# adri-romsor/iterative_inference_segm

Measured on AMD Instinct MI355X. Metric: refined images/s (FCN-8 + standard DAE, 10-step iterative inference, 224x224, 11 classes), higher is better.
Workload: dtype f32; 1 GPU; BASELINE configs[1]: FCN-8 + standard DAE (f64c1p2, pool4, trackind, skip), 224x224x3, batch 64/GPU, 10 steps, step 0.1, early stop off; per batch: pred_fcn_fn, val_fn, pred_dae_fn+val_fn, refine, val_fn; global_batch=64, parallelism=dp1

## Files before the change

### include/iiseg.h

```cpp
#ifndef IISEG_H
#define IISEG_H

#include <stdint.h>

#ifdef __cplusplus
extern "C" {
#endif

typedef enum iiseg_status {
    IISEG_OK = 0,
    IISEG_ERR_NULL = -1,
    IISEG_ERR_SHAPE = -2,
    IISEG_ERR_ALIGN = -3,
    IISEG_ERR_LAUNCH = -4,
    IISEG_ERR_UNSUPPORTED = -5
} iiseg_status;

const char* iiseg_strerror(int status);
const char* iiseg_last_hip_error(void);
int iiseg_abi_version(void);
const char* iiseg_target_arch(void);

int iiseg_profile_begin(int capacity);
int iiseg_profile_count(void);
int iiseg_profile_end(float* ms, int capacity);


#define IISEG_CONV_RELU 1u
#define IISEG_CONV_UNPOOL 2u
#define IISEG_CONV_TRANSPOSED2 4u
#define IISEG_CONV_X3 8u
#define IISEG_CONV_ZINS 16u

typedef struct iiseg_conv_desc {
    int32_t B, C1, C2, H, W;
    int32_t Cout, KH, KW, pad, dil;
    int32_t oy0, ox0, OH, OW;
    int32_t AH, AW, ay0, ax0;
    uint32_t flags;
    int32_t Kpad, Mpad;
    int32_t out_ctot, out_c0;
    int32_t out_H, out_W, out_y0, out_x0;
    int32_t tile_y0, tile_x0;
} iiseg_conv_desc;

int iiseg_conv_ktab_entries(const iiseg_conv_desc* d);
int iiseg_conv_plan(iiseg_conv_desc* d);

int iiseg_conv_pack_f32(void* stream, const iiseg_conv_desc* d, const float* w,
                        int64_t stride_o, int64_t stride_c, float* wp, int32_t* ktab);

int iiseg_conv_f32(void* stream, const iiseg_conv_desc* d, const float* x1, const float* x2,
                   const float* pre, const float* pooled, const float* wp, const int32_t* ktab,
                   const float* bias, const float* add, float* out);

int iiseg_conv_small_supported(const iiseg_conv_desc* d);
int iiseg_conv_pool_supported(const iiseg_conv_desc* d);
int iiseg_conv_pool_f32(void* stream, const iiseg_conv_desc* d, const float* x1, const float* x2,
                        const float* pre, const float* pooled, const float* wp, const int32_t* ktab,
                        const float* bias, const float* add, float* out, float* pool_out);

int iiseg_conv_mask_supported(const iiseg_conv_desc* d);
int iiseg_conv_mask_f32(void* stream, const iiseg_conv_desc* d, const float* x1, const float* x2,
                        const float* pre, const float* pooled, const uint8_t* mask_in,
                        const float* wp, const int32_t* ktab, const float* bias, const float* add,
                        float* out, float* pool_out, uint8_t* mask_out);

int iiseg_conv_bnrelu_supported(const iiseg_conv_desc* d);
int iiseg_conv_bnrelu_f32(void* stream, const iiseg_conv_desc* d, const float* x, int64_t x_bstride,
                          const float* beta, const float* gamma, const float* mean,
                          const float* inv_std, const float* wp, const int32_t* ktab,
                          const float* bias, float* out);

#define IISEG_WINO_INPUT 1u
#define IISEG_WINO_GEMM 2u
#define IISEG_WINO_OUTPUT 4u
#define IISEG_WINO_ALL 7u
#define IISEG_WINO_FUSED 8u
int iiseg_conv_wino_supported(const iiseg_conv_desc* d);
int64_t iiseg_conv_wino_weight_elems(const iiseg_conv_desc* d);
int64_t iiseg_conv_wino_workspace_elems(const iiseg_conv_desc* d);
int iiseg_conv_wino_pack_f32(void* stream, const iiseg_conv_desc* d, const float* w,
                             int64_t stride_o, int64_t stride_c, float* U);
int iiseg_conv_wino_f32(void* stream, const iiseg_conv_desc* d, const float* x1, const float* x2,
                        const float* pre, const float* pooled, const float* U, const float* bias,
                        const float* add, float* workspace, float* out, uint32_t stages);

int iiseg_conv_wino_bf16_supported(const iiseg_conv_desc* d);
int64_t iiseg_conv_wino_bf16_weight_bytes(const iiseg_conv_desc* d);
int64_t iiseg_conv_wino_bf16_workspace_bytes(const iiseg_conv_desc* d);
int iiseg_conv_wino_bf16_pack(void* stream, const iiseg_conv_desc* d, const float* w,
                              int64_t stride_o, int64_t stride_c, void* U16);
int iiseg_conv_wino_bf16(void* stream, const iiseg_conv_desc* d, const float* x1, const float* x2,
                         const float* pre, const float* pooled, const void* U16, const float* bias,
                         const float* add, void* workspace, float* out, uint32_t stages);

int iiseg_conv_gemm_bf16_supported(const iiseg_conv_desc* d);
int64_t iiseg_conv_gemm_bf16_weight_bytes(const iiseg_conv_desc* d);
int64_t iiseg_conv_gemm_bf16_workspace_bytes(const iiseg_conv_desc* d);
int iiseg_conv_gemm_bf16_pack(void* stream, const iiseg_conv_desc* d, const float* w,
                              int64_t stride_o, int64_t stride_c, void* U16);
int iiseg_conv_gemm_bf16(void* stream, const iiseg_conv_desc* d, const float* x, const void* U16,
                         const float* bias, void* workspace, float* out);

int iiseg_conv_halo_bf16_supported(const iiseg_conv_desc* d);
int64_t iiseg_conv_halo_bf16_weight_bytes(const iiseg_conv_desc* d);
int iiseg_conv_halo_bf16_pack(void* stream, const iiseg_conv_desc* d, const float* w,
                              int64_t stride_o, int64_t stride_c, void* wp16);
int iiseg_conv_halo_bf16(void* stream, const iiseg_conv_desc* d, const float* x1, const float* x2,
                         const float* pre, const float* pooled, const void* wp16, const float* bias,
                         const float* add, float* out, float* pool_out, const uint8_t* mask_in,
                         uint8_t* mask_out);

int iiseg_conv_wino_f64_supported(const iiseg_conv_desc* d);
int64_t iiseg_conv_wino_f64_weight_elems(const iiseg_conv_desc* d);
int64_t iiseg_conv_wino_f64_workspace_elems(const iiseg_conv_desc* d);
int iiseg_conv_wino_pack_f64(void* stream, const iiseg_conv_desc* d, const double* w,
                             int64_t stride_o, int64_t stride_c, double* U);
int iiseg_conv_wino_f64(void* stream, const iiseg_conv_desc* d, const double* x1, const double* x2,
                        const double* pre, const double* pooled, const double* U, const double* bias,
                        const double* add, double* workspace, double* out);

int iiseg_conv_c8_supported(const iiseg_conv_desc* d);
int iiseg_conv_c8_is_flat(const iiseg_conv_desc* d);
int iiseg_conv_c8_tiling(const iiseg_conv_desc* d, int pool, int32_t* out4);
int iiseg_conv_c8_force_tiling(int kind, int th, int tw);
int iiseg_conv_c8(void* stream, const iiseg_conv_desc* d, const void* x1, const void* x2,
                  const uint8_t* mask_in, const void* wp16, const float* bias, const void* add,
                  int add_kind, void* out, int out_kind, void* pool_out, uint8_t* mask_out);
int iiseg_conv_c8_slice(void* stream, const iiseg_conv_desc* d, const void* x1, int32_t x1_ctot,
                        const void* x2, const uint8_t* mask_in, const void* wp16, const float* bias,
                        const void* add, int add_kind, void* out, int out_kind, void* pool_out,
                        uint8_t* mask_out);
int iiseg_unpool_c8(void* stream, const void* up, const uint8_t* mask, void* out, int BC8, int H, int W,
                    int y0, int x0, int wh, int ww);
int iiseg_conv_c8_m16_supported(const iiseg_conv_desc* d);
int iiseg_conv_c8_m16(void* stream, const iiseg_conv_desc* d, const void* x1, int in_ctot,
                      const uint8_t* mask_in, const float* bn_a, const float* bn_b, const void* wp16,
                      const float* bias, void* out, int out_kind);
int64_t iiseg_conv_c8_m16_workspace_bytes(const iiseg_conv_desc* d);
int iiseg_conv_c8_m16_ws(void* stream, const iiseg_conv_desc* d, const void* x1, int in_ctot,
                         const uint8_t* mask_in, const float* bn_a, const float* bn_b, const void* wp16,
                         const float* bias, void* out, int out_kind, void* workspace,
                         int64_t workspace_bytes, float* stat_mean, float* stat_inv_std, double stat_eps,
                         const float* fold_beta, const float* fold_gamma, float* fold_a, float* fold_b,
                         int fold_n);
int64_t iiseg_conv1x1_c8_weight_bytes(int Cout, int Cin);
int iiseg_conv1x1_c8_pack(void* stream, const float* w, int64_t stride_o, int64_t stride_c, int Cout,
                          int Cin_w, int Cin, void* wp);
int iiseg_conv1x1_c8(void* stream, const void* x, int B, int Cin, int in_ctot, int H, int W,
                     const float* bn_a, const float* bn_b, const void* wp, const float* bias, int Cout,
                     int pool, void* out, int out_ctot, int out_c0);
int iiseg_bn_fold_f32(void* stream, const float* beta, const float* gamma, const float* mean,
                      const float* inv_std, float* a, float* b, int n);
int64_t iiseg_bn_stats_c8_workspace_elems(int n);
int iiseg_bn_stats_c8(void* stream, const void* x, int B, int Ctot, int c0, int n, int H, int W,
                      double eps, float* mean, float* inv_std, double* workspace);
int iiseg_nchw_to_c8(void* stream, const float* x, void* out, int B, int C, int H, int W, int C8n);
int iiseg_c8_to_nchw(void* stream, const void* x, float* out, int B, int C, int H, int W, int C8n);
int iiseg_nchw_to_c8_slice(void* stream, const float* x, void* out, int B, int C, int H, int W, int C8tot,
                           int c8_0);
int iiseg_c8_slice_to_nchw(void* stream, const void* x, float* out, int B, int C, int H, int W, int C8tot,
                           int c8_0);
int iiseg_pool_mask_c8(void* stream, const void* pre, int pre_f32, void* pooled, uint8_t* mask,
                       int BC8, int PH, int PW, int py0, int px0, int H, int W, int y0, int x0, int wh,
                       int ww);
int iiseg_conv_c8_split_weights(void* stream, const float* w, int64_t stride_o, int64_t stride_c,
                                int Cout, int Cin, float* out);
int iiseg_nchw_to_c8x3(void* stream, const float* x, void* out, int B, int C, int H, int W, int C8n);
int iiseg_c8x3_to_nchw(void* stream, const void* x, float* out, int B, int C, int H, int W, int C8n);
int iiseg_pool_mask_c8x3(void* stream, const void* pre, void* pooled, uint8_t* mask, int B, int C8n,
                         int PH, int PW, int py0, int px0, int H, int W, int y0, int x0, int wh,
                         int ww);

int iiseg_conv_gemm_supported(const iiseg_conv_desc* d);
int64_t iiseg_conv_gemm_workspace_elems(const iiseg_conv_desc* d);
int iiseg_conv_gemm_f32(void* stream, const iiseg_conv_desc* d, const float* x, const float* wp,
                        const float* bias, float* workspace, float* out, uint32_t stages);

int iiseg_maxpool2x2_f32(void* stream, const float* x, float* out, int32_t BC, int32_t H,
                         int32_t W);

int iiseg_maxpool2x2_window_f32(void* stream, const float* x, float* out, int32_t BC, int32_t H,
                                int32_t W, int32_t y0, int32_t x0, int32_t wh, int32_t ww);
int iiseg_maxpool2x2_window_f64(void* stream, const double* x, double* out, int32_t BC, int32_t H,
                                int32_t W, int32_t y0, int32_t x0, int32_t wh, int32_t ww);

int iiseg_unpool_eqmask_f32(void* stream, const float* up, const float* pre,
                            const float* pooled, float* out, int32_t BC, int32_t H, int32_t W);
int iiseg_unpool_eqmask_window_f32(void* stream, const float* up, const float* pre,
                                   const float* pooled, float* out, int32_t BC, int32_t H,
                                   int32_t W, int32_t y0, int32_t x0, int32_t wh, int32_t ww);

typedef struct iiseg_deconv_desc {
    int32_t B, Cin, H, W, Cout, K, stride;
    int32_t oy0, ox0, OH, OW;
    int32_t AH, AW, ay0, ax0;
} iiseg_deconv_desc;

int iiseg_deconv_f32(void* stream, const iiseg_deconv_desc* d, const float* x, const float* w,
                     const float* bias, const float* add, float* out);

int iiseg_deconv_phase_supported(const iiseg_deconv_desc* d, int has_add, int is_f64);
int64_t iiseg_deconv_phase_weight_elems(const iiseg_deconv_desc* d);
int iiseg_deconv_phase_pack_f32(void* stream, const iiseg_deconv_desc* d, const float* w, float* wp);
int iiseg_deconv_phase_pack_f64(void* stream, const iiseg_deconv_desc* d, const double* w, double* wp);
int iiseg_deconv_phase_f32(void* stream, const iiseg_deconv_desc* d, const float* x, const float* wp,
                           const float* bias, const float* add, float* out);
int iiseg_deconv_phase_f64(void* stream, const iiseg_deconv_desc* d, const double* x, const double* wp,
                           const double* bias, const double* add, double* out);

int iiseg_crop_softmax_f32(void* stream, const float* score, const float* minuend, float* out,
                           int32_t B, int32_t C, int32_t SH, int32_t SW, int32_t sy0,
                           int32_t sx0, int32_t H, int32_t W);

int iiseg_refine_partials(int32_t H, int32_t W);
int iiseg_refine_update_f32(void* stream, const float* score, float* y, const int32_t* active,
                            double* partial, int32_t B, int32_t C, int32_t SH, int32_t SW,
                            int32_t sy0, int32_t sx0, int32_t H, int32_t W, float step);
int iiseg_refine_update_c8_f32(void* stream, const float* score, float* y, const int32_t* active,
                               double* partial, void* y8, int32_t C8n, int32_t B, int32_t C,
                               int32_t SH, int32_t SW, int32_t sy0, int32_t sx0, int32_t H, int32_t W,
                               float step);
int iiseg_refine_finalize(void* stream, const double* partial, int32_t* active, int32_t* iters,
                          double* last_norm, int32_t B, int32_t nblk, int32_t HW, double eps);

int iiseg_ctx_tail_partials(int32_t H, int32_t W);
int iiseg_ctx_tail_f32(void* stream, const float* x, const float* wp6, int32_t Mpad6, const float* b6,
                       const float* wp7, int32_t Mpad7, const float* b7, float* y, const int32_t* active,
                       double* partial, float* ycat, int32_t cat_ctot, int32_t cat_c0, int32_t cat_H,
                       int32_t cat_W, int32_t cat_y0, int32_t cat_x0, int32_t B, int32_t C, int32_t H,
                       int32_t W, float step);

int iiseg_confusion_f32(void* stream, const float* y, const float* t, int64_t* cm, double* sums,
                        int32_t B, int32_t C, int32_t HW);

int iiseg_confusion_masked_f32(void* stream, const float* y, const float* t, const int32_t* active,
                               int64_t* cm, double* sums, int32_t B, int32_t C, int32_t HW);
int iiseg_confusion_masked_f64(void* stream, const double* y, const double* t,
                               const int32_t* active, int64_t* cm, double* sums, int32_t B,
                               int32_t C, int32_t HW);

int iiseg_count_nonfinite_f32(void* stream, const float* x, int64_t n, int32_t* counter);
int iiseg_count_nonfinite_f64(void* stream, const double* x, int64_t n, int32_t* counter);

int iiseg_sqerr_softmax_bwd_f32(void* stream, const float* score, const float* y, float* gscore,
                                int32_t B, int32_t C, int32_t SH, int32_t SW, int32_t sy0,
                                int32_t sx0, int32_t H, int32_t W);
int iiseg_sqerr_softmax_bwd_f64(void* stream, const double* score, const double* y, double* gscore,
                                int32_t B, int32_t C, int32_t SH, int32_t SW, int32_t sy0,
                                int32_t sx0, int32_t H, int32_t W);
int iiseg_depool_bwd_f32(void* stream, const float* gout, const float* pre, const float* pooled,
                         float* gup, int32_t BC, int32_t H, int32_t W);
int iiseg_depool_bwd_f64(void* stream, const double* gout, const double* pre, const double* pooled,
                         double* gup, int32_t BC, int32_t H, int32_t W);
int iiseg_pool_relu_bwd_f32(void* stream, const float* gpool, const float* pre, const float* pooled,
                            float* gz, int32_t BC, int32_t H, int32_t W);
int iiseg_pool_relu_bwd_f64(void* stream, const double* gpool, const double* pre,
                            const double* pooled, double* gz, int32_t BC, int32_t H, int32_t W);
int iiseg_grad_update_f32(void* stream, const float* score, const float* gthrough, float* y,
                          const int32_t* active, double* partial, int32_t B, int32_t C, int32_t SH,
                          int32_t SW, int32_t sy0, int32_t sx0, int32_t H, int32_t W, float step);
int iiseg_grad_update_f64(void* stream, const double* score, const double* gthrough, double* y,
                          const int32_t* active, double* partial, int32_t B, int32_t C, int32_t SH,
                          int32_t SW, int32_t sy0, int32_t sx0, int32_t H, int32_t W, double step);

int iiseg_add_noise_f32(void* stream, const float* x, const float* eps, float sigma, float* out,
                        int64_t n);
int iiseg_add_noise_f64(void* stream, const double* x, const double* eps, double sigma, double* out,
// ... 86 lines not shown
```

### iterative_inference_segm_amd/_lib.py

```python
import ctypes as C
import os

HERE = os.path.dirname(os.path.abspath(__file__))
LIB_PATH = os.path.join(HERE, 'libiiseg_hip.so')

ABI_VERSION = 32

CONV_RELU = 1
CONV_UNPOOL = 2
CONV_X3 = 8
CONV_TRANSPOSED2 = 4
CONV_ZINS = 16


class ConvDesc(C.Structure):
    _fields_ = [(n, C.c_int32) for n in
                ('B', 'C1', 'C2', 'H', 'W', 'Cout', 'KH', 'KW', 'pad', 'dil',
                 'oy0', 'ox0', 'OH', 'OW', 'AH', 'AW', 'ay0', 'ax0')] + \
               [('flags', C.c_uint32), ('Kpad', C.c_int32), ('Mpad', C.c_int32),
                ('out_ctot', C.c_int32), ('out_c0', C.c_int32),
                ('out_H', C.c_int32), ('out_W', C.c_int32), ('out_y0', C.c_int32),
                ('out_x0', C.c_int32), ('tile_y0', C.c_int32), ('tile_x0', C.c_int32)]


class DeconvDesc(C.Structure):
    _fields_ = [(n, C.c_int32) for n in
                ('B', 'Cin', 'H', 'W', 'Cout', 'K', 'stride', 'oy0', 'ox0', 'OH', 'OW',
                 'AH', 'AW', 'ay0', 'ax0')]


CRF_BILATERAL = 1
CRF_INPUT_0_255 = 2


class CrfDesc(C.Structure):
    _fields_ = [(n, C.c_int32) for n in ('B', 'C', 'H', 'W', 'R')] + [('flags', C.c_uint32)] + \
               [(n, C.c_double) for n in ('sxy_g', 'w_g', 'sxy_b', 'srgb', 'w_b', 'clip')]


_vp, _i32, _i64, _f32, _f64 = C.c_void_p, C.c_int32, C.c_int64, C.c_float, C.c_double

SIGNATURES = {
    'iiseg_strerror': (C.c_char_p, [C.c_int]),
    'iiseg_last_hip_error': (C.c_char_p, []),
    'iiseg_abi_version': (C.c_int, []),
    'iiseg_profile_begin': (C.c_int, [C.c_int]),
    'iiseg_profile_count': (C.c_int, []),
    'iiseg_profile_end': (C.c_int, [C.POINTER(C.c_float), C.c_int]),
    'iiseg_target_arch': (C.c_char_p, []),
    'iiseg_conv_ktab_entries': (C.c_int, [C.POINTER(ConvDesc)]),
    'iiseg_conv_plan': (C.c_int, [C.POINTER(ConvDesc)]),
    'iiseg_conv_pack_f32': (C.c_int, [_vp, C.POINTER(ConvDesc), _vp, _i64, _i64, _vp, _vp]),
    'iiseg_conv_f32': (C.c_int, [_vp, C.POINTER(ConvDesc)] + [_vp] * 9),
    'iiseg_conv_small_supported': (C.c_int, [C.POINTER(ConvDesc)]),
    'iiseg_conv_pool_supported': (C.c_int, [C.POINTER(ConvDesc)]),
    'iiseg_conv_pool_f32': (C.c_int, [_vp, C.POINTER(ConvDesc)] + [_vp] * 10),
    'iiseg_conv_mask_supported': (C.c_int, [C.POINTER(ConvDesc)]),
    'iiseg_conv_mask_f32': (C.c_int, [_vp, C.POINTER(ConvDesc)] + [_vp] * 12),
    'iiseg_conv_bnrelu_supported': (C.c_int, [C.POINTER(ConvDesc)]),
    'iiseg_conv_bnrelu_f32': (C.c_int, [_vp, C.POINTER(ConvDesc), _vp, _i64] + [_vp] * 8),
    'iiseg_conv_wino_supported': (C.c_int, [C.POINTER(ConvDesc)]),
    'iiseg_conv_wino_weight_elems': (_i64, [C.POINTER(ConvDesc)]),
    'iiseg_conv_wino_workspace_elems': (_i64, [C.POINTER(ConvDesc)]),
    'iiseg_conv_wino_pack_f32': (C.c_int, [_vp, C.POINTER(ConvDesc), _vp, _i64, _i64, _vp]),
    'iiseg_conv_wino_f32': (C.c_int, [_vp, C.POINTER(ConvDesc)] + [_vp] * 9 + [C.c_uint32]),
    'iiseg_conv_wino_bf16_supported': (C.c_int, [C.POINTER(ConvDesc)]),
    'iiseg_conv_wino_bf16_weight_bytes': (_i64, [C.POINTER(ConvDesc)]),
    'iiseg_conv_wino_bf16_workspace_bytes': (_i64, [C.POINTER(ConvDesc)]),
    'iiseg_conv_wino_bf16_pack': (C.c_int, [_vp, C.POINTER(ConvDesc), _vp, _i64, _i64, _vp]),
    'iiseg_conv_wino_bf16': (C.c_int, [_vp, C.POINTER(ConvDesc)] + [_vp] * 9 + [C.c_uint32]),
    'iiseg_conv_gemm_bf16_supported': (C.c_int, [C.POINTER(ConvDesc)]),
    'iiseg_conv_gemm_bf16_weight_bytes': (_i64, [C.POINTER(ConvDesc)]),
    'iiseg_conv_gemm_bf16_workspace_bytes': (_i64, [C.POINTER(ConvDesc)]),
    'iiseg_conv_gemm_bf16_pack': (C.c_int, [_vp, C.POINTER(ConvDesc), _vp, _i64, _i64, _vp]),
    'iiseg_conv_gemm_bf16': (C.c_int, [_vp, C.POINTER(ConvDesc)] + [_vp] * 5),
    'iiseg_conv_halo_bf16_supported': (C.c_int, [C.POINTER(ConvDesc)]),
    'iiseg_conv_halo_bf16_weight_bytes': (_i64, [C.POINTER(ConvDesc)]),
    'iiseg_conv_halo_bf16_pack': (C.c_int, [_vp, C.POINTER(ConvDesc), _vp, _i64, _i64, _vp]),
    'iiseg_conv_halo_bf16': (C.c_int, [_vp, C.POINTER(ConvDesc)] + [_vp] * 11),
    'iiseg_conv_wino_f64_supported': (C.c_int, [C.POINTER(ConvDesc)]),
    'iiseg_conv_wino_f64_weight_elems': (_i64, [C.POINTER(ConvDesc)]),
    'iiseg_conv_wino_f64_workspace_elems': (_i64, [C.POINTER(ConvDesc)]),
    'iiseg_conv_wino_pack_f64': (C.c_int, [_vp, C.POINTER(ConvDesc), _vp, _i64, _i64, _vp]),
    'iiseg_conv_wino_f64': (C.c_int, [_vp, C.POINTER(ConvDesc)] + [_vp] * 9),
    'iiseg_conv_c8_supported': (C.c_int, [C.POINTER(ConvDesc)]),
    'iiseg_conv_c8_is_flat': (C.c_int, [C.POINTER(ConvDesc)]),
    'iiseg_conv_c8_force_tiling': (C.c_int, [C.c_int, C.c_int, C.c_int]),
    'iiseg_conv_c8_tiling': (C.c_int, [C.POINTER(ConvDesc), C.c_int, C.POINTER(C.c_int32)]),
    'iiseg_conv_c8': (C.c_int, [_vp, C.POINTER(ConvDesc)] + [_vp] * 6 + [_i32, _vp, _i32, _vp, _vp]),
    'iiseg_conv_c8_slice': (C.c_int, [_vp, C.POINTER(ConvDesc), _vp, _i32] + [_vp] * 5 + [_i32, _vp, _i32, _vp, _vp]),
    'iiseg_unpool_c8': (C.c_int, [_vp] * 4 + [C.c_int] * 7),
    'iiseg_conv_c8_m16_supported': (C.c_int, [C.POINTER(ConvDesc)]),
    'iiseg_conv_c8_m16': (C.c_int, [_vp, C.POINTER(ConvDesc), _vp, _i32] + [_vp] * 6 + [_i32]),
    'iiseg_conv_c8_m16_workspace_bytes': (_i64, [C.POINTER(ConvDesc)]),
    'iiseg_conv_c8_m16_ws': (C.c_int, [_vp, C.POINTER(ConvDesc), _vp, _i32] + [_vp] * 6 + [_i32, _vp, _i64, _vp, _vp, _f64] + [_vp] * 4 + [_i32]),
    'iiseg_conv1x1_c8_weight_bytes': (_i64, [C.c_int, C.c_int]),
    'iiseg_conv1x1_c8_pack': (C.c_int, [_vp, _vp, _i64, _i64, C.c_int, C.c_int, C.c_int, _vp]),
    'iiseg_conv1x1_c8': (C.c_int, [_vp, _vp] + [C.c_int] * 5 + [_vp] * 4 + [C.c_int, C.c_int, _vp, C.c_int, C.c_int]),
    'iiseg_bn_fold_f32': (C.c_int, [_vp] * 7 + [_i32]),
    'iiseg_bn_stats_c8_workspace_elems': (C.c_int64, [_i32]),
    'iiseg_bn_stats_c8': (C.c_int, [_vp, _vp] + [_i32] * 6 + [C.c_double, _vp, _vp, _vp]),
    'iiseg_nchw_to_c8_slice': (C.c_int, [_vp, _vp, _vp] + [_i32] * 6),
    'iiseg_c8_slice_to_nchw': (C.c_int, [_vp, _vp, _vp] + [_i32] * 6),
    'iiseg_nchw_to_c8': (C.c_int, [_vp, _vp, _vp] + [_i32] * 5),
    'iiseg_c8_to_nchw': (C.c_int, [_vp, _vp, _vp] + [_i32] * 5),
    'iiseg_pool_mask_c8': (C.c_int, [_vp, _vp, _i32, _vp, _vp] + [_i32] * 11),
    'iiseg_conv_c8_split_weights': (C.c_int, [_vp, _vp, _i64, _i64, _i32, _i32, _vp]),
    'iiseg_nchw_to_c8x3': (C.c_int, [_vp, _vp, _vp] + [_i32] * 5),
    'iiseg_c8x3_to_nchw': (C.c_int, [_vp, _vp, _vp] + [_i32] * 5),
    'iiseg_pool_mask_c8x3': (C.c_int, [_vp, _vp, _vp, _vp] + [_i32] * 12),
    'iiseg_conv_gemm_supported': (C.c_int, [C.POINTER(ConvDesc)]),
    'iiseg_conv_gemm_workspace_elems': (_i64, [C.POINTER(ConvDesc)]),
    'iiseg_conv_gemm_f32': (C.c_int, [_vp, C.POINTER(ConvDesc)] + [_vp] * 5 + [C.c_uint32]),
    'iiseg_maxpool2x2_f32': (C.c_int, [_vp, _vp, _vp, _i32, _i32, _i32]),
    'iiseg_unpool_eqmask_f32': (C.c_int, [_vp, _vp, _vp, _vp, _vp, _i32, _i32, _i32]),
    'iiseg_maxpool2x2_window_f32': (C.c_int, [_vp] * 3 + [_i32] * 7),
    'iiseg_maxpool2x2_window_f64': (C.c_int, [_vp] * 3 + [_i32] * 7),
    'iiseg_unpool_eqmask_window_f32': (C.c_int, [_vp] * 5 + [_i32] * 7),
    'iiseg_unpool_eqmask_window_f64': (C.c_int, [_vp] * 5 + [_i32] * 7),
    'iiseg_deconv_f32': (C.c_int, [_vp, C.POINTER(DeconvDesc)] + [_vp] * 5),
    'iiseg_deconv_phase_supported': (C.c_int, [C.POINTER(DeconvDesc), C.c_int, C.c_int]),
    'iiseg_deconv_phase_weight_elems': (C.c_int64, [C.POINTER(DeconvDesc)]),
    'iiseg_deconv_phase_pack_f32': (C.c_int, [_vp, C.POINTER(DeconvDesc), _vp, _vp]),
    'iiseg_deconv_phase_pack_f64': (C.c_int, [_vp, C.POINTER(DeconvDesc), _vp, _vp]),
    'iiseg_deconv_phase_f32': (C.c_int, [_vp, C.POINTER(DeconvDesc)] + [_vp] * 5),
    'iiseg_deconv_phase_f64': (C.c_int, [_vp, C.POINTER(DeconvDesc)] + [_vp] * 5),
    'iiseg_crop_softmax_f32': (C.c_int, [_vp, _vp, _vp, _vp] + [_i32] * 8),
    'iiseg_refine_partials': (C.c_int, [_i32, _i32]),
    'iiseg_refine_update_f32': (C.c_int, [_vp] * 5 + [_i32] * 8 + [_f32]),
    'iiseg_refine_update_c8_f32': (C.c_int, [_vp] * 6 + [_i32] * 9 + [_f32]),
    'iiseg_refine_finalize': (C.c_int, [_vp] * 5 + [_i32] * 3 + [_f64]),
    'iiseg_ctx_tail_partials': (C.c_int, [_i32, _i32]),
    'iiseg_ctx_tail_f32': (C.c_int, [_vp] * 3 + [_i32] + [_vp] * 2 + [_i32] + [_vp] * 5 + [_i32] * 10 + [_f32]),
    'iiseg_confusion_f32': (C.c_int, [_vp] * 5 + [_i32] * 3),
    'iiseg_confusion_masked_f32': (C.c_int, [_vp] * 6 + [_i32] * 3),
    'iiseg_confusion_masked_f64': (C.c_int, [_vp] * 6 + [_i32] * 3),
    'iiseg_bn_stats_workspace_elems': (_i64, [_i32]),
    'iiseg_bn_stats_f32': (C.c_int, [_vp, _vp, _i64, _i32, _i32, _i32, _f32, _vp, _vp, _vp]),
    'iiseg_bn_relu_f32': (C.c_int, [_vp, _vp, _i64, _i32, _i32, _i32] + [_vp] * 5),
    'iiseg_bn_stats_f64': (C.c_int, [_vp, _vp, _i64, _i32, _i32, _i32, _f64, _vp, _vp, _vp]),
    'iiseg_bn_relu_f64': (C.c_int, [_vp, _vp, _i64, _i32, _i32, _i32] + [_vp] * 5),
    'iiseg_sqerr_softmax_bwd_f32': (C.c_int, [_vp] * 4 + [_i32] * 8),
    'iiseg_sqerr_softmax_bwd_f64': (C.c_int, [_vp] * 4 + [_i32] * 8),
    'iiseg_depool_bwd_f32': (C.c_int, [_vp] * 5 + [_i32] * 3),
    'iiseg_depool_bwd_f64': (C.c_int, [_vp] * 5 + [_i32] * 3),
    'iiseg_pool_relu_bwd_f32': (C.c_int, [_vp] * 5 + [_i32] * 3),
    'iiseg_pool_relu_bwd_f64': (C.c_int, [_vp] * 5 + [_i32] * 3),
    'iiseg_grad_update_f32': (C.c_int, [_vp] * 6 + [_i32] * 8 + [C.c_float]),
    'iiseg_grad_update_f64': (C.c_int, [_vp] * 6 + [_i32] * 8 + [C.c_double]),
    'iiseg_add_noise_f32': (C.c_int, [_vp, _vp, _vp, C.c_float, _vp, _i64]),
    'iiseg_add_noise_f64': (C.c_int, [_vp, _vp, _vp, C.c_double, _vp, _i64]),
    'iiseg_dropout_apply_f32': (C.c_int, [_vp, _vp, _vp, C.c_float, _i64]),
    'iiseg_dropout_apply_f64': (C.c_int, [_vp, _vp, _vp, C.c_double, _i64]),
    'iiseg_bn_affine_window_f32': (C.c_int, [_vp, _vp] + [_i32] * 8 + [_vp] * 4),
    'iiseg_bn_affine_window_f64': (C.c_int, [_vp, _vp] + [_i32] * 8 + [_vp] * 4),
    'iiseg_conv_plan_f64': (C.c_int, [C.POINTER(ConvDesc)]),
    'iiseg_conv_pack_f64': (C.c_int, [_vp, C.POINTER(ConvDesc), _vp, _i64, _i64, _vp]),
    'iiseg_conv_f64': (C.c_int, [_vp, C.POINTER(ConvDesc)] + [_vp] * 8),
    'iiseg_conv_halo_f64_supported': (C.c_int, [C.POINTER(ConvDesc)]),
    'iiseg_conv_pool_f64_supported': (C.c_int, [C.POINTER(ConvDesc)]),
    'iiseg_conv_pool_f64': (C.c_int, [_vp, C.POINTER(ConvDesc)] + [_vp] * 9),
    'iiseg_conv_mask_f64_supported': (C.c_int, [C.POINTER(ConvDesc)]),
    'iiseg_conv_mask_f64': (C.c_int, [_vp, C.POINTER(ConvDesc)] + [_vp] * 11),
    'iiseg_conv_gemm_f64_supported': (C.c_int, [C.POINTER(ConvDesc)]),
    'iiseg_conv_gemm_f64_workspace_elems': (_i64, [C.POINTER(ConvDesc)]),
    'iiseg_conv_gemm_f64': (C.c_int, [_vp, C.POINTER(ConvDesc)] + [_vp] * 5),
    'iiseg_im2col_f64': (C.c_int, [_vp, _vp, _vp] + [_i32] * 6),
    'iiseg_maxpool2x2_f64': (C.c_int, [_vp, _vp, _vp, _i32, _i32, _i32]),
    'iiseg_unpool_eqmask_f64': (C.c_int, [_vp, _vp, _vp, _vp, _vp, _i32, _i32, _i32]),
    'iiseg_deconv_f64': (C.c_int, [_vp, C.POINTER(DeconvDesc)] + [_vp] * 5),
    'iiseg_crop_softmax_f64': (C.c_int, [_vp, _vp, _vp, _vp] + [_i32] * 8),
    'iiseg_refine_update_f64': (C.c_int, [_vp] * 5 + [_i32] * 8 + [_f64]),
    'iiseg_confusion_f64': (C.c_int, [_vp] * 5 + [_i32] * 3),
    'iiseg_count_nonfinite_f32': (C.c_int, [_vp, _vp, _i64, _vp]),
    'iiseg_count_nonfinite_f64': (C.c_int, [_vp, _vp, _i64, _vp]),
    'iiseg_crf_supported': (C.c_int, [C.POINTER(CrfDesc)]),
    'iiseg_crf_prepare_f32': (C.c_int, [_vp, C.POINTER(CrfDesc)] + [_vp] * 7),
    'iiseg_crf_prepare_f64': (C.c_int, [_vp, C.POINTER(CrfDesc)] + [_vp] * 7),
    'iiseg_crf_step_f32': (C.c_int, [_vp, C.POINTER(CrfDesc)] + [_vp] * 6),
    'iiseg_crf_step_f64': (C.c_int, [_vp, C.POINTER(CrfDesc)] + [_vp] * 6),
}

_lib = None


def load():
    global _lib
    if _lib is not None:
        return _lib
    if not os.path.exists(LIB_PATH):
        raise RuntimeError(
            'libiiseg_hip.so is missing (%s). Build it with '
            '`python -m iterative_inference_segm_amd.build`; there is no CPU fallback.' % LIB_PATH)
    import torch
    lib = C.CDLL(LIB_PATH)
    for name, (res, args) in SIGNATURES.items():
        fn = getattr(lib, name)
        fn.restype = res
        fn.argtypes = args
    if lib.iiseg_abi_version() != ABI_VERSION:
# ... 13 lines not shown
```

### iterative_inference_segm_amd/csrc/abi.hip

```cpp
#include <mutex>
#include <vector>
#include "common.h"

namespace {
std::mutex g_prof_mu;
std::vector<hipEvent_t> g_prof_ev;
int g_prof_on = 0, g_prof_n = 0, g_prof_cap = 0;
}

extern "C" int iiseg_prof_next(hipEvent_t* start, hipEvent_t* stop) {
    if (!g_prof_on) return 0;
    std::lock_guard<std::mutex> g(g_prof_mu);
    if (!g_prof_on || g_prof_n >= g_prof_cap) return 0;
    *start = g_prof_ev[2 * g_prof_n];
    *stop = g_prof_ev[2 * g_prof_n + 1];
    ++g_prof_n;
    return 1;
}

extern "C" int iiseg_profile_begin(int capacity) {
    if (capacity <= 0) return IISEG_ERR_SHAPE;
    std::lock_guard<std::mutex> g(g_prof_mu);
    while ((int)g_prof_ev.size() < 2 * capacity) {
        hipEvent_t e;
        if (hipEventCreate(&e) != hipSuccess) return IISEG_ERR_LAUNCH;
        g_prof_ev.push_back(e);
    }
    g_prof_cap = capacity;
    g_prof_n = 0;
    g_prof_on = 1;
    return IISEG_OK;
}

extern "C" int iiseg_profile_count(void) { return g_prof_on ? g_prof_n : -1; }

extern "C" int iiseg_profile_end(float* ms, int capacity) {
    std::lock_guard<std::mutex> g(g_prof_mu);
    if (!g_prof_on) return -1;
    g_prof_on = 0;
    const int n = g_prof_n < capacity ? g_prof_n : capacity;
    for (int i = 0; i < n; ++i) {
        if (hipEventSynchronize(g_prof_ev[2 * i + 1]) != hipSuccess ||
            hipEventElapsedTime(&ms[i], g_prof_ev[2 * i], g_prof_ev[2 * i + 1]) != hipSuccess)
            return IISEG_ERR_LAUNCH;
    }
    return n;
}

extern "C" const char* iiseg_strerror(int status) {
    switch (status) {
        case IISEG_OK: return "ok";
        case IISEG_ERR_NULL: return "required pointer is NULL";
        case IISEG_ERR_SHAPE: return "inconsistent or unsupported shape";
        case IISEG_ERR_ALIGN: return "pointer is not 16-byte aligned";
        case IISEG_ERR_LAUNCH: return "kernel launch failed";
        case IISEG_ERR_UNSUPPORTED: return "no kernel variant implements this request";
        default: return "unknown iiseg status";
    }
}

extern "C" const char* iiseg_last_hip_error(void) {
    return hipGetErrorString((hipError_t)iiseg_hip_error_slot());
}

extern "C" int iiseg_abi_version(void) { return 32; }
extern "C" const char* iiseg_target_arch(void) { return "gfx950"; }
```

### iterative_inference_segm_amd/csrc/conv_wino.hip

```cpp
#include <hip/hip_runtime.h>
#include <stdint.h>
#include <stdlib.h>
#include "iiseg.h"
#include "common.h"
#include "conv_common.h"

using namespace iiseg;

namespace {

struct WinoParams {
    const float* x1;
    const float* x2;
    const float* pre;
    const float* pooled;
    int h2, w2;
    const float* U;
    const float* bias;
    const float* add;
    float* V;
    float* M;
    float* out;
    int B, C1, C2, H, W;
    int Cout, pad;
    int oy0, ox0, OH, OW;
    int ty0, tx0, nty, ntx;
    int T, Tpad;
    int Kc, Mpad;
    int AH, AW, ay0, ax0;
    int relu;
    int out_ctot, out_c0, out_H, out_W, out_y0, out_x0;
    int n_ttiles, n_mtiles;
};

constexpr int RSRC_W3 = 0x00027000;

__device__ __forceinline__ __amdgpu_buffer_rsrc_t mk_rsrc(const float* base, int bytes) {
    return __builtin_amdgcn_make_buffer_rsrc((void*)base, 0, bytes, RSRC_W3);
}

__global__ void wino_weight_kernel(const float* __restrict__ w, int64_t so, int64_t sc,
                                   float* __restrict__ U, int Cin, int Cout, int Kc, int Mpad) {
    const int64_t n = (int64_t)Kc * Mpad;
    for (int64_t i = blockIdx.x * (int64_t)blockDim.x + threadIdx.x; i < n;
         i += (int64_t)gridDim.x * blockDim.x) {
        const int c = (int)(i / Mpad), co = (int)(i % Mpad);
        double g[3][3], t[4][3];
        const bool real = c < Cin && co < Cout;
#pragma unroll
        for (int a = 0; a < 3; ++a)
#pragma unroll
            for (int b = 0; b < 3; ++b) g[a][b] = real ? (double)w[co * so + c * sc + a * 3 + b] : 0.0;
#pragma unroll
        for (int b = 0; b < 3; ++b) {
            t[0][b] = g[0][b];
            t[1][b] = 0.5 * (g[0][b] + g[1][b] + g[2][b]);
            t[2][b] = 0.5 * (g[0][b] - g[1][b] + g[2][b]);
            t[3][b] = g[2][b];
        }
#pragma unroll
        for (int a = 0; a < 4; ++a) {
            const double u0 = t[a][0], u1 = 0.5 * (t[a][0] + t[a][1] + t[a][2]),
                         u2 = 0.5 * (t[a][0] - t[a][1] + t[a][2]), u3 = t[a][2];
            U[(int64_t)(a * 4 + 0) * n + i] = (float)u0;
            U[(int64_t)(a * 4 + 1) * n + i] = (float)u1;
            U[(int64_t)(a * 4 + 2) * n + i] = (float)u2;
            U[(int64_t)(a * 4 + 3) * n + i] = (float)u3;
        }
    }
}

constexpr int ICH = 4;
template <bool UNPOOL, int PY, int PX>
__global__ __launch_bounds__(256) void wino_input_kernel(const WinoParams p) {
    const int t = blockIdx.x * 256 + threadIdx.x;
    if (t >= p.T) return;
    const int ntt = p.nty * p.ntx;
    const int b = t / ntt;
    const int r = t - b * ntt;
    const int tyl = r / p.ntx, txl = r - tyl * p.ntx;
    const int iy0 = p.ty0 + 2 * tyl - p.pad, ix0 = p.tx0 + 2 * txl - p.pad;
    int rowoff[4];
    bool rok[4], cok[4];
#pragma unroll
    for (int i = 0; i < 4; ++i) {
        rok[i] = (unsigned)(iy0 + i) < (unsigned)p.H;
        cok[i] = (unsigned)(ix0 + i) < (unsigned)p.W;
        rowoff[i] = (iy0 + i) * p.W + ix0;
    }
    constexpr int NQY = UNPOOL ? (PY ? 3 : 2) : 1, NQX = UNPOOL ? (PX ? 3 : 2) : 1;
    const int qy0 = (iy0 - PY) >> 1, qx0 = (ix0 - PX) >> 1;
    bool qrok[NQY], qcok[NQX];
    int qoff[NQY];
    if constexpr (UNPOOL) {
#pragma unroll
        for (int i = 0; i < NQY; ++i) {
            qrok[i] = (unsigned)(qy0 + i) < (unsigned)p.h2;
            qoff[i] = (qy0 + i) * p.w2 + qx0;
        }
#pragma unroll
        for (int j = 0; j < NQX; ++j) qcok[j] = (unsigned)(qx0 + j) < (unsigned)p.w2;
    }
    const size_t HW = (size_t)p.H * p.W, hw2 = (size_t)p.h2 * p.w2;
    const size_t xis = (size_t)p.Kc * p.Tpad;
    constexpr int NC_ = UNPOOL ? ICH / 2 : ICH;
    const int c0 = blockIdx.y * NC_;
    float pv[NC_][4][4];
    float pq[UNPOOL ? NC_ : 1][NQY][NQX], uq[UNPOOL ? NC_ : 1][NQY][NQX];
#pragma unroll
    for (int cc = 0; cc < NC_; ++cc) {
        const int c = min(c0 + cc, p.Kc - 1);
        if constexpr (UNPOOL) {
            const float* prep = p.pre + ((size_t)b * p.C1 + c) * HW;
            const float* poolp = p.pooled + ((size_t)b * p.C1 + c) * hw2;
            const float* upp = p.x1 + ((size_t)b * p.C1 + c) * hw2;
#pragma unroll
            for (int i = 0; i < NQY; ++i)
#pragma unroll
                for (int j = 0; j < NQX; ++j) {
                    const int o = (qrok[i] && qcok[j]) ? qoff[i] + j : 0;
                    pq[cc][i][j] = poolp[o];
                    uq[cc][i][j] = upp[o];
                }
#pragma unroll
            for (int i = 0; i < 4; ++i)
#pragma unroll
                for (int j = 0; j < 4; ++j) pv[cc][i][j] = prep[(rok[i] && cok[j]) ? rowoff[i] + j : 0];
        } else {
            const float* src = c < p.C1 ? p.x1 + ((size_t)b * p.C1 + c) * HW
                                        : p.x2 + ((size_t)b * p.C2 + (c - p.C1)) * HW;
#pragma unroll
            for (int i = 0; i < 4; ++i)
#pragma unroll
                for (int j = 0; j < 4; ++j) pv[cc][i][j] = src[(rok[i] && cok[j]) ? rowoff[i] + j : 0];
        }
    }
#pragma unroll
    for (int cc = 0; cc < NC_; ++cc) {
        const int c = c0 + cc;
        if (c >= p.Kc) break;
        float d[4][4];
#pragma unroll
        for (int i = 0; i < 4; ++i)
#pragma unroll
            for (int j = 0; j < 4; ++j) {
                if constexpr (UNPOOL) {
                    const int qi = (PY + i) >> 1, qj = (PX + j) >> 1;
                    const bool ok = rok[i] && cok[j] && qrok[qi] && qcok[qj];
                    d[i][j] = (ok && pv[cc][i][j] == pq[cc][qi][qj]) ? uq[cc][qi][qj] : 0.f;
                } else {
                    d[i][j] = (rok[i] && cok[j]) ? pv[cc][i][j] : 0.f;
                }
            }
        float e[4][4];
#pragma unroll
        for (int j = 0; j < 4; ++j) {
            e[0][j] = d[0][j] - d[2][j];
            e[1][j] = d[1][j] + d[2][j];
            e[2][j] = d[2][j] - d[1][j];
            e[3][j] = d[1][j] - d[3][j];
        }
        float* v = p.V + (size_t)c * p.Tpad + t;
#pragma unroll
        for (int i = 0; i < 4; ++i) {
            v[(size_t)(i * 4 + 0) * xis] = e[i][0] - e[i][2];
            v[(size_t)(i * 4 + 1) * xis] = e[i][1] + e[i][2];
            v[(size_t)(i * 4 + 2) * xis] = e[i][2] - e[i][1];
            v[(size_t)(i * 4 + 3) * xis] = e[i][1] - e[i][3];
        }
    }
}


constexpr int ILDS_E = 12, ILDS_CH = 8;
template <bool UNPOOL, int NT>
__global__ __launch_bounds__(NT) void wino_input_lds_kernel(const WinoParams p, const int chunks) {
    constexpr int ILDS_CAP = ILDS_E * NT;
    __shared__ __attribute__((aligned(16))) float Ls[2][ILDS_CAP];
    const int tid = threadIdx.x;
    const int b = blockIdx.x / chunks, chunk = blockIdx.x - b * chunks;
    const int ntt = p.nty * p.ntx;
    const int tl0 = chunk * NT, tl = tl0 + tid;
    const bool tvalid = tl < ntt;
    const int row_first = tl0 / p.ntx;
    const int row_last = min(ntt - 1, tl0 + NT - 1) / p.ntx;
    const int NR = 2 * (row_last - row_first + 1) + 2, NC = 2 * p.ntx + 2, NE = NR * NC;
    const int iyb = p.ty0 + 2 * row_first - p.pad, ixb = p.tx0 - p.pad;
    int goff[ILDS_E], qoff[UNPOOL ? ILDS_E : 1];
#pragma unroll
    for (int i = 0; i < ILDS_E; ++i) {
        const int e = i * NT + tid;
        const int r = e / NC, c = e - r * NC;
        const int iy = iyb + r, ix = ixb + c;
        bool ok = e < NE && (unsigned)iy < (unsigned)p.H && (unsigned)ix < (unsigned)p.W;
        goff[i] = ok ? iy * p.W + ix : -1;
        if constexpr (UNPOOL) {
            ok = ok && iy < 2 * p.h2 && ix < 2 * p.w2;
            qoff[i] = ok ? (iy >> 1) * p.w2 + (ix >> 1) : -1;
        }
    }
    const int tyl = tl / p.ntx, txl = tl - tyl * p.ntx;
    const int lbase = 2 * (tyl - row_first) * NC + 2 * txl;
    const size_t HW = (size_t)p.H * p.W, hw2 = (size_t)p.h2 * p.w2;
    const size_t xis = (size_t)p.Kc * p.Tpad;
    const int t = b * ntt + tl;
    const int c0 = blockIdx.y * ILDS_CH;
    float v[ILDS_E];

    auto fetch = [&](int c) __attribute__((always_inline)) {
        if constexpr (UNPOOL) {
            const float* prep = p.pre + ((size_t)b * p.C1 + c) * HW;
            const float* poolp = p.pooled + ((size_t)b * p.C1 + c) * hw2;
            const float* upp = p.x1 + ((size_t)b * p.C1 + c) * hw2;
            float pv[ILDS_E], pq[ILDS_E], uq[ILDS_E];
#pragma unroll
            for (int i = 0; i < ILDS_E; ++i) {
                const int go = qoff[i] >= 0 ? goff[i] : 0, qo = qoff[i] >= 0 ? qoff[i] : 0;
                pv[i] = prep[go];
                pq[i] = poolp[qo];
                uq[i] = upp[qo];
            }
#pragma unroll
            for (int i = 0; i < ILDS_E; ++i) v[i] = (qoff[i] >= 0 && pv[i] == pq[i]) ? uq[i] : 0.f;
        } else {
            const float* src = c < p.C1 ? p.x1 + ((size_t)b * p.C1 + c) * HW
                                        : p.x2 + ((size_t)b * p.C2 + (c - p.C1)) * HW;
            float pv[ILDS_E];
#pragma unroll
            for (int i = 0; i < ILDS_E; ++i) pv[i] = src[goff[i] >= 0 ? goff[i] : 0];
#pragma unroll
            for (int i = 0; i < ILDS_E; ++i) v[i] = goff[i] >= 0 ? pv[i] : 0.f;
        }
    };

    fetch(c0);
    for (int cc = 0; cc < ILDS_CH; ++cc) {
        const int c = c0 + cc;
        float* L = Ls[cc & 1];
#pragma unroll
        for (int i = 0; i < ILDS_E; ++i)
            if (i * NT + tid < NE) L[i * NT + tid] = v[i];
        if (cc + 1 < ILDS_CH) fetch(c + 1);
        __syncthreads();
        if (tvalid) {
            float d[4][4];
#pragma unroll
            for (int i = 0; i < 4; ++i) {
                const float2 lo = *reinterpret_cast<const float2*>(L + lbase + i * NC);
                const float2 hi = *reinterpret_cast<const float2*>(L + lbase + i * NC + 2);
                d[i][0] = lo.x; d[i][1] = lo.y; d[i][2] = hi.x; d[i][3] = hi.y;
            }
            float e[4][4];
#pragma unroll
            for (int j = 0; j < 4; ++j) {
                e[0][j] = d[0][j] - d[2][j];
                e[1][j] = d[1][j] + d[2][j];
                e[2][j] = d[2][j] - d[1][j];
                e[3][j] = d[1][j] - d[3][j];
            }
            float* vo = p.V + (size_t)c * p.Tpad + t;
#pragma unroll
            for (int i = 0; i < 4; ++i) {
                vo[(size_t)(i * 4 + 0) * xis] = e[i][0] - e[i][2];
                vo[(size_t)(i * 4 + 1) * xis] = e[i][1] + e[i][2];
                vo[(size_t)(i * 4 + 2) * xis] = e[i][2] - e[i][1];
                vo[(size_t)(i * 4 + 3) * xis] = e[i][1] - e[i][3];
            }
        }
    }
}

template <int BM, int BN, int WM, int WN, int NBUF, int BK = 16>
__global__ __launch_bounds__(WM * WN * 64, 2) void wino_gemm_kernel(const WinoParams p) {
    constexpr int NCH = BK / 2;
    constexpr int WTM = BM / WM, WTN = BN / WN;
    constexpr int TM = WTM / 32, TN = WTN / 32;
    constexpr int NW = WM * WN, NT = NW * 64;
    constexpr int AV = BK * BM / 4, BV = BK * BN / 4;
    constexpr int NA = NW == 8 ? 256 : NT;
    constexpr int APT = AV / NA, BPT = BV / 256;
    static_assert((NW == 4 || NW == 8) && AV % NA == 0 && BV % 256 == 0, "tile config");

    __shared__ __attribute__((aligned(16))) float As[NBUF][BK][BM];
    __shared__ __attribute__((aligned(16))) float Bs[NBUF][BK][BN];

    const int per_xi = p.n_ttiles * p.n_mtiles;
    int xi, tt, mt;
    {
        const int nb = gridDim.x, bid = blockIdx.x;
        const int q = nb / 8, r = nb % 8, xcd = bid % 8, l = bid / 8;
        const int v = (xcd < r ? xcd * (q + 1) : r * (q + 1) + (xcd - r) * q) + l;
        xi = v / per_xi;
        const int w = v - xi * per_xi;
// ... 192 lines not shown
    for (int s = 0; s < total; ++s) {
        const int buf = s & 1;
        int nxi = xi, nkt1 = kt + 1;
        if (nkt1 == nkt) { nkt1 = 0; ++nxi; }
        const bool more = s + 1 < total;
        float a[2][TM], b[2][TN];
#pragma unroll
        for (int i = 0; i < TM; ++i) a[0][i] = As[buf][lh][wm * WTM + i * 32 + l31];
#pragma unroll
        for (int j = 0; j < TN; ++j) b[0][j] = Bs[buf][lh][wn * WTN + j * 32 + l31];
        static_for<0, NCH>([&](auto CH) __attribute__((always_inline)) {
            constexpr int ch = decltype(CH)::value;
            if constexpr (ch + 1 < NCH) {
                const int kk = (ch + 1) * 2 + lh;
#pragma unroll
                for (int i = 0; i < TM; ++i) a[(ch + 1) & 1][i] = As[buf][kk][wm * WTM + i * 32 + l31];
#pragma unroll
                for (int j = 0; j < TN; ++j) b[(ch + 1) & 1][j] = Bs[buf][kk][wn * WTN + j * 32 + l31];
            }
#pragma unroll
            for (int i = 0; i < TM; ++i)
#pragma unroll
                for (int j = 0; j < TN; ++j)
                    acc[i][j] = __builtin_amdgcn_mfma_f32_32x32x2f32(a[ch & 1][i], b[ch & 1][j],
                                                                     acc[i][j], 0, 0, 0);
            if constexpr (ch == 0) {
                if (more) WINO_STAGE(nxi, nkt1, buf ^ 1)
            }
            __builtin_amdgcn_sched_barrier(0);
        });
        if (nkt1 == 0) {
            const int wi = xi >> 2, wj = xi & 3;
            const float r0 = wi < 3 ? 1.f : 0.f, r1 = wi == 0 ? 0.f : (wi == 1 ? 1.f : -1.f);
            const float c0 = wj < 3 ? 1.f : 0.f, c1 = wj == 0 ? 0.f : (wj == 1 ? 1.f : -1.f);
            const float k00 = r0 * c0, k01 = r0 * c1, k10 = r1 * c0, k11 = r1 * c1;
#define WINO_FOLD(Q, KQ)                                                                            \
            if ((KQ) != 0.f) {                                                                      \
                _Pragma("unroll") for (int i = 0; i < TM; ++i)                                      \
                _Pragma("unroll") for (int j = 0; j < TN; ++j)                                      \
                _Pragma("unroll") for (int r = 0; r < 16; ++r)                                      \
                    Y[Q][i][j][r] = fmaf((KQ), acc[i][j][r], Y[Q][i][j][r]);                        \
            }
            WINO_FOLD(0, k00)
            WINO_FOLD(1, k01)
            WINO_FOLD(2, k10)
            WINO_FOLD(3, k11)
#undef WINO_FOLD
#pragma unroll
            for (int i = 0; i < TM; ++i)
#pragma unroll
                for (int j = 0; j < TN; ++j)
#pragma unroll
                    for (int r = 0; r < 16; ++r) acc[i][j][r] = 0.f;
        }
        xi = nxi;
        kt = nkt1;
        asm volatile("s_waitcnt vmcnt(0)" ::: "memory");
        __syncthreads();
    }
#undef WINO_STAGE

    typedef float f32x2u __attribute__((ext_vector_type(2), aligned(4)));
    const int ntt = p.nty * p.ntx;
    const size_t OPL = (size_t)p.out_H * p.out_W, APL = (size_t)p.AH * p.AW;
    float* Lbias = &As[0][0][0];
    for (int f = tid; f < BM; f += NT) Lbias[f] = (p.bias && m0 + f < p.Cout) ? p.bias[m0 + f] : 0.f;
    __syncthreads();
    float bias_r[TM][16];
#pragma unroll
    for (int i = 0; i < TM; ++i)
#pragma unroll
        for (int r = 0; r < 16; ++r) bias_r[i][r] = Lbias[wm * WTM + i * 32 + (r & 3) + 8 * (r >> 2) + 4 * lh];
#pragma unroll
    for (int j = 0; j < TN; ++j) {
        const int t = t0 + wn * WTN + j * 32 + l31;
        if (t >= p.T) continue;
        const int b = t / ntt;
        const int rr = t - b * ntt;
        const int tyl = rr / p.ntx, txl = rr - tyl * p.ntx;
        const int wy = p.ty0 + 2 * tyl - p.oy0, wx = p.tx0 + 2 * txl - p.ox0;
        const bool rok[2] = {(unsigned)wy < (unsigned)p.OH, (unsigned)(wy + 1) < (unsigned)p.OH};
        const bool cok[2] = {(unsigned)wx < (unsigned)p.OW, (unsigned)(wx + 1) < (unsigned)p.OW};
        const bool pair = cok[0] && cok[1];
        float* ob = p.out + ((size_t)b * p.out_ctot + p.out_c0) * OPL +
                    (ptrdiff_t)(p.out_y0 + wy) * p.out_W + p.out_x0 + wx;
        const float* ab = p.add ? p.add + (size_t)b * p.Cout * APL +
                                      (ptrdiff_t)(p.ay0 + wy) * p.AW + p.ax0 + wx
                                : nullptr;
#pragma unroll
        for (int i = 0; i < TM; ++i)
#pragma unroll
            for (int r = 0; r < 16; ++r) {
                const int co = m0 + wm * WTM + i * 32 + (r & 3) + 8 * (r >> 2) + 4 * lh;
                if (co >= p.Cout) continue;
                const float bias = bias_r[i][r];
                float* oc = ob + (size_t)co * OPL;
                const float* ac = ab ? ab + (size_t)co * APL : nullptr;
#pragma unroll
                for (int a = 0; a < 2; ++a) {
                    if (!rok[a]) continue;
                    float v0 = Y[2 * a][i][j][r] + bias, v1 = Y[2 * a + 1][i][j][r] + bias;
                    if (pair) {
                        if (ac) {
                            const f32x2u a2 = *reinterpret_cast<const f32x2u*>(ac + a * p.AW);
                            v0 += a2[0];
                            v1 += a2[1];
                        }
                        if (p.relu) {
                            v0 = fmaxf(v0, 0.f);
                            v1 = fmaxf(v1, 0.f);
                        }
                        *reinterpret_cast<f32x2u*>(oc + (size_t)a * p.out_W) = f32x2u{v0, v1};
                    } else {
                        if (cok[0]) {
                            if (ac) v0 += ac[a * p.AW];
                            if (p.relu) v0 = fmaxf(v0, 0.f);
                            oc[(size_t)a * p.out_W] = v0;
                        }
                        if (cok[1]) {
                            if (ac) v1 += ac[a * p.AW + 1];
                            if (p.relu) v1 = fmaxf(v1, 0.f);
                            oc[(size_t)a * p.out_W + 1] = v1;
                        }
                    }
                }
            }
    }
}

constexpr int OCH = 4;
__global__ __launch_bounds__(256) void wino_output_kernel(const WinoParams p) {
    const int t = blockIdx.x * 256 + threadIdx.x;
    if (t >= p.T) return;
    const int ntt = p.nty * p.ntx;
    const int b = t / ntt;
    const int r = t - b * ntt;
    const int tyl = r / p.ntx, txl = r - tyl * p.ntx;
    const int wy = p.ty0 + 2 * tyl - p.oy0, wx = p.tx0 + 2 * txl - p.ox0;
    const bool okr[2] = {(unsigned)wy < (unsigned)p.OH, (unsigned)(wy + 1) < (unsigned)p.OH};
    const bool okc[2] = {(unsigned)wx < (unsigned)p.OW, (unsigned)(wx + 1) < (unsigned)p.OW};
    const size_t xis = (size_t)p.Mpad * p.Tpad;
    const size_t OPL = (size_t)p.out_H * p.out_W, APL = (size_t)p.AH * p.AW;
    const int co0 = blockIdx.y * OCH;
    float mv[OCH][16], av[OCH][4];
#pragma unroll
    for (int cc = 0; cc < OCH; ++cc) {
        const int co = min(co0 + cc, p.Cout - 1);
        const float* m = p.M + (size_t)co * p.Tpad + t;
#pragma unroll
        for (int x = 0; x < 16; ++x) mv[cc][x] = m[(size_t)x * xis];
        if (p.add) {
            const float* ad = p.add + ((size_t)b * p.Cout + co) * APL;
#pragma unroll
            for (int i = 0; i < 2; ++i)
#pragma unroll
                for (int j = 0; j < 2; ++j) {
                    const bool ok = okr[i] && okc[j];
                    const ptrdiff_t idx = (ptrdiff_t)(p.ay0 + wy + i) * p.AW + p.ax0 + wx + j;
                    const float a = ad[ok ? idx : 0];
                    av[cc][i * 2 + j] = ok ? a : 0.f;
                }
        }
    }
#pragma unroll
    for (int cc = 0; cc < OCH; ++cc) {
        const int co = co0 + cc;
        if (co >= p.Cout) break;
        float s2[2][4];
#pragma unroll
        for (int j = 0; j < 4; ++j) {
            const float m0 = mv[cc][j], m1 = mv[cc][4 + j], m2 = mv[cc][8 + j], m3 = mv[cc][12 + j];
            s2[0][j] = m0 + m1 + m2;
            s2[1][j] = m1 - m2 - m3;
        }
        const float bias = p.bias ? p.bias[co] : 0.f;
        float* o = p.out + ((size_t)b * p.out_ctot + p.out_c0 + co) * OPL +
                   (ptrdiff_t)(p.out_y0 + wy) * p.out_W + p.out_x0 + wx;
#pragma unroll
        for (int i = 0; i < 2; ++i) {
            float y[2] = {s2[i][0] + s2[i][1] + s2[i][2], s2[i][1] - s2[i][2] - s2[i][3]};
#pragma unroll
            for (int j = 0; j < 2; ++j) {
                if (okr[i] && okc[j]) {
                    float v = y[j] + bias;
                    if (p.add) v += av[cc][i * 2 + j];
                    if (p.relu) v = fmaxf(v, 0.f);
                    o[(ptrdiff_t)i * p.out_W + j] = v;
                }
            }
        }
    }
}

inline int round_up(int v, int m) { return (v + m - 1) / m * m; }

struct WinoGeom {
    int Kc, Mpad, bm, ty0, tx0, nty, ntx, T, Tpad;
};

int wino_geom(const iiseg_conv_desc* d, WinoGeom& g) {
    if (!d) return IISEG_ERR_NULL;
    if (d->KH != 3 || d->KW != 3 || d->dil != 1 || (d->flags & IISEG_CONV_TRANSPOSED2))
        return IISEG_ERR_UNSUPPORTED;
    if ((d->flags & IISEG_CONV_UNPOOL) && d->C2 != 0) return IISEG_ERR_UNSUPPORTED;
    if (d->B <= 0 || d->C1 <= 0 || d->C2 < 0 || d->H <= 0 || d->W <= 0 || d->Cout <= 0 ||
        d->pad < 0 || d->OH <= 0 || d->OW <= 0 || d->oy0 < 0 || d->ox0 < 0)
        return IISEG_ERR_SHAPE;
    const int fullH = d->H + 2 * d->pad - 2, fullW = d->W + 2 * d->pad - 2;
    if (d->oy0 + d->OH > fullH || d->ox0 + d->OW > fullW) return IISEG_ERR_SHAPE;
    if ((d->C1 + d->C2) % 16) return IISEG_ERR_UNSUPPORTED;
    g.Kc = d->C1 + d->C2;
    g.bm = d->Cout > 128 ? 256 : (d->Cout > 64 ? 128 : 64);
    g.Mpad = round_up(d->Cout, g.bm);
    if ((d->tile_y0 | d->tile_x0) & ~1) return IISEG_ERR_SHAPE;
    g.ty0 = d->oy0 - ((d->oy0 - d->tile_y0) & 1);
    g.tx0 = d->ox0 - ((d->ox0 - d->tile_x0) & 1);
    g.nty = (d->oy0 + d->OH - g.ty0 + 1) >> 1;
    g.ntx = (d->ox0 + d->OW - g.tx0 + 1) >> 1;
    const int64_t T = (int64_t)d->B * g.nty * g.ntx;
    const int64_t Tpad = (T + 127) / 128 * 128;
    if (Tpad * g.Kc * 4 >= (int64_t)1 << 31 || (int64_t)g.Kc * g.Mpad * 4 >= (int64_t)1 << 31)
        return IISEG_ERR_UNSUPPORTED;
    g.T = (int)T;
    g.Tpad = (int)Tpad;
    return IISEG_OK;
}

void launch_wino_input(hipStream_t s, const WinoParams& p, bool unpool) {
    static const int lds = getenv("IISEG_WINO_INPUT_LDS") ? atoi(getenv("IISEG_WINO_INPUT_LDS")) : 1;
    const int ntt = p.nty * p.ntx;
    int nt = 0;
    double best = 0.0;
    for (int cand = 256; cand >= 128; cand >>= 1) {
        const int span = (cand - 1 + p.ntx - 1) / p.ntx + 1;
        const int rows = span < p.nty ? span : p.nty;
        if ((2 * rows + 2) * (2 * p.ntx + 2) > ILDS_E * cand) continue;
        const double util = (double)ntt / (((ntt + cand - 1) / cand) * cand);
        if (util > best + 0.02) { best = util; nt = cand; }
    }
    if (lds && nt && best >= 0.8 && p.Kc % ILDS_CH == 0) {
        const int chunks = (ntt + nt - 1) / nt;
        const dim3 g2(p.B * chunks, p.Kc / ILDS_CH);
#define WINO_ILDS(U, N) IISEG_LAUNCH((wino_input_lds_kernel<U, N>), g2, dim3(N), 0, s, p, chunks)
        if (unpool) { if (nt == 256) WINO_ILDS(true, 256); else if (nt == 128) WINO_ILDS(true, 128); else WINO_ILDS(true, 64); }
        else { if (nt == 256) WINO_ILDS(false, 256); else if (nt == 128) WINO_ILDS(false, 128); else WINO_ILDS(false, 64); }
#undef WINO_ILDS
        return;
    }
    const int nc = unpool ? ICH / 2 : ICH;
    const dim3 grid((p.T + 255) / 256, (p.Kc + nc - 1) / nc), block(256);
    if (!unpool) {
        IISEG_LAUNCH((wino_input_kernel<false, 0, 0>), grid, block, 0, s, p);
        return;
    }
    const int py = (p.ty0 - p.pad) & 1, px = (p.tx0 - p.pad) & 1;
    if (py && px) IISEG_LAUNCH((wino_input_kernel<true, 1, 1>), grid, block, 0, s, p);
    else if (py) IISEG_LAUNCH((wino_input_kernel<true, 1, 0>), grid, block, 0, s, p);
    else if (px) IISEG_LAUNCH((wino_input_kernel<true, 0, 1>), grid, block, 0, s, p);
    else IISEG_LAUNCH((wino_input_kernel<true, 0, 0>), grid, block, 0, s, p);
}

}

int iiseg_wino_output_launch(hipStream_t s, const iiseg_conv_desc* d, const float* M, int Mpad,
                             int Tpad, const float* bias, const float* add, float* out) {
    WinoParams p = {};
    p.M = const_cast<float*>(M);
    p.bias = bias; p.add = add; p.out = out;
    p.B = d->B; p.Cout = d->Cout; p.pad = d->pad;
    p.oy0 = d->oy0; p.ox0 = d->ox0; p.OH = d->OH; p.OW = d->OW;
    p.ty0 = d->oy0 - ((d->oy0 - d->tile_y0) & 1);
    p.tx0 = d->ox0 - ((d->ox0 - d->tile_x0) & 1);
    p.nty = (d->oy0 + d->OH - p.ty0 + 1) >> 1;
    p.ntx = (d->ox0 + d->OW - p.tx0 + 1) >> 1;
    p.T = d->B * p.nty * p.ntx;
    p.Tpad = Tpad; p.Mpad = Mpad;
    p.AH = d->AH; p.AW = d->AW; p.ay0 = d->ay0; p.ax0 = d->ax0;
    p.relu = (d->flags & IISEG_CONV_RELU) ? 1 : 0;
    p.out_ctot = d->out_ctot > 0 ? d->out_ctot : d->Cout;
    p.out_c0 = d->out_ctot > 0 ? d->out_c0 : 0;
    p.out_H = d->out_H > 0 ? d->out_H : d->OH;
    p.out_W = d->out_H > 0 ? d->out_W : d->OW;
    p.out_y0 = d->out_H > 0 ? d->out_y0 : 0;
    p.out_x0 = d->out_H > 0 ? d->out_x0 : 0;
    IISEG_LAUNCH(wino_output_kernel, dim3((p.T + 255) / 256, (d->Cout + OCH - 1) / OCH),
                       dim3(256), 0, s, p);
    return iiseg_check_launch();
}

extern "C" int iiseg_conv_wino_supported(const iiseg_conv_desc* d) {
    WinoGeom g;
    return wino_geom(d, g) == IISEG_OK ? 1 : 0;
}

extern "C" int64_t iiseg_conv_wino_weight_elems(const iiseg_conv_desc* d) {
    WinoGeom g;
    if (wino_geom(d, g) != IISEG_OK) return 0;
    return (int64_t)16 * g.Kc * g.Mpad;
}

extern "C" int64_t iiseg_conv_wino_workspace_elems(const iiseg_conv_desc* d) {
    WinoGeom g;
    if (wino_geom(d, g) != IISEG_OK) return 0;
    return (int64_t)16 * g.Tpad * ((int64_t)g.Kc + g.Mpad);
}

extern "C" int iiseg_conv_wino_pack_f32(void* stream, const iiseg_conv_desc* d, const float* w,
                                        int64_t stride_o, int64_t stride_c, float* U) {
    WinoGeom g;
    const int st = wino_geom(d, g);
    if (st) return st;
    if (!w || !U) return IISEG_ERR_NULL;
    const int64_t n = (int64_t)g.Kc * g.Mpad;
    const int grid = (int)((n + 255) / 256 < 4096 ? (n + 255) / 256 : 4096);
    IISEG_LAUNCH(wino_weight_kernel, dim3(grid), dim3(256), 0, (hipStream_t)stream, w,
                       stride_o, stride_c, U, d->C1 + d->C2, d->Cout, g.Kc, g.Mpad);
    return iiseg_check_launch();
}

extern "C" int iiseg_conv_wino_f32(void* stream, const iiseg_conv_desc* d, const float* x1,
                                   const float* x2, const float* pre, const float* pooled,
                                   const float* U, const float* bias,
                                   const float* add, float* workspace, float* out,
                                   uint32_t stages) {
    WinoGeom g;
    const int st = wino_geom(d, g);
    if (st) return st;
    if (!x1 || !U || !workspace || !out) return IISEG_ERR_NULL;
    if (d->C2 > 0 && !x2) return IISEG_ERR_NULL;
    const bool unpool = (d->flags & IISEG_CONV_UNPOOL) != 0;
    if (unpool && (!pre || !pooled)) return IISEG_ERR_NULL;
    if (((uintptr_t)U & 15) || ((uintptr_t)workspace & 15)) return IISEG_ERR_ALIGN;
    WinoParams p;
    p.x1 = x1;
    p.x2 = x2;
    p.pre = pre;
    p.pooled = pooled;
    p.h2 = d->H / 2;
    p.w2 = d->W / 2;
    p.U = U;
    p.bias = bias;
    p.add = add;
    p.V = workspace;
    p.M = workspace + (size_t)16 * g.Kc * g.Tpad;
    p.out = out;
    p.B = d->B; p.C1 = d->C1; p.C2 = d->C2; p.H = d->H; p.W = d->W;
    p.Cout = d->Cout; p.pad = d->pad;
    p.oy0 = d->oy0; p.ox0 = d->ox0; p.OH = d->OH; p.OW = d->OW;
    p.ty0 = g.ty0; p.tx0 = g.tx0; p.nty = g.nty; p.ntx = g.ntx;
    p.T = g.T; p.Tpad = g.Tpad; p.Kc = g.Kc; p.Mpad = g.Mpad;
    p.AH = d->AH; p.AW = d->AW; p.ay0 = d->ay0; p.ax0 = d->ax0;
    if (add && (d->ay0 < 0 || d->ax0 < 0 || d->ay0 + d->OH > d->AH || d->ax0 + d->OW > d->AW))
        return IISEG_ERR_SHAPE;
    p.relu = (d->flags & IISEG_CONV_RELU) ? 1 : 0;
    p.out_ctot = d->out_ctot > 0 ? d->out_ctot : d->Cout;
    p.out_c0 = d->out_ctot > 0 ? d->out_c0 : 0;
    if (p.out_c0 < 0 || p.out_c0 + d->Cout > p.out_ctot) return IISEG_ERR_SHAPE;
    p.out_H = d->out_H > 0 ? d->out_H : d->OH;
    p.out_W = d->out_H > 0 ? d->out_W : d->OW;
    p.out_y0 = d->out_H > 0 ? d->out_y0 : 0;
    p.out_x0 = d->out_H > 0 ? d->out_x0 : 0;
    if (p.out_y0 < 0 || p.out_x0 < 0 || p.out_y0 + d->OH > p.out_H || p.out_x0 + d->OW > p.out_W)
        return IISEG_ERR_SHAPE;
    p.n_ttiles = g.Tpad / 128;
    p.n_mtiles = g.Mpad / g.bm;
    hipStream_t s = (hipStream_t)stream;
    const int tb = (g.T + 255) / 256;
    if (stages & IISEG_WINO_FUSED) {
        if (g.Kc % 32) return IISEG_ERR_UNSUPPORTED;
        if (stages & IISEG_WINO_INPUT)
            launch_wino_input(s, p, unpool);
        if (stages & IISEG_WINO_GEMM) {
            if (g.bm == 64) {
                p.n_mtiles = g.Mpad / 64;
                IISEG_LAUNCH((wino_fused_kernel<64, 128, 1, 4, 32, 2>),
                                   dim3(p.n_ttiles * p.n_mtiles), dim3(256), 0, s, p);
                return iiseg_check_launch();
            }
            p.n_mtiles = g.Mpad / 128;
            const int w0 = p.n_ttiles * p.n_mtiles, w2 = (g.Tpad / 64) * p.n_mtiles;
            const double cost0 = (w0 + 255) / 256, cost2 = 0.5 * 1.03 * ((w2 + 255) / 256);
            static const int bk64 = getenv("IISEG_WINO_FUSED_BK") ? atoi(getenv("IISEG_WINO_FUSED_BK")) == 64 : 0;
            const bool big = bk64 && g.Kc % 64 == 0;
            if (g.Kc <= 128 || cost2 < cost0) {
                p.n_ttiles = g.Tpad / 64;
                if (big)
                    IISEG_LAUNCH((wino_fused_kernel<128, 64, 2, 2, 64, 2>),
                                       dim3(p.n_ttiles * p.n_mtiles), dim3(256), 0, s, p);
                else
                IISEG_LAUNCH((wino_fused_kernel<128, 64, 2, 2, 32, 2>),
                                   dim3(p.n_ttiles * p.n_mtiles), dim3(256), 0, s, p);
            } else if (big)
                IISEG_LAUNCH((wino_fused_kernel<128, 128, 2, 4, 64, 2>),
                                   dim3(p.n_ttiles * p.n_mtiles), dim3(512), 0, s, p);
            else
            IISEG_LAUNCH((wino_fused_kernel<128, 128, 2, 4, 32, 2>),
                               dim3(p.n_ttiles * p.n_mtiles), dim3(512), 0, s, p);
        }
        return iiseg_check_launch();
    }
    if (stages & IISEG_WINO_INPUT)
        launch_wino_input(s, p, unpool);
    const int grid = 16 * p.n_ttiles * p.n_mtiles;
    if (stages & IISEG_WINO_GEMM) {
        static const int nbuf = getenv("IISEG_WINO_NBUF") ? atoi(getenv("IISEG_WINO_NBUF")) : 2;
        int bm = g.bm;
        if (bm == 64) {
            IISEG_LAUNCH((wino_gemm_kernel<64, 128, 1, 4, 2>), dim3(grid), dim3(256), 0, s, p);
            bm = 0;
        }
        if (bm == 256) {
            const int w256 = grid, w128 = 2 * grid;
            if (0.5 * 1.06 * ((w128 + 255) / 256) < (double)((w256 + 255) / 256)) bm = 128;
        }
        const int grid2 = bm ? 16 * p.n_ttiles * (g.Mpad / bm) : 0;
        if (bm) p.n_mtiles = g.Mpad / bm;
        static const int bk32 = getenv("IISEG_WINO_GEMM_BK") ? atoi(getenv("IISEG_WINO_GEMM_BK")) == 32 : 0;
        if (bm && bk32 && g.Kc % 32 == 0 && nbuf != 3) {
            if (bm == 256)
                IISEG_LAUNCH((wino_gemm_kernel<256, 128, 4, 2, 2, 32>), dim3(grid), dim3(512), 0, s, p);
            else
                IISEG_LAUNCH((wino_gemm_kernel<128, 128, 2, 2, 2, 32>), dim3(grid2), dim3(256), 0, s, p);
        } else
        if (bm == 0) {
        } else if (bm == 256 && nbuf == 3)
            IISEG_LAUNCH((wino_gemm_kernel<256, 128, 4, 2, 3>), dim3(grid), dim3(512), 0, s, p);
        else if (bm == 256)
            IISEG_LAUNCH((wino_gemm_kernel<256, 128, 4, 2, 2>), dim3(grid), dim3(512), 0, s, p);
        else if (nbuf == 3)
            IISEG_LAUNCH((wino_gemm_kernel<128, 128, 2, 2, 3>), dim3(grid2), dim3(256), 0, s, p);
        else
            IISEG_LAUNCH((wino_gemm_kernel<128, 128, 2, 2, 2>), dim3(grid2), dim3(256), 0, s, p);
    }
    if (stages & IISEG_WINO_OUTPUT)
        IISEG_LAUNCH(wino_output_kernel, dim3(tb, (d->Cout + OCH - 1) / OCH), dim3(256), 0, s,
                           p);
    return iiseg_check_launch();
}

namespace {

struct GemmConvGeom {
    int K, Kpad, Mpad, bm, T, Tpad, S, Kc;
};

__global__ __launch_bounds__(256) void gemm_im2col_kernel(const float* __restrict__ x,
                                                          float* __restrict__ V, int B, int C, int H,
                                                          int W, int KH, int KW, int OH, int OW, int K,
                                                          int Kpad, int T, int Tpad) {
    const int t = blockIdx.x * 256 + threadIdx.x;
    if (t >= T) return;
    const int OHW = OH * OW;
    const int b = t / OHW, r = t - b * OHW;
    const int oy = r / OW, ox = r - oy * OW;
    const int KK = KH * KW;
    const float* xb = x + (size_t)b * C * H * W + (size_t)oy * W + ox;
    for (int k = blockIdx.y; k < Kpad; k += gridDim.y) {
        float v = 0.f;
        if (k < K) {
            const int c = k / KK, tap = k - c * KK;
            const int ky = tap / KW, kx = tap - ky * KW;
            v = xb[(size_t)c * H * W + ky * W + kx];
        }
        V[(size_t)k * Tpad + t] = v;
    }
}

__global__ __launch_bounds__(256) void gemm_output_kernel(const float* __restrict__ M,
                                                          const float* __restrict__ bias,
                                                          float* __restrict__ out, int Cout, int OHW,
                                                          int T, int Tpad, int Mpad, int S, int relu) {
    const int t = blockIdx.x * 256 + threadIdx.x;
    if (t >= T) return;
    const int b = t / OHW, px = t - b * OHW;
    const size_t ss = (size_t)Mpad * Tpad;
    for (int co = blockIdx.y; co < Cout; co += gridDim.y) {
        const float* m = M + (size_t)co * Tpad + t;
        float v = m[0];
        for (int s = 1; s < S; ++s) v += m[(size_t)s * ss];
        if (bias) v += bias[co];
        if (relu) v = fmaxf(v, 0.f);
        out[((size_t)b * Cout + co) * OHW + px] = v;
    }
}

int gemm_conv_geom(const iiseg_conv_desc* d, GemmConvGeom& g) {
    if (!d) return IISEG_ERR_NULL;
    if (d->pad != 0 || d->dil != 1 || d->C2 != 0 ||
        (d->flags & (IISEG_CONV_UNPOOL | IISEG_CONV_TRANSPOSED2)))
        return IISEG_ERR_UNSUPPORTED;
    const int fullH = d->H - d->KH + 1, fullW = d->W - d->KW + 1;
    if (fullH <= 0 || fullW <= 0) return IISEG_ERR_SHAPE;
    if (d->oy0 != 0 || d->ox0 != 0 || d->OH != fullH || d->OW != fullW || d->out_ctot != 0 ||
        d->out_H != 0)
        return IISEG_ERR_UNSUPPORTED;
    g.K = d->C1 * d->KH * d->KW;
    g.Kpad = d->Kpad;
    g.Mpad = d->Mpad;
    if (g.Kpad < g.K || g.Kpad % 16 || g.Mpad % 128 || g.Mpad < d->Cout) return IISEG_ERR_UNSUPPORTED;
    g.bm = g.Mpad % 256 == 0 ? 256 : 128;
    const int64_t T = (int64_t)d->B * fullH * fullW;
    const int64_t Tpad = (T + 127) / 128 * 128;
    if (Tpad * g.Kpad * 4 >= (int64_t)1 << 31 || (int64_t)g.Kpad * g.Mpad * 4 >= (int64_t)1 << 31)
        return IISEG_ERR_UNSUPPORTED;
    g.T = (int)T;
    g.Tpad = (int)Tpad;
    const int tiles = 25 * (g.Mpad / g.bm), units = g.Kpad / 16;
    const double tile_s = 2.0 * g.Kpad * g.bm * 128 / (131e12 / 256);
    const double red_s = 8.0 * g.Mpad * 3200 / 5e12;
    double best = 1e30;
    g.S = 1;
    for (int S = 1; S <= 16; ++S) {
        if (units % S || units / S < 8) continue;
        const double cost = (double)((S * tiles + 255) / 256) / S * tile_s + S * red_s;
        if (cost < best) { best = cost; g.S = S; }
    }
    g.Kc = g.Kpad / g.S;
    return IISEG_OK;
}

}

// ... 59 lines not shown
```

### iterative_inference_segm_amd/csrc/pool_unpool.hip

```cpp
#include "common.h"

namespace {

template <typename T>
__global__ __launch_bounds__(256) void maxpool2x2_kernel(const T* __restrict__ x,
                                                         T* __restrict__ out, int BC, int H,
                                                         int W, int h, int w) {
    const size_t n = (size_t)BC * h * w;
    for (size_t i = blockIdx.x * (size_t)blockDim.x + threadIdx.x; i < n;
         i += (size_t)gridDim.x * blockDim.x) {
        const int ox = (int)(i % w);
        const size_t t = i / w;
        const int oy = (int)(t % h);
        const size_t bc = t / h;
        const T* r0 = x + (bc * H + 2 * oy) * (size_t)W + 2 * ox;
        const T* r1 = r0 + W;
        const T a = r0[0] > r0[1] ? r0[0] : r0[1];
        const T b = r1[0] > r1[1] ? r1[0] : r1[1];
        out[i] = a > b ? a : b;
    }
}

template <typename T>
__global__ __launch_bounds__(256) void unpool_eqmask_kernel(const T* __restrict__ up,
                                                            const T* __restrict__ pre,
                                                            const T* __restrict__ pooled,
                                                            T* __restrict__ out, int BC, int H,
                                                            int W, int h, int w) {
    const size_t n = (size_t)BC * H * W;
    for (size_t i = blockIdx.x * (size_t)blockDim.x + threadIdx.x; i < n;
         i += (size_t)gridDim.x * blockDim.x) {
        const int x = (int)(i % W);
        const size_t t = i / W;
        const int y = (int)(t % H);
        const size_t bc = t / H;
        T v = 0;
        if (y < 2 * h && x < 2 * w) {
            const size_t j = (bc * h + (y >> 1)) * (size_t)w + (x >> 1);
            v = (pre[i] == pooled[j]) ? up[j] : (T)0;
        }
        out[i] = v;
    }
}

template <typename T>
__global__ __launch_bounds__(256) void maxpool2x2_window_kernel(const T* __restrict__ x,
                                                                T* __restrict__ out, int BC, int H,
                                                                int W, int h, int w, int y0, int x0,
                                                                int wh, int ww) {
    const size_t n = (size_t)BC * wh * ww;
    if (n < ((size_t)1 << 31)) {
        const unsigned n32 = (unsigned)n, uww = (unsigned)ww, uwh = (unsigned)wh;
        for (unsigned i = blockIdx.x * blockDim.x + threadIdx.x; i < n32; i += gridDim.x * blockDim.x) {
            const unsigned t = i / uww;
            const int ox = x0 + (int)(i - t * uww);
            const unsigned bc = t / uwh;
            const int oy = y0 + (int)(t - bc * uwh);
            const T* r0 = x + ((size_t)bc * H + 2 * oy) * (size_t)W + 2 * ox;
            const T* r1 = r0 + W;
            const T a = r0[0] > r0[1] ? r0[0] : r0[1];
            const T b = r1[0] > r1[1] ? r1[0] : r1[1];
            out[((size_t)bc * h + oy) * (size_t)w + ox] = a > b ? a : b;
        }
        return;
    }
    for (size_t i = blockIdx.x * (size_t)blockDim.x + threadIdx.x; i < n;
         i += (size_t)gridDim.x * blockDim.x) {
        const int ox = x0 + (int)(i % ww);
        const size_t t = i / ww;
        const int oy = y0 + (int)(t % wh);
        const size_t bc = t / wh;
        const T* r0 = x + (bc * H + 2 * oy) * (size_t)W + 2 * ox;
        const T* r1 = r0 + W;
        const T a = r0[0] > r0[1] ? r0[0] : r0[1];
        const T b = r1[0] > r1[1] ? r1[0] : r1[1];
        out[(bc * h + oy) * (size_t)w + ox] = a > b ? a : b;
    }
}

template <typename T>
__global__ __launch_bounds__(256) void unpool_eqmask_window_kernel(
    const T* __restrict__ up, const T* __restrict__ pre, const T* __restrict__ pooled,
    T* __restrict__ out, int BC, int H, int W, int h, int w, int y0, int x0, int wh, int ww) {
    const size_t n = (size_t)BC * wh * ww;
    for (size_t i = blockIdx.x * (size_t)blockDim.x + threadIdx.x; i < n;
         i += (size_t)gridDim.x * blockDim.x) {
        const int x = x0 + (int)(i % ww);
        const size_t t = i / ww;
        const int y = y0 + (int)(t % wh);
        const size_t bc = t / wh;
        const size_t o = (bc * H + y) * (size_t)W + x;
        T v = 0;
        if (y < 2 * h && x < 2 * w) {
            const size_t j = (bc * h + (y >> 1)) * (size_t)w + (x >> 1);
            v = (pre[o] == pooled[j]) ? up[j] : (T)0;
        }
        out[o] = v;
    }
}

template <typename T>
__global__ __launch_bounds__(256) void depool_bwd_kernel(const T* __restrict__ gout,
                                                         const T* __restrict__ pre,
                                                         const T* __restrict__ pooled,
                                                         T* __restrict__ gup, int BC, int H, int W,
                                                         int h, int w) {
    const size_t n = (size_t)BC * h * w;
    for (size_t i = blockIdx.x * (size_t)blockDim.x + threadIdx.x; i < n;
         i += (size_t)gridDim.x * blockDim.x) {
        const int ox = (int)(i % w);
        const size_t t = i / w;
        const int oy = (int)(t % h);
        const size_t bc = t / h;
        const size_t o = (bc * H + 2 * oy) * (size_t)W + 2 * ox;
        const T m = pooled[i];
        T s = 0;
        s += pre[o] == m ? gout[o] : (T)0;
        s += pre[o + 1] == m ? gout[o + 1] : (T)0;
        s += pre[o + W] == m ? gout[o + W] : (T)0;
        s += pre[o + W + 1] == m ? gout[o + W + 1] : (T)0;
        gup[i] = s;
    }
}

template <typename T>
__global__ __launch_bounds__(256) void pool_relu_bwd_kernel(const T* __restrict__ gpool,
                                                            const T* __restrict__ pre,
                                                            const T* __restrict__ pooled,
                                                            T* __restrict__ gz, int BC, int H, int W,
                                                            int h, int w) {
    const size_t n = (size_t)BC * H * W;
    for (size_t i = blockIdx.x * (size_t)blockDim.x + threadIdx.x; i < n;
         i += (size_t)gridDim.x * blockDim.x) {
        const int x = (int)(i % W);
        const size_t t = i / W;
        const int y = (int)(t % H);
        const size_t bc = t / H;
        T v = 0;
        if (y < 2 * h && x < 2 * w) {
            const size_t j = (bc * h + (y >> 1)) * (size_t)w + (x >> 1);
            const T pv = pre[i];
            v = (pv == pooled[j] && pv > (T)0) ? gpool[j] : (T)0;
        }
        gz[i] = v;
    }
}

inline int grid_for(size_t n) {
    size_t g = (n + 255) / 256;
    return (int)(g < 1 ? 1 : (g > 8192 ? 8192 : g));
}

template <typename T>
int maxpool(void* stream, const T* x, T* out, int32_t BC, int32_t H, int32_t W) {
    if (!x || !out) return IISEG_ERR_NULL;
    if (BC <= 0 || H < 2 || W < 2) return IISEG_ERR_SHAPE;
    const int h = H / 2, w = W / 2;
    IISEG_LAUNCH(maxpool2x2_kernel<T>, dim3(grid_for((size_t)BC * h * w)), dim3(256), 0,
                       (hipStream_t)stream, x, out, BC, H, W, h, w);
    return iiseg_check_launch();
}

template <typename T>
int unpool(void* stream, const T* up, const T* pre, const T* pooled, T* out, int32_t BC, int32_t H,
           int32_t W) {
    if (!up || !pre || !pooled || !out) return IISEG_ERR_NULL;
    if (BC <= 0 || H < 2 || W < 2) return IISEG_ERR_SHAPE;
    IISEG_LAUNCH(unpool_eqmask_kernel<T>, dim3(grid_for((size_t)BC * H * W)), dim3(256), 0,
                       (hipStream_t)stream, up, pre, pooled, out, BC, H, W, H / 2, W / 2);
    return iiseg_check_launch();
}

template <typename T>
int maxpool_window(void* stream, const T* x, T* out, int32_t BC, int32_t H, int32_t W, int32_t y0,
                   int32_t x0, int32_t wh, int32_t ww) {
    if (!x || !out) return IISEG_ERR_NULL;
    if (BC <= 0 || H < 2 || W < 2 || y0 < 0 || x0 < 0 || wh <= 0 || ww <= 0 || y0 + wh > H / 2 ||
        x0 + ww > W / 2)
        return IISEG_ERR_SHAPE;
    IISEG_LAUNCH(maxpool2x2_window_kernel<T>, dim3(grid_for((size_t)BC * wh * ww)), dim3(256),
                       0, (hipStream_t)stream, x, out, BC, H, W, H / 2, W / 2, y0, x0, wh, ww);
    return iiseg_check_launch();
}

template <typename T>
int unpool_window(void* stream, const T* up, const T* pre, const T* pooled, T* out, int32_t BC,
                  int32_t H, int32_t W, int32_t y0, int32_t x0, int32_t wh, int32_t ww) {
    if (!up || !pre || !pooled || !out) return IISEG_ERR_NULL;
    if (BC <= 0 || H < 2 || W < 2 || y0 < 0 || x0 < 0 || wh <= 0 || ww <= 0 || y0 + wh > H ||
        x0 + ww > W)
        return IISEG_ERR_SHAPE;
    IISEG_LAUNCH(unpool_eqmask_window_kernel<T>, dim3(grid_for((size_t)BC * wh * ww)),
                       dim3(256), 0, (hipStream_t)stream, up, pre, pooled, out, BC, H, W, H / 2,
                       W / 2, y0, x0, wh, ww);
    return iiseg_check_launch();
}

template <typename T>
int depool_bwd(void* stream, const T* gout, const T* pre, const T* pooled, T* gup, int32_t BC,
               int32_t H, int32_t W) {
    if (!gout || !pre || !pooled || !gup) return IISEG_ERR_NULL;
    if (BC <= 0 || H < 2 || W < 2) return IISEG_ERR_SHAPE;
    IISEG_LAUNCH(depool_bwd_kernel<T>, dim3(grid_for((size_t)BC * (H / 2) * (W / 2))), dim3(256),
                       0, (hipStream_t)stream, gout, pre, pooled, gup, BC, H, W, H / 2, W / 2);
    return iiseg_check_launch();
}

template <typename T>
int pool_relu_bwd(void* stream, const T* gpool, const T* pre, const T* pooled, T* gz, int32_t BC,
                  int32_t H, int32_t W) {
    if (!gpool || !pre || !pooled || !gz) return IISEG_ERR_NULL;
    if (BC <= 0 || H < 2 || W < 2) return IISEG_ERR_SHAPE;
    IISEG_LAUNCH(pool_relu_bwd_kernel<T>, dim3(grid_for((size_t)BC * H * W)), dim3(256), 0,
                       (hipStream_t)stream, gpool, pre, pooled, gz, BC, H, W, H / 2, W / 2);
    return iiseg_check_launch();
}

}

extern "C" int iiseg_depool_bwd_f32(void* stream, const float* gout, const float* pre,
                                    const float* pooled, float* gup, int32_t BC, int32_t H, int32_t W) {
    return depool_bwd<float>(stream, gout, pre, pooled, gup, BC, H, W);
}
extern "C" int iiseg_depool_bwd_f64(void* stream, const double* gout, const double* pre,
                                    const double* pooled, double* gup, int32_t BC, int32_t H,
                                    int32_t W) {
    return depool_bwd<double>(stream, gout, pre, pooled, gup, BC, H, W);
}
extern "C" int iiseg_pool_relu_bwd_f32(void* stream, const float* gpool, const float* pre,
                                       const float* pooled, float* gz, int32_t BC, int32_t H,
                                       int32_t W) {
    return pool_relu_bwd<float>(stream, gpool, pre, pooled, gz, BC, H, W);
}
extern "C" int iiseg_pool_relu_bwd_f64(void* stream, const double* gpool, const double* pre,
                                       const double* pooled, double* gz, int32_t BC, int32_t H,
                                       int32_t W) {
    return pool_relu_bwd<double>(stream, gpool, pre, pooled, gz, BC, H, W);
}

extern "C" int iiseg_maxpool2x2_window_f32(void* stream, const float* x, float* out, int32_t BC,
                                           int32_t H, int32_t W, int32_t y0, int32_t x0,
                                           int32_t wh, int32_t ww) {
    return maxpool_window<float>(stream, x, out, BC, H, W, y0, x0, wh, ww);
}
extern "C" int iiseg_maxpool2x2_window_f64(void* stream, const double* x, double* out, int32_t BC,
                                           int32_t H, int32_t W, int32_t y0, int32_t x0,
                                           int32_t wh, int32_t ww) {
    return maxpool_window<double>(stream, x, out, BC, H, W, y0, x0, wh, ww);
}
extern "C" int iiseg_unpool_eqmask_window_f32(void* stream, const float* up, const float* pre,
                                              const float* pooled, float* out, int32_t BC,
                                              int32_t H, int32_t W, int32_t y0, int32_t x0,
                                              int32_t wh, int32_t ww) {
    return unpool_window<float>(stream, up, pre, pooled, out, BC, H, W, y0, x0, wh, ww);
}
extern "C" int iiseg_unpool_eqmask_window_f64(void* stream, const double* up, const double* pre,
                                              const double* pooled, double* out, int32_t BC,
                                              int32_t H, int32_t W, int32_t y0, int32_t x0,
                                              int32_t wh, int32_t ww) {
    return unpool_window<double>(stream, up, pre, pooled, out, BC, H, W, y0, x0, wh, ww);
}

extern "C" int iiseg_maxpool2x2_f32(void* stream, const float* x, float* out, int32_t BC,
                                    int32_t H, int32_t W) {
    return maxpool<float>(stream, x, out, BC, H, W);
}
extern "C" int iiseg_maxpool2x2_f64(void* stream, const double* x, double* out, int32_t BC,
                                    int32_t H, int32_t W) {
    return maxpool<double>(stream, x, out, BC, H, W);
}
extern "C" int iiseg_unpool_eqmask_f32(void* stream, const float* up, const float* pre,
                                       const float* pooled, float* out, int32_t BC, int32_t H,
                                       int32_t W) {
    return unpool<float>(stream, up, pre, pooled, out, BC, H, W);
}
extern "C" int iiseg_unpool_eqmask_f64(void* stream, const double* up, const double* pre,
                                       const double* pooled, double* out, int32_t BC, int32_t H,
                                       int32_t W) {
    return unpool<double>(stream, up, pre, pooled, out, BC, H, W);
}
```

### iterative_inference_segm_amd/dae.py

```python
import os

import numpy as np

import torch

from . import ops
from .weights import load_param_list

F64_FUSE_UNPOOL = os.environ.get('IISEG_F64_FUSE_UNPOOL', '1') != '0'


def _n_pool(concat_h, additional_pool):
    n = int(concat_h[-1][-1]) if 'pool' in concat_h[-1] else 0
    return n, n + additional_pool


def param_order(concat_h=('pool4',), conv_before_pool=1, additional_pool=2,
                unpool_type='trackind', bn=0):
    _, total = _n_pool(list(concat_h), additional_pool)
    names = []
    for p in range(total):
        for i in range(1, conv_before_pool + 1):
            names.append('conv%d_%d' % (p + 1, i))
            if bn:
# ... 30 lines not shown
        if unpool_type not in ('standard', 'trackind', 'inverse'):
            raise ValueError('Unkown unpool type')
        if unpool_type == 'standard' and dtype != torch.float32:
            raise NotImplementedError("unpool_type='standard' (4x4/2 transposed conv) is float32 "
                                      "only")
        self.bn = bool(bn)
        self.enc_bn = {}
        self.noise, self.dropout = float(noise), float(dropout)
        self.emulate_noise = bool(emulate_noise)
        self.random_source = None
        self._seed, self._gen = int(seed), None
        self.dtype = dtype
        self._bwd, self._saved = None, None
        self.unpool_type = unpool_type
        self.concat_h, self.padding, self.skip = concat_h, padding, skip
        self.conv_before_pool = conv_before_pool
        self.n_classes = n_classes
        self.n_pool, self.total = _n_pool(concat_h, additional_pool)
        self.device = device
        self.enc, self.dec = {}, {}
        for p in range(self.total):
            for i in range(1, conv_before_pool + 1):
                first_pad = (p == 0 and i == 1 and (len(concat_h) == 1 or pad_multi_concat)
                             and concat_h[-1] != 'input' and padding > 0)
                name = 'conv%d_%d' % (p + 1, i)
                self.enc[name] = ops.Conv(params[name][0], params[name][1],
                                          pad=padding if first_pad else 1, relu=True,
                                          device=device, dtype=dtype, mma=mma)
                if bn:
                    self.enc_bn[name] = tuple(
                        torch.as_tensor(np.asarray(a)).to(dtype).contiguous().to(device)
                        for a in params[name + '_bn'])
        self.hsplit = {}
        if dtype == torch.float32 and os.environ.get('IISEG_H_SPLIT', '1') != '0':
            prev = n_classes
            for p in range(self.total):
                name = 'conv%d_1' % (p + 1)
                W, b = params[name]
                ch = W.shape[1] - prev
                at = 'input' if p == 0 else 'pool%d' % p
                if ch > 0 and at in concat_h:
                    Wt = torch.as_tensor(W)
                    conv_h = ops.Conv(Wt[:, :ch].contiguous(), b, pad=self.enc[name].pad,
                                      relu=False, device=device, dtype=dtype, mma=mma)
                    conv_y = ops.Conv(Wt[:, ch:].contiguous(), None, pad=self.enc[name].pad,
                                      relu=True, device=device, dtype=dtype, mma=mma)
                    self.hsplit[name] = (conv_h, conv_y)
                prev = params['conv%d_%d' % (p + 1, conv_before_pool)][0].shape[0]
        for p in range(self.total, 0, -1):
            if unpool_type == 'standard':
                name = 'up%d' % p
                self.dec[name] = ops.Conv(params[name][0], params[name][1], pad=0, relu=False,
                                          layout='iohw', transposed=True, device=device,
                                          dtype=dtype, mma=mma)
                continue
            name = 'up_conv%d' % p
            W, b = params[name]
            if bn:
                beta, gamma, mean, inv_std = (np.asarray(a, np.float64) for a in params[name + '_bn'])
                sc = gamma * inv_std
                W = np.asarray(W, np.float64) * sc[:, None, None, None]
                b = (np.asarray(b, np.float64) - mean) * sc + beta
            self.dec[name] = ops.Conv(W, b, pad=1, relu=False, device=device,
                                      dtype=dtype, mma=mma)
        self.conv_log = None
        env = os.environ.get('IISEG_FUSE_UNPOOL', 'auto')
        self.fuse_unpool = None if env == 'auto' else env != '0'
        self.dce = os.environ.get('IISEG_DECODER_DCE', '1') != '0'
        self.licm = os.environ.get('IISEG_ENCODER_LICM', '1') != '0'
        self.fold_border = os.environ.get('IISEG_DAE_BORDER_FOLD', '1') != '0'
        self._store = None
        self._scratch_sessions = {}
        self.trace = None
        self.use_masks = os.environ.get('IISEG_DEPOOL_MASKS', '1') != '0'
        self.keep_pre = False

    def _mask_levels(self, overridden):
        if not self.use_masks or overridden or self.keep_pre or self.bn or self.trace is not None or \
                self.unpool_type == 'standard' or self.dtype not in (torch.float32, torch.float64) or \
                self.fuse_unpool is False:
            return frozenset()
        levels = set()
        for L in range(1, self.total + 1):
            enc = self.enc['conv%d_%d' % (L, self.conv_before_pool)]
            fed_by_h = self.conv_before_pool == 1 and \
                ('input' if L == 1 else 'pool%d' % (L - 1)) in self.concat_h
            if not fed_by_h and enc.pool_fusable(False) and enc.mask_ok(False) and \
                    self.dec['up_conv%d' % L].mask_ok(False):
                levels.add(L)
        return frozenset(levels)

    def new_session(self, h_list=None, y=None, tags=None):
        tags = list(tags) if tags is not None else [None] * len(h_list or [])
        if self.licm and self.fold_border and y is not None and tags and \
                all(t is not None for t in tags):
            key = (tuple(t[0] for t in tags), tuple(y.shape), y.dtype)
            st = self._store
            if st is not None and st.get('key') == key and st.get('primed'):
                st['y8_fresh'] = False
                st['h_fresh'] = True
                st['h_dep'] = [t[1] for t in tags]
                return st
            self._store = {'primed': False, 'key': key}
            return self._store
        if self.c8 and y is not None and h_list is not None and \
                all(isinstance(h, torch.Tensor) for h in h_list):
            key = (tuple(tuple(h.shape) for h in h_list), tuple(y.shape), y.dtype)
            st = self._scratch_sessions.get(key)
            if st is None:
                while len(self._scratch_sessions) >= 2:
                    self._scratch_sessions.pop(next(iter(self._scratch_sessions)))
                st = self._scratch_sessions[key] = {'stable': True}
            else:
                self._scratch_sessions[key] = self._scratch_sessions.pop(key)
            st.update(primed=False, h_stale=True, y8_fresh=False, h_fresh=False)
            return st
        return {'primed': False}

    @property
    def stable_sessions(self):
        return bool(self.c8)

    def conv_layers(self):
        d = dict(self.enc)
        d.update(self.dec)
        return d

    def scores(self, h_list, y, mask_override=None, session=None):
        h_list = list(h_list)
        if len(h_list) != len(self.concat_h):
            raise ValueError('expected %d h tensors, got %d' % (len(self.concat_h), len(h_list)))
        if self.c8:
            if mask_override is not None:
                raise NotImplementedError("mask injection needs fp32 activations (mma='bf16' / 'f32')")
            return self._scores_c8(h_list, y, session)
        pos = 0
        pending_h = None
        h_fresh = session is not None and session.get('h_fresh', False)
        if self.concat_h[pos] == 'input':
            pending_h, pos = h_list[pos], pos + 1
        t = y
        pre, pool = {}, {0: y}
        primed = session is not None and session.get('primed', False) and self.licm
        will_override = mask_override is not None or (
            self.emulate_noise and (self.noise > 0 or self.dropout > 0) and
            self.unpool_type == 'trackind')
        masked = self._mask_levels(will_override)
        if session is not None:
            if primed and session.get('masked', frozenset()) != masked:
                primed = False
            session['masked'] = masked
            if not primed:
                session['gen'] = session.get('gen', 0) + 1
        masks = {}
        dep = (0, 0, y.shape[2], y.shape[3])
        ydep = dep

        def clip(lo, hi, size):
            lo, hi = max(lo, 0), min(hi, size)
            return lo, max(hi - lo, 0)

        for p in range(self.total):
            fused_pool = None
            for i in range(1, self.conv_before_pool + 1):
                name = 'conv%d_%d' % (p + 1, i)
                conv = self.enc[name]
                fh, fw = conv.out_hw(t.shape[2], t.shape[3])
                ydep = (clip(ydep[0] + conv.pad - (conv.KH - 1), ydep[0] + ydep[2] + conv.pad, fh) +
                        clip(ydep[1] + conv.pad - (conv.KW - 1), ydep[1] + ydep[3] + conv.pad, fw))
                ydep = (ydep[0], ydep[2], ydep[1], ydep[3])
                kw = dict(anchor=(ydep[0], ydep[1]))
                if primed and pending_h is not None and h_fresh:
                    hd = session['h_dep'][pos - 1]
                    y1 = max(dep[0] + dep[2], hd[0] + hd[2])
                    x1 = max(dep[1] + dep[3], hd[1] + hd[3])
                    dep = (min(dep[0], hd[0]), min(dep[1], hd[1]), 0, 0)
                    dep = (dep[0], dep[1], y1 - dep[0], x1 - dep[1])
                if primed:
                    buf = session[name]
                    fh, fw = buf.shape[2], buf.shape[3]
                    wy0, wh = clip(dep[0] + conv.pad - (conv.KH - 1), dep[0] + dep[2] + conv.pad, fh)
                    wx0, ww = clip(dep[1] + conv.pad - (conv.KW - 1), dep[1] + dep[3] + conv.pad, fw)
                    dep = (wy0, wx0, wh, ww)
                    kw.update(window=dep, out=buf, place=(wy0, wx0))
                if pending_h is not None and name in self.hsplit:
                    conv_h, conv_y = self.hsplit[name]
                    keep = session is not None and self.licm
                    hb = session.get('hb_' + name) if keep else None
                    if hb is None:
                        hb = conv_h(pending_h)
                        if keep:
                            session['hb_' + name] = hb
                    elif h_fresh:
                        hd = session['h_dep'][pos - 1]
                        hy0, hh = clip(hd[0] + conv_h.pad - (conv_h.KH - 1), hd[0] + hd[2] + conv_h.pad,
                                       hb.shape[2])
                        hx0, hw = clip(hd[1] + conv_h.pad - (conv_h.KW - 1), hd[1] + hd[3] + conv_h.pad,
                                       hb.shape[3])
                        conv_h(pending_h, window=(hy0, hx0, hh, hw), out=hb, place=(hy0, hx0))
                    off = kw['place'] if 'place' in kw else (0, 0)
                    t = conv_y(t, add=hb, add_off=off, **kw)
                    pending_h = None
                elif pending_h is not None:
                    t = conv(pending_h, x2=t, **kw)
                    pending_h = None
                else:
                    pw_ = None
                    if i == self.conv_before_pool and not self.bn:
                        pw_ = conv.pool_window(t.shape[2], t.shape[3], dep if primed else None, c8=False)
                    if pw_ is not None:
                        fh, fw = conv.out_hw(t.shape[2], t.shape[3])
                        if primed:
                            pooled_t = session['pool%d' % (p + 1)]
                            kw.update(window=pw_, place=(pw_[0], pw_[1]))
                        else:
                            pooled_t = torch.empty((t.shape[0], conv.Cout, fh // 2, fw // 2),
                                                   dtype=t.dtype, device=t.device)
                        fused_pool = pooled_t
                        kw['pool_out'] = pooled_t
                    if (p + 1) in masked:
                        if pw_ is None:
                            raise RuntimeError('internal: level %d was planned for byte masks but '
                                               'its pool is not fused' % (p + 1))
                        m = session['mask%d' % (p + 1)] if primed else \
                            torch.empty(pooled_t.shape, dtype=torch.uint8, device=t.device)
                        masks[p + 1] = m
                        kw.update(mask_out=m, store_out=False)
                        conv(t, **kw)
                        t = torch.empty((t.shape[0], conv.Cout, fh, fw), dtype=t.dtype, device='meta')
                    else:
                        t = conv(t, **kw)
                if self.bn:
                    ops.bn_affine(t, self.enc_bn[name], window=dep if primed else None)
                if session is not None and not primed:
                    session[name] = t
                    if (p + 1) in masks and i == self.conv_before_pool:
                        session['mask%d' % (p + 1)] = masks[p + 1]
                self._count(name, conv, t, computed=(dep[2], dep[3]) if primed else None)
            pre[p + 1] = t
            ydep = (ydep[0] // 2, ydep[1] // 2,
                    min((ydep[0] + ydep[2] + 1) // 2, t.shape[2] // 2) - ydep[0] // 2,
                    min((ydep[1] + ydep[3] + 1) // 2, t.shape[3] // 2) - ydep[1] // 2)
            if primed:
                buf = session['pool%d' % (p + 1)]
                qy0, qh = clip(dep[0] // 2, (dep[0] + dep[2] + 1) // 2, buf.shape[2])
                qx0, qw = clip(dep[1] // 2, (dep[1] + dep[3] + 1) // 2, buf.shape[3])
                dep = (qy0, qx0, qh, qw)
                t = buf if fused_pool is not None else ops.maxpool2x2(t, out=buf, window=dep)
            else:
                t = fused_pool if fused_pool is not None else ops.maxpool2x2(t)
                if session is not None:
                    session['pool%d' % (p + 1)] = t
            pool[p + 1] = t
            if p < self.n_pool and pos < len(self.concat_h) and \
                    self.concat_h[pos] == 'pool%d' % (p + 1):
                pending_h, pos = h_list[pos], pos + 1
        if session is not None:
            session['primed'] = True
            session['h_fresh'] = False
        if pending_h is not None:
            raise NotImplementedError('h concatenated at the last pool feeds DePool2D directly '
                                      '(additional_pool=0); not shape-consistent in the reference')
        if self.emulate_noise and (self.noise > 0 or self.dropout > 0) and \
                self.unpool_type == 'trackind' and mask_override is None:
            mask_override = self.hidden_masks(h_list, y)
        if self.unpool_type == 'standard':
            for p in range(self.total, 0, -1):
                name = 'up%d' % p
                conv = self.dec[name]
                other = pool[p - 1]
                uh, uw = conv.out_hw(t.shape[2], t.shape[3])
                oh, ow = min(uh, other.shape[2]), min(uw, other.shape[3])
                kw = dict(window=(_center(uh, oh), _center(uw, ow), oh, ow))
                if self.skip and p > 1:
                    kw.update(add=other, add_off=(_center(other.shape[2], oh),
                                                  _center(other.shape[3], ow)))
                t = conv(t, **kw)
                self._count(name, conv, t, full=(uh, uw))
            return t
        geom = {}
        for p in range(self.total, 0, -1):
            ph, pw = pre[p].shape[2], pre[p].shape[3]
            other = pool[p - 1]
            oh, ow = min(ph, other.shape[2]), min(pw, other.shape[3])
            geom[p] = (ph, pw, oh, ow, _center(ph, oh), _center(pw, ow))
        win = {1: (0, 0, geom[1][2], geom[1][3])}
        for p in range(1, self.total):
            ph, pw, oh, ow, cy, cx = geom[p]
            y0, x0, nh, nw = win[p]
            uy0, ux0 = max(cy + y0 - 1, 0), max(cx + x0 - 1, 0)
            uy1, ux1 = min(cy + y0 + nh + 1, ph), min(cx + x0 + nw + 1, pw)
            qh, qw = geom[p + 1][2], geom[p + 1][3]
            ny0, nx0 = uy0 // 2, ux0 // 2
            ny1, nx1 = min((uy1 + 1) // 2, qh), min((ux1 + 1) // 2, qw)
            win[p + 1] = (ny0, nx0, ny1 - ny0, nx1 - nx0)
        need = win if self.dce else {p: (0, 0, geom[p][2], geom[p][3]) for p in geom}
        for p in range(self.total, 0, -1):
            name = 'up_conv%d' % p
            conv = self.dec[name]
            ph, pw, oh, ow, cy, cx = geom[p]
            other = pool[p - 1]
            y0, x0, nh, nw = need[p]
            window = (cy + y0, cx + x0, nh, nw)
            mpre, mpool = pre[p], pool[p]
            if mask_override and p in mask_override:
                mpre, mpool = mask_override[p]
            fuse = self.fuse_unpool
            if fuse is None:
                fuse = conv.dtype == torch.float32 or getattr(conv, 'wino_f64', False) or \
                    (F64_FUSE_UNPOOL and (conv.KH, conv.KW, conv.dil) == (3, 3, 1) and not conv.transposed)
            if not fuse:
                uy0, ux0 = max(cy + y0 - 1, 0), max(cx + x0 - 1, 0)
                uy1, ux1 = min(cy + y0 + nh + 1, ph), min(cx + x0 + nw + 1, pw)
                u = torch.empty_like(mpre)
                t = ops.unpool_eqmask(t, mpre, mpool, out=u, window=(uy0, ux0, uy1 - uy0, ux1 - ux0))
                mpre = mpool = None
            full = (nh, nw) == (oh, ow)
            out = None if full else torch.empty((y.shape[0], conv.Cout, oh, ow), dtype=y.dtype,
                                                device=y.device)
            kw = dict(pre=mpre, pooled=mpool, window=window, out=out,
                      place=None if full else (y0, x0),
                      anchor=(cy + win[p][0], cx + win[p][1]))
            if p in masks:
                kw.update(pre=None, pooled=None, mask_in=masks[p], unpool_hw=(ph, pw))
            if self.skip and p > 1:
                kw.update(add=other, add_off=(_center(other.shape[2], oh) + y0,
                                              _center(other.shape[3], ow) + x0))
            t = conv(t, **kw)
            self._count(name, conv, t, full=(ph, pw), computed=(nh, nw))
            if self.trace is not None:
                self.trace['fused_up%d' % p] = t
                self.trace['need%d' % p] = need[p]
        if self.trace is not None:
# ... 336 lines not shown
```

### iterative_inference_segm_amd/fcn8.py

```python
import itertools
import os

import numpy as np
import torch

from . import ops
from .weights import load_param_list

PARAM_ORDER = ['conv1_1', 'conv1_2', 'conv2_1', 'conv2_2', 'conv3_1', 'conv3_2', 'conv3_3',
               'conv4_1', 'conv4_2', 'conv4_3', 'conv5_1', 'conv5_2', 'conv5_3',
               'fc6', 'fc7', 'score_fr', 'score2', 'score_pool4', 'score4', 'score_pool3',
               'upsample']

_BLOCKS = [('conv1_1', 'conv1_2'), ('conv2_1', 'conv2_2'), ('conv3_1', 'conv3_2', 'conv3_3'),
           ('conv4_1', 'conv4_2', 'conv4_3'), ('conv5_1', 'conv5_2', 'conv5_3')]


_UID = itertools.count(1)


def _center(big, small):
    return (big - small) // 2


# ... 3 lines not shown


def _conv_region(dep, conv, fh, fw):
    ey, ex = conv.dil * (conv.KH - 1), conv.dil * (conv.KW - 1)
    y0, h = _clip(dep[0] + conv.pad - ey, dep[0] + dep[2] + conv.pad, fh)
    x0, w = _clip(dep[1] + conv.pad - ex, dep[1] + dep[3] + conv.pad, fw)
    return (y0, x0, h, w)


def _pool_region(dep, ph, pw):
    y0, h = _clip(dep[0] // 2, (dep[0] + dep[2] + 1) // 2, ph)
    x0, w = _clip(dep[1] // 2, (dep[1] + dep[3] + 1) // 2, pw)
    return (y0, x0, h, w)


class FCN8:
    def __init__(self, params, n_classes, layer=('probs_dimshuffle',), pad=100, temperature=1.0,
                 device='cuda', dtype=torch.float32, mma=None):
        if mma is None:
            mma = 'f32' if ops.DEFAULT_MMA == 'bf16x3' else ops.DEFAULT_MMA
        self.c8 = mma in ('bf16c8', 'bf16x3') and dtype == torch.float32
        self.x3 = self.c8 and mma == 'bf16x3'
        self.layer = list(layer)
        self.n_classes = n_classes
        self.pad = pad
        self.device = device
        self.dtype = dtype
        p = params
        c = lambda name, pad_, relu=True: ops.Conv(p[name][0], p[name][1], pad=pad_, relu=relu,
                                                   device=device, dtype=dtype, mma=mma)
        self.convs = {}
        for bi, names in enumerate(_BLOCKS):
            for ni, name in enumerate(names):
                self.convs[name] = c(name, pad if (bi == 0 and ni == 0) else 1)
        self.convs['fc6'] = c('fc6', 0)
        self.convs['fc7'] = c('fc7', 0)
        self.convs['score_fr'] = c('score_fr', 0)
        self.convs['score_pool4'] = c('score_pool4', 0)
        self.convs['score_pool3'] = c('score_pool3', 0)
        self.score2 = ops.Deconv(p['score2'][0], p['score2'][1], 2, device=device, dtype=dtype)
        self.score4 = ops.Deconv(p['score4'][0], p['score4'][1], 2, device=device, dtype=dtype)
        Wu, bu = p['upsample']
        self.upsample = ops.Deconv(np.asarray(Wu) / temperature, np.asarray(bu) / temperature, 8,
                                   device=device, dtype=dtype)
        self.conv_log = None
        self.fold_border = os.environ.get('IISEG_FCN_BORDER_FOLD', '1') != '0'
        self._border = {}
        self._uid = next(_UID)
        self.last_provenance = None

    def conv_layers(self):
        return self.convs

    def __call__(self, x):
        return self.forward(x)

    def forward(self, x, hs=None, session=None):
        hs = hs or {}
        own = False
        if session is None and self.fold_border and not hs:
            key = (tuple(x.shape), x.dtype)
            if self._border.get('key') != key:
                self._border = {'key': key, 'primed': False}
            session, own = self._border, True
        primed = session is not None and session.get('primed', False)
        net = {'input': x}
        t = x
        c8 = self.c8 and not hs
        if c8:
            t = ops.nchw_to_c8(x, x3=self.x3)
        dep = (0, 0, x.shape[2], x.shape[3])
        deps = {}
        pending = hs.get('input')
        for bi, names in enumerate(_BLOCKS):
            fused_pool = None
            for name in names:
                conv = self.convs[name]
                fh, fw = conv.out_hw(t.shape[2], t.shape[3])
                dep = _conv_region(dep, conv, fh, fw)
                kw = dict(anchor=(dep[0], dep[1]))
                if primed:
                    kw.update(window=dep, out=session[name], place=(dep[0], dep[1]))
                if name == names[-1] and pending is None:
                    pw_ = conv.pool_window(t.shape[2], t.shape[3], dep if primed else None, c8=c8)
                    if pw_ is not None:
                        if primed:
                            fused_pool = session['pool%d' % (bi + 1)]
                            kw.update(window=pw_, place=(pw_[0], pw_[1]))
                        elif c8:
                            fused_pool = ops.empty_c8(t.shape[0], conv.Cout, fh // 2, fw // 2, t.device,
                                                      x3=self.x3)
                        else:
                            fused_pool = torch.empty((t.shape[0], conv.Cout, fh // 2, fw // 2),
                                                     dtype=t.dtype, device=t.device)
                        kw['pool_out'] = fused_pool
                        if c8:
                            kw = dict(pool_out=fused_pool, store_out=False)
                            if primed:
                                kw['window'] = pw_
                if pending is not None:
                    t = self._conv(name, pending, x2=t, **kw)
                    pending = None
                else:
                    t = self._conv(name, t, **kw)
                if session is not None and not primed:
                    session[name] = t
            pname = 'pool%d' % (bi + 1)
            dep = _pool_region(dep, fh // 2, fw // 2)
            if fused_pool is not None:
                t = fused_pool
                if session is not None and not primed:
                    session[pname] = t
            elif primed:
                t = ops.maxpool2x2(t, out=session[pname], window=dep)
            else:
                t = ops.maxpool2x2(t)
                if session is not None:
                    session[pname] = t
            net[pname] = t
            deps[pname] = dep
            pending = hs.get(pname)
        if session is not None:
            session['primed'] = True
        if c8:
            f32 = {k: ops.c8_to_nchw(v, self.convs[_BLOCKS[int(k[-1]) - 1][-1]].Cout, x3=self.x3)
                   for k, v in net.items() if k.startswith('pool') and
                   (k in self.layer or k in ('pool3', 'pool4'))}
            net.update(f32)
            t = ops.c8_to_nchw(t, self.convs['conv5_3'].Cout, x3=self.x3)
        if pending is not None:
            t = self._conv('fc6', pending, x2=t)
        else:
            t = self._conv('fc6', t)
        t = self._conv('fc7', t)
        t = self._conv('score_fr', t)
        t = self._deconv_sum(self.score2, t, 'score_pool4', net['pool4'])
        t = self._deconv_sum(self.score4, t, 'score_pool3', net['pool3'])
        H, W = x.shape[2], x.shape[3]
        uh, uw = self.upsample.out_hw(t.shape[2], t.shape[3])
        oh, ow = min(uh, H), min(uw, W)
        score = self.upsample(t, window=(_center(uh, oh), _center(uw, ow), oh, ow))
        net['score'] = score
        net['probs_dimshuffle'] = ops.crop_softmax(score, oh, ow, off=(0, 0))
        res, prov = [], []
        for el in self.layer:
            t = net[el]
            tag = None
            if own and el.startswith('pool'):
                if not c8:
                    t = t.clone()
                tag = ((self._uid, session['key']), deps[el])
            res.append(t)
            prov.append(tag)
        self.last_provenance = prov
        return res

    def new_session(self):
        return {'primed': False}

    def _conv(self, name, t, **kw):
        conv = self.convs[name]
        out = conv(t, **kw)
        if self.conv_log is not None:
            fh, fw = conv.out_hw(t.shape[2], t.shape[3])
            if kw.get('window') is not None:
                ch, cw = kw['window'][2], kw['window'][3]
            elif out is not None:
# ... 78 lines not shown
```

### iterative_inference_segm_amd/ops.py

```python
import ctypes as C
import os

import torch

from . import _lib
from ._lib import ConvDesc, DeconvDesc, CONV_RELU, CONV_UNPOOL, CONV_TRANSPOSED2, CONV_X3, CONV_ZINS, check

CONV_PROFILE = None
CONV_PROFILE_INFO = None
KERNEL_BYTES = {}

_SUFFIX = {torch.float32: 'f32', torch.float64: 'f64'}

WINO_MIN_CIN = int(os.environ.get('IISEG_WINO_MIN_CIN', '128'))
WINO_F64 = os.environ.get('IISEG_WINO_F64', '1') != '0'
WINO_F64_MIN_CIN = int(os.environ.get('IISEG_WINO_F64_MIN_CIN', '128'))
WINO_F64_MIN_COUT = int(os.environ.get('IISEG_WINO_F64_MIN_COUT', '128'))
WINO_MIN_COUT = int(os.environ.get('IISEG_WINO_MIN_COUT', '128'))
WINO_FUSED_MAX_CIN = int(os.environ.get('IISEG_WINO_FUSED_MAX_CIN', '256'))
POOL_FUSE = os.environ.get('IISEG_POOL_FUSE', '1') != '0'
F64_POOL_FUSE = os.environ.get('IISEG_F64_POOL_FUSE', '1') != '0'
F64_MASKS = os.environ.get('IISEG_F64_MASKS', '1') != '0'
BNRELU_FUSE = os.environ.get('IISEG_BNRELU_FUSE', '0') != '0'
CONV_GEMM = os.environ.get('IISEG_CONV_GEMM', '1') != '0'
DEFAULT_MMA = os.environ.get('IISEG_MMA', 'f32')
BF16_WINO_MIN_CIN = int(os.environ.get('IISEG_BF16_WINO_MIN_CIN', '256'))
BF16_TUNE = os.environ.get('IISEG_BF16_TUNE', '0') == '1'
BF16_FORCE = os.environ.get('IISEG_BF16_FORM', '')
BF16_PICKS_FILE = os.path.join(os.path.dirname(os.path.abspath(__file__)), 'bf16_picks.json')


def _bf16_key(Cin, Cout, C1, C2, unpool, OH, OW):
    return '%d,%d,%d,%d,%d,%d,%d' % (Cin, Cout, C1, C2, 1 if unpool else 0, OH, OW)


def _load_bf16_picks():
    import json
    try:
        with open(BF16_PICKS_FILE) as f:
            return {k: v for k, v in json.load(f).get('picks', {}).items() if v in ('wino', 'halo')}
    except OSError:
        return {}


BF16_PICKS = _load_bf16_picks()
BF16_TIMES = {}


def _bf16_static_pick(Cin, OW):
    fill = OW / (32.0 * ((OW + 31) // 32))
    return 'wino' if (Cin >= 1024 or fill < 0.7) else 'halo'


C8_M16 = os.environ.get('IISEG_C8_M16', '1') != '0'
BF16_UPCONV1 = os.environ.get('IISEG_BF16_UPCONV1', '0') != '0'
BF16_WINO_MIN_COUT = int(os.environ.get('IISEG_BF16_WINO_MIN_COUT', '256'))
_wino_ws = {}
_wino_ws64 = {}
_bn_ws = {}


_WS_TAG = [0]


class workspace_tag:

    def __init__(self, tag):
        self.tag, self.prev = tag, None

    def __enter__(self):
        self.prev, _WS_TAG[0] = _WS_TAG[0], self.tag
        return self

    def __exit__(self, *exc):
        _WS_TAG[0] = self.prev
        return False


def _ws_key(device):
    return (device, _WS_TAG[0])


def _wino_workspace(n, device):
    key = _ws_key(device)
    ws = _wino_ws.get(key)
    if ws is None or ws.numel() < n:
        _wino_ws[key] = None
        ws = _wino_ws[key] = torch.empty(int(n), dtype=torch.float32, device=device)
    return ws


def _wino_workspace64(n, device):
    key = _ws_key(device)
    ws = _wino_ws64.get(key)
    if ws is None or ws.numel() < n:
        _wino_ws64[key] = None
        ws = _wino_ws64[key] = torch.empty(int(n), dtype=torch.float64, device=device)
    return ws


_m16_ws = {}


# ... 146 lines not shown
        self._W16 = None
        self._W16c8 = None
        self._form_cache = {}
        self._plans = {}
        self._packs = {}

    def out_hw(self, H, W):
        if self.transposed:
            return (H - 1) * 2 + self.KH, (W - 1) * 2 + self.KW
        return (H + 2 * self.pad - self.dil * (self.KH - 1),
                W + 2 * self.pad - self.dil * (self.KW - 1))

    def flops(self, B, OH, OW):
        return 2.0 * self.Cin * self.Cout * self.KH * self.KW * OH * OW * B

    def _plan(self, B, C1, C2, H, W, window, add_geom, unpool, out_slice=None, place=None,
              anchor=(0, 0)):
        key = (B, C1, C2, H, W, window, add_geom, unpool, out_slice, place, anchor)
        plan = self._plans.get(key)
        if plan is not None:
            return plan
        if C1 + C2 != self.Cin:
            raise RuntimeError('conv expects %d input channels, got %d+%d' % (self.Cin, C1, C2))
        fullH, fullW = self.out_hw(H, W)
        oy0, ox0, OH, OW = window if window is not None else (0, 0, fullH, fullW)
        d = ConvDesc()
        d.B, d.C1, d.C2, d.H, d.W = B, C1, C2, H, W
        d.Cout, d.KH, d.KW, d.pad, d.dil = self.Cout, self.KH, self.KW, self.pad, self.dil
        d.oy0, d.ox0, d.OH, d.OW = oy0, ox0, OH, OW
        if add_geom is not None:
            d.AH, d.AW, d.ay0, d.ax0 = add_geom
        d.flags = (CONV_RELU if self.relu else 0) | (CONV_UNPOOL if unpool else 0) | \
            (CONV_TRANSPOSED2 if self.transposed else 0)
        if out_slice is not None:
            d.out_ctot, d.out_c0 = out_slice
        if place is not None:
            d.out_H, d.out_W, d.out_y0, d.out_x0 = place
        d.tile_y0, d.tile_x0 = int(anchor[0]) & 1, int(anchor[1]) & 1
        so, sc = self.so, self.sc
        if self.via_im2col:
            d.C1, d.C2, d.H, d.W = C1 * self.KH * self.KW, 0, fullH, fullW
            d.KH = d.KW = 1
            so, sc = self.Cin * self.KH * self.KW, 1
        pkey = (d.C1, d.C2, d.H, d.W)
        packed = self._packs.get(pkey)
        if self.dtype == torch.float64:
            check(self.lib.iiseg_conv_plan_f64(C.byref(d)), 'iiseg_conv_plan_f64')
            if packed is None:
                wp = torch.empty(d.Kpad * d.Mpad, dtype=self.dtype, device=self.W.device)
                check(self.lib.iiseg_conv_pack_f64(_stream(), C.byref(d), _ptr(self.W, self.dtype),
                                                   so, sc, _ptr(wp, self.dtype)),
                      'iiseg_conv_pack_f64')
                packed = self._packs[pkey] = (wp, None)
        else:
            check(self.lib.iiseg_conv_plan(C.byref(d)), 'iiseg_conv_plan')
            if packed is None:
                wp = torch.empty(d.Kpad * d.Mpad, dtype=self.dtype, device=self.W.device)
                ktab = torch.empty(d.Kpad * 4, dtype=torch.int32, device=self.W.device)
                check(self.lib.iiseg_conv_pack_f32(_stream(), C.byref(d), _ptr(self.W), so, sc,
                                                   _ptr(wp), _ptr(ktab, torch.int32)),
                      'iiseg_conv_pack_f32')
                packed = self._packs[pkey] = (wp, ktab)
        wp, ktab = packed
        plan = (d, wp, ktab)
        self._plans[key] = plan
        return plan

    def __call__(self, x1, x2=None, pre=None, pooled=None, add=None, add_off=(0, 0),
                 window=None, out=None, out_c0=None, place=None, anchor=(0, 0), pool_out=None,
                 mask_in=None, unpool_hw=None, mask_out=None, store_out=True, out_format=None,
                 in_c=None, bn=None, stats=None, fold=None, zins=False):
        if is_c8(x1):
            return self._call_c8(x1, x2, add, add_off, window, out, place, pool_out, mask_in,
                                 unpool_hw, mask_out, store_out, out_format, out_c0, in_c, bn, stats, fold,
                                 zins)
        if zins or in_c is not None or bn is not None or stats is not None or fold is not None:
            raise RuntimeError('in_c / bn / stats: C8 input only (layers with at most 16 output channels)')
        dt = self.dtype
        unpool = pre is not None or mask_in is not None
        masked = mask_in is not None or mask_out is not None
        B, C1 = x1.shape[0], x1.shape[1]
        if masked:
            if not self.mask_ok(False):
                raise RuntimeError('DePool2D byte masks need a halo-kernel layer (Conv.mask_ok)')
            if mask_in is not None and (pre is not None or mask_in.dtype != torch.uint8 or
                                        mask_in.shape != x1.shape or unpool_hw is None or
                                        (unpool_hw[0] // 2, unpool_hw[1] // 2) != tuple(x1.shape[2:])):
                raise RuntimeError('mask_in: uint8 of x1\'s shape %s with unpool_hw, without pre'
                                   % (tuple(x1.shape),))
            if mask_out is not None and (pool_out is None or mask_out.dtype != torch.uint8 or
                                         mask_out.shape != pool_out.shape):
                raise RuntimeError('mask_out: uint8 of pool_out\'s shape')
        if not store_out and (mask_out is None or out_c0 is not None):
            raise RuntimeError('store_out=False needs pool_out and mask_out')
        if mask_in is not None:
            H, W = int(unpool_hw[0]), int(unpool_hw[1])
        elif unpool:
            H, W = pre.shape[2], pre.shape[3]
            if pooled.shape != x1.shape or pre.shape[:2] != x1.shape[:2] or \
                    (H // 2, W // 2) != tuple(x1.shape[2:]):
                raise RuntimeError('unpool shapes: up %s pre %s pooled %s'
                                   % (tuple(x1.shape), tuple(pre.shape), tuple(pooled.shape)))
        else:
            H, W = x1.shape[2], x1.shape[3]
        C2 = 0
        if x2 is not None:
            if x2.shape[0] != B or tuple(x2.shape[2:]) != (H, W):
                raise RuntimeError('concat shapes %s vs %s' % (tuple(x1.shape), tuple(x2.shape)))
            C2 = x2.shape[1]
        add_geom = None
        if add is not None:
            add_geom = (add.shape[2], add.shape[3], add_off[0], add_off[1])
            if add.shape[0] != B or add.shape[1] != self.Cout:
                raise RuntimeError('add tensor shape %s' % (tuple(add.shape),))
        if self.via_im2col:
            if x2 is not None or unpool or window is not None:
                raise NotImplementedError('float64 im2col path: plain single-source conv only')
            fullH, fullW = self.out_hw(H, W)
            cols = torch.empty((B, C1 * self.KH * self.KW, fullH, fullW), dtype=dt, device=x1.device)
            check(self.lib.iiseg_im2col_f64(_stream(), _ptr(x1, dt), _ptr(cols, dt), B, C1, H, W,
                                            self.KH, self.KW), 'iiseg_im2col_f64')
            d, wp, ktab = self._plan(B, C1, 0, H, W, None, add_geom, False)
            x1 = cols
        else:
            out_slice = None if out_c0 is None else (out.shape[1], int(out_c0))
            pl = None if place is None else (out.shape[2], out.shape[3], int(place[0]), int(place[1]))
            d, wp, ktab = self._plan(B, C1, C2, H, W, window, add_geom, unpool, out_slice, pl,
                                     (int(anchor[0]) & 1, int(anchor[1]) & 1))
        if not store_out:
            out = None
        elif place is not None:
            if self.via_im2col or out is None or out.shape[0] != B or out.dtype != dt or \
                    (out_c0 is None and out.shape[1] != self.Cout):
                raise RuntimeError('bad placement target %s' % (None if out is None else tuple(out.shape),))
        elif out_c0 is not None:
            if self.via_im2col or tuple(out.shape[2:]) != (d.OH, d.OW) or out.shape[0] != B or \
                    out.dtype != dt or out_c0 + self.Cout > out.shape[1]:
                raise RuntimeError('bad output slice %s @%d' % (tuple(out.shape), out_c0))
        elif out is None:
            out = torch.empty((B, self.Cout, d.OH, d.OW), dtype=dt, device=x1.device)
        elif tuple(out.shape) != (B, self.Cout, d.OH, d.OW) or out.dtype != dt:
            raise RuntimeError('out shape %s != %s' % (tuple(out.shape), (B, self.Cout, d.OH, d.OW)))
        prof = CONV_PROFILE
        wino16 = not masked and pool_out is None and self.wino_bf16 and \
            bool(self.lib.iiseg_conv_wino_bf16_supported(C.byref(d)))
        if wino16 and self.lib.iiseg_conv_halo_bf16_supported(C.byref(d)):
            key = _bf16_key(self.Cin, self.Cout, C1, C2, unpool, d.OH, d.OW)
            pick = BF16_FORCE or BF16_PICKS.get(key)
            if not pick and BF16_TUNE and not torch.cuda.is_current_stream_capturing():
                forms = (lambda: self._call_wino_bf16(d, x1, x2, pre, pooled, add, out, None),
                         lambda: self._call_halo_bf16(d, x1, x2, pre, pooled, add, out, None, None,
                                                      None, None, B, H, W))
                ms = []
                for f in forms:
                    f()
                    e0 = _ev(); f(); f(); f(); e1 = _ev()
                    e1.synchronize()
                    ms.append(e0.elapsed_time(e1))
                pick = BF16_PICKS[key] = 'wino' if ms[0] <= ms[1] else 'halo'
                BF16_TIMES[key] = ms
            if not pick:
                pick = _bf16_static_pick(self.Cin, d.OW)
            if pick == 'halo':
                return self._call_halo_bf16(d, x1, x2, pre, pooled, add, out, None, None, None, prof,
                                            B, H, W)
        if wino16:
            return self._call_wino_bf16(d, x1, x2, pre, pooled, add, out, prof)
        if self.halo_bf16 and \
                not (unpool and self.Cout <= 16 and mask_in is None and not BF16_UPCONV1) and \
                self.lib.iiseg_conv_halo_bf16_supported(C.byref(d)):
            return self._call_halo_bf16(d, x1, x2, pre, pooled, add, out, pool_out, mask_in,
                                        mask_out, prof, B, H, W)
        if not masked and pool_out is None and self.wino and \
                self.lib.iiseg_conv_wino_supported(C.byref(d)) and \
                self._form_by_full_map(self.lib.iiseg_conv_wino_supported, d):
            return self._call_wino(d, x1, x2, pre, pooled, add, out, prof)
        if masked and dt == torch.float64:
            if pool_out is not None:
                fh, fw = self.out_hw(H, W)
                if tuple(pool_out.shape) != (B, self.Cout, fh // 2, fw // 2) or pool_out.dtype != dt:
                    raise RuntimeError('pool_out shape %s' % (tuple(pool_out.shape),))
            ev0 = _ev() if prof is not None else None
            check(self.lib.iiseg_conv_mask_f64(_stream(), C.byref(d), _ptr(x1, dt), _ptr(x2, dt), _ptr(pre, dt),
                                               _ptr(pooled, dt), _ptr(mask_in, torch.uint8), _ptr(wp, dt),
                                               _ptr(self.b, dt), _ptr(add, dt), _ptr(out, dt), _ptr(pool_out, dt),
                                               _ptr(mask_out, torch.uint8)), 'iiseg_conv_mask_f64')
            if prof is not None:
                prof.append(('conv_halo_f64_kernel', self.flops(B, d.OH, d.OW), ev0, _ev()))
            return out
        if masked:
            if pool_out is not None:
                fh, fw = self.out_hw(H, W)
                if tuple(pool_out.shape) != (B, self.Cout, fh // 2, fw // 2):
                    raise RuntimeError('pool_out shape %s' % (tuple(pool_out.shape),))
            ev0 = _ev() if prof is not None else None
            check(self.lib.iiseg_conv_mask_f32(_stream(), C.byref(d), _ptr(x1), _ptr(x2), _ptr(pre),
                                               _ptr(pooled), _ptr(mask_in, torch.uint8), _ptr(wp),
                                               _ptr(ktab, torch.int32), _ptr(self.b), _ptr(add),
                                               _ptr(out), _ptr(pool_out),
                                               _ptr(mask_out, torch.uint8)), 'iiseg_conv_mask_f32')
            if prof is not None:
                prof.append((self.kernel, self.flops(B, d.OH, d.OW), ev0, _ev()))
            return out
        if pool_out is not None and dt == torch.float64:
            fh, fw = self.out_hw(H, W)
            if tuple(pool_out.shape) != (B, self.Cout, fh // 2, fw // 2) or pool_out.dtype != dt or \
                    not self.lib.iiseg_conv_pool_f64_supported(C.byref(d)) or add is not None:
                raise RuntimeError('conv + pool fusion is not available for this launch')
            ev0 = _ev() if prof is not None else None
            check(self.lib.iiseg_conv_pool_f64(_stream(), C.byref(d), _ptr(x1, dt), _ptr(x2, dt), _ptr(pre, dt),
                                               _ptr(pooled, dt), _ptr(wp, dt), _ptr(self.b, dt), None,
                                               _ptr(out, dt), _ptr(pool_out, dt)), 'iiseg_conv_pool_f64')
            if prof is not None:
                prof.append(('conv_halo_f64_kernel', self.flops(B, d.OH, d.OW), ev0, _ev()))
            return out
        if pool_out is not None:
            fh, fw = self.out_hw(H, W)
            if dt != torch.float32 or tuple(pool_out.shape) != (B, self.Cout, fh // 2, fw // 2) or \
                    not self.lib.iiseg_conv_pool_supported(C.byref(d)):
                raise RuntimeError('conv + pool fusion is not available for this launch')
            ev0 = _ev() if prof is not None else None
            check(self.lib.iiseg_conv_pool_f32(_stream(), C.byref(d), _ptr(x1), _ptr(x2), _ptr(pre),
                                               _ptr(pooled), _ptr(wp), _ptr(ktab, torch.int32),
                                               _ptr(self.b), _ptr(add), _ptr(out), _ptr(pool_out)),
                  'iiseg_conv_pool_f32')
            if prof is not None:
                prof.append((self.kernel, self.flops(B, d.OH, d.OW), ev0, _ev()))
            return out
        gemm_shape = self.kernel == 'conv_igemm_f32_kernel' or (
            dt == torch.float32 and (self.KH, self.KW) == (1, 1) and self.Cin >= 1024)
        if gemm_shape and CONV_GEMM and self.mma == 'bf16' and x2 is None and not unpool and \
                add is None and self.lib.iiseg_conv_gemm_bf16_supported(C.byref(d)):
            lib = self.lib
            if self._W16 is None:
                self._W16 = torch.empty(lib.iiseg_conv_gemm_bf16_weight_bytes(C.byref(d)) // 2,
                                        dtype=torch.bfloat16, device=self.W.device)
                check(lib.iiseg_conv_gemm_bf16_pack(_stream(), C.byref(d), _ptr(self.W), self.so,
                                                    self.sc, _ptr(self._W16, torch.bfloat16)),
                      'iiseg_conv_gemm_bf16_pack')
            ws = _wino_workspace((lib.iiseg_conv_gemm_bf16_workspace_bytes(C.byref(d)) + 3) // 4,
                                 x1.device)
            ev0 = _ev() if prof is not None else None
            check(lib.iiseg_conv_gemm_bf16(_stream(), C.byref(d), _ptr(x1),
                                           _ptr(self._W16, torch.bfloat16), _ptr(self.b), _ptr(ws),
                                           _ptr(out)), 'iiseg_conv_gemm_bf16')
            if prof is not None:
                prof.append(('wino_gemm_bf16_kernel', self.flops(B, d.OH, d.OW), ev0, _ev()))
            return out
        if gemm_shape and CONV_GEMM and x2 is None and not unpool and \
                add is None and self.lib.iiseg_conv_gemm_supported(C.byref(d)):
            ws = _wino_workspace(self.lib.iiseg_conv_gemm_workspace_elems(C.byref(d)), x1.device)
            args = (C.byref(d), _ptr(x1), _ptr(wp), _ptr(self.b), _ptr(ws), _ptr(out))
            if prof is None:
                check(self.lib.iiseg_conv_gemm_f32(_stream(), *args, 7), 'iiseg_conv_gemm_f32')
                return out
            names = ('gemm_im2col_kernel', 'wino_gemm_kernel', 'gemm_output_kernel')
            ev0 = _ev()
            for i, stage in enumerate((1, 2, 4)):
                check(self.lib.iiseg_conv_gemm_f32(_stream(), *args, stage), 'iiseg_conv_gemm_f32')
# ... 10 lines not shown
                  'iiseg_conv_gemm_f64')
            if prof is not None:
                prof.append(('wino64_gemm_kernel', self.flops(B, d.OH, d.OW), ev0, _ev()))
            return out
        if dt == torch.float64 and self.wino_f64 and not self.via_im2col and \
                self.lib.iiseg_conv_wino_f64_supported(C.byref(d)) and \
                self._form_by_full_map(self.lib.iiseg_conv_wino_f64_supported, d):
            return self._call_wino_f64(d, x1, x2, pre, pooled, add, out, prof, B)
        ev0 = _ev() if prof is not None else None
        if dt == torch.float64:
            check(self.lib.iiseg_conv_f64(_stream(), C.byref(d), _ptr(x1, dt), _ptr(x2, dt),
                                          _ptr(pre, dt), _ptr(pooled, dt), _ptr(wp, dt),
                                          _ptr(self.b, dt), _ptr(add, dt), _ptr(out, dt)),
                  'iiseg_conv_f64')
        else:
            check(self.lib.iiseg_conv_f32(_stream(), C.byref(d), _ptr(x1), _ptr(x2), _ptr(pre),
                                          _ptr(pooled), _ptr(wp), _ptr(ktab, torch.int32),
                                          _ptr(self.b), _ptr(add), _ptr(out)), 'iiseg_conv_f32')
        if prof is not None:
            ev1 = _ev()
            kern = self.kernel
            if dt == torch.float64 and self.lib.iiseg_conv_halo_f64_supported(C.byref(d)):
                kern = 'conv_halo_f64_kernel'
            if dt == torch.float32 and (add is None or self.b is None) and \
                    self.lib.iiseg_conv_small_supported(C.byref(d)):
                kern = 'conv_small_f32_kernel'
                KERNEL_BYTES[kern] = KERNEL_BYTES.get(kern, 0.0) + \
                    4.0 * B * (self.Cin * d.H * d.W + (2 if add is not None else 1) * self.Cout * d.OH * d.OW)
            if kern == 'conv_halo_f32_kernel' and C2 > 0 and C1 % 4:
                kern = 'conv_taps_f32_kernel'
            prof.append((kern, self.flops(B, d.OH, d.OW), ev0, ev1))
        return out


    def bnrelu_conv(self, stack, n, bn, out, out_c0):
        if self.dtype != torch.float32 or not BNRELU_FUSE or (self.KH, self.KW) != (3, 3) or \
                self.Cout > 16 or self.dil != 1 or self.transposed:
            return None
        B, cap, H, W = stack.shape
        pl = None
        out_slice = (out.shape[1], int(out_c0))
        d, wp, ktab = self._plan(B, n, 0, H, W, None, None, False, out_slice, pl)
        if not self.lib.iiseg_conv_bnrelu_supported(C.byref(d)) or \
                tuple(out.shape[2:]) != (d.OH, d.OW) or out_c0 + self.Cout > out.shape[1]:
            return None
        prof = CONV_PROFILE
        beta, gamma, mean, inv_std = bn
        ev0 = _ev() if prof is not None else None
        check(self.lib.iiseg_conv_bnrelu_f32(_stream(), C.byref(d), _ptr(stack), cap * H * W,
                                             _ptr(beta), _ptr(gamma), _ptr(mean), _ptr(inv_std),
                                             _ptr(wp), _ptr(ktab, torch.int32), _ptr(self.b),
                                             _ptr(out)), 'iiseg_conv_bnrelu_f32')
        if prof is not None:
            prof.append((self.kernel, self.flops(B, d.OH, d.OW), ev0, _ev()))
        return out

    def _form_by_full_map(self, supported, d):
        key = (id(supported), d.B, d.C1, d.C2, d.H, d.W, d.flags)
        ok = self._form_cache.get(key)
        if ok is None:
            full = ConvDesc()
            C.memmove(C.byref(full), C.byref(d), C.sizeof(ConvDesc))
            fh, fw = self.out_hw(d.H, d.W)
            full.oy0, full.ox0, full.OH, full.OW = 0, 0, fh, fw
            full.out_H = full.out_W = full.out_y0 = full.out_x0 = 0
            if full.AH:
                full.AH, full.AW, full.ay0, full.ax0 = max(full.AH, fh), max(full.AW, fw), 0, 0
            ok = self._form_cache[key] = bool(supported(C.byref(full)))
        return ok

    def _f64_halo_runs(self):
        ok = self._form_cache.get('f64_halo')
        if ok is None:
            d = ConvDesc()
            d.B, d.C1, d.C2, d.H, d.W = 1, self.Cin, 0, 16, 16
            d.Cout, d.KH, d.KW, d.pad, d.dil = self.Cout, self.KH, self.KW, self.pad, self.dil
            d.OH, d.OW = self.out_hw(16, 16)
            d.flags = CONV_RELU if self.relu else 0
            ok = self.lib.iiseg_conv_plan_f64(C.byref(d)) == 0 and \
                bool(self.lib.iiseg_conv_halo_f64_supported(C.byref(d)))
            self._form_cache['f64_halo'] = ok
        return ok

    def pool_fusable(self, c8=None):
        if not POOL_FUSE:
            return False
        if self.dtype == torch.float64:
            return F64_POOL_FUSE and (self.KH, self.KW) == (3, 3) and self.dil == 1 and not self.transposed and \
                not self.wino_f64 and self.Cout > 16 and self._f64_halo_runs()
        if self.dtype != torch.float32:
            return False
        if self.c8 and c8 is not False:
            return True
        if self.mma == 'bf16':
            return self.halo_bf16
        return not (self.wino or self.kernel != 'conv_halo_f32_kernel' or not 16 < self.Cout < 256)

    def mask_ok(self, c8=None):
        if self.c8 and c8 is not False:
            return True
        if self.dtype == torch.float64:
            return F64_MASKS and (self.KH, self.KW) == (3, 3) and self.dil == 1 and not self.transposed and \
                not self.wino_f64 and self._f64_halo_runs()
        if self.dtype != torch.float32 or (self.KH, self.KW) != (3, 3) or self.dil != 1 or \
                self.transposed or self.kernel != 'conv_halo_f32_kernel' or self.wino_bf16:
            return False
        return self.halo_bf16 if self.mma == 'bf16' else not self.wino

    def pool_window(self, H, W, region=None, c8=None):
        if not self.pool_fusable(c8):
            return None
        fh, fw = self.out_hw(H, W)
        if region is None:
            return (0, 0, fh, fw)
        y0, x0 = region[0] & ~1, region[1] & ~1
        y1, x1 = min((region[0] + region[2] + 1) & ~1, fh), min((region[1] + region[3] + 1) & ~1, fw)
        if region[0] + region[2] == fh:
            y1 = fh
        if region[1] + region[3] == fw:
            x1 = fw
        return (y0, x0, y1 - y0, x1 - x0)

    def c8_tiling(self, d, pool):
        t = (C.c_int32 * 4)()
        check(self.lib.iiseg_conv_c8_tiling(C.byref(d), 1 if pool else 0, t), 'iiseg_conv_c8_tiling')
        return tuple(t)

    def _call_c8_m16(self, x1, window, out, place, mask_in, unpool_hw, out_format, out_c0, in_c, bn,
                     stats=None, fold=None):
        lib = self.lib
        unpool = mask_in is not None
        B = x1.shape[0]
        in_ctot = c8_ctot(x1)
        C1 = x1.shape[1] * 8 if in_c is None else int(in_c)
        if C1 % 16 or C1 > x1.shape[1] * 8 or C1 < self.Cin or C1 - self.Cin >= 16:
            raise RuntimeError('conv of %d input channels on the first %d of %d C8 channels'
                               % (self.Cin, C1, in_ctot))
        if unpool:
            if unpool_hw is None or not is_c8_mask(mask_in) or tuple(mask_in.shape) != tuple(x1.shape) or \
                    (unpool_hw[0] // 2, unpool_hw[1] // 2) != tuple(x1.shape[2:4]) or C1 != in_ctot or \
                    not x1.is_contiguous():
                raise RuntimeError('C8 DePool2D input: up %s, mask %s, unpool_hw %s'
                                   % (tuple(x1.shape), tuple(mask_in.shape), unpool_hw))
            H, W = int(unpool_hw[0]), int(unpool_hw[1])
        else:
            H, W = x1.shape[2], x1.shape[3]
        fullH, fullW = self.out_hw(H, W)
        oy0, ox0, OH, OW = window if window is not None else (0, 0, fullH, fullW)
        fmt = out_format or ('c8' if self.Cout % 8 == 0 else 'nchw')
        if fmt not in ('c8', 'nchw'):
            raise RuntimeError('16-channel C8 layer: bf16 C8 or fp32 NCHW output')
        d = ConvDesc()
        d.B, d.C1, d.C2, d.H, d.W = B, C1, 0, H, W
        d.Cout, d.KH, d.KW, d.pad, d.dil = self.Cout, 3, 3, self.pad, 1
        d.oy0, d.ox0, d.OH, d.OW = oy0, ox0, OH, OW
        d.flags = (CONV_RELU if self.relu else 0) | (CONV_UNPOOL if unpool else 0)
        if place is not None:
            if out is None:
                raise RuntimeError('placement needs a target')
            d.out_H, d.out_W, d.out_y0, d.out_x0 = out.shape[2], out.shape[3], int(place[0]), int(place[1])
        if out is None:
            if out_c0 is not None:
                raise RuntimeError('out_c0 needs a target')
            out = torch.empty((B, self.Cout, OH, OW), dtype=torch.float32, device=x1.device) if fmt == 'nchw' \
                else torch.empty((B, 2, OH, OW, 8), dtype=torch.bfloat16, device=x1.device)
        if fmt == 'nchw':
            ok = out.dim() == 4 and out.dtype == torch.float32 and out.shape[1] == self.Cout and out_c0 is None
        else:
            ok = out.dim() == 5 and out.dtype == torch.bfloat16 and out.shape[1] % 2 == 0
            if ok and (out_c0 is not None or out.shape[1] != 2 or not out.is_contiguous()):
                c0 = int(out_c0 or 0)
                ok = c0 % 16 == 0 and c0 + 16 <= out.shape[1] * 8
                d.out_ctot, d.out_c0 = c8_ctot(out), c0
        if not ok or out.shape[0] != B or (place is None and tuple(out.shape[2:4]) != (OH, OW)):
            raise RuntimeError('bad output target %s for a 16-channel C8 layer' % (tuple(out.shape),))
        if bn is not None:
            if len(bn) != 2 or any(t.dtype != torch.float32 or t.numel() < C1 for t in bn):
                raise RuntimeError('bn = (a, b): float32, at least %d entries' % C1)
        if self._W16c8 is None:
            dp = ConvDesc()
            dp.B, dp.C1, dp.C2, dp.H, dp.W = 1, self.Cin, 0, 8, 8
            dp.Cout, dp.KH, dp.KW, dp.pad, dp.dil = self.Cout, 3, 3, 1, 1
            dp.OH, dp.OW = 8, 8
            self._W16c8 = torch.empty(lib.iiseg_conv_halo_bf16_weight_bytes(C.byref(dp)) // 2,
                                      dtype=torch.bfloat16, device=self.W.device)
            check(lib.iiseg_conv_halo_bf16_pack(_stream(), C.byref(dp), _ptr(self.W), self.so, self.sc,
                                                _ptr(self._W16c8, torch.bfloat16)),
                  'iiseg_conv_halo_bf16_pack')
        dtp = lambda t: None if t is None else (_c8ptr(t) if is_c8(t) else _ptr(t, t.dtype))
        prof = CONV_PROFILE
        ev0 = _ev() if prof is not None else None
        nws = lib.iiseg_conv_c8_m16_workspace_bytes(C.byref(d))
        ws = _m16_workspace(nws, x1.device) if nws else None
# ... 153 lines not shown
        ev0 = _ev() if prof is not None else None
        check(lib.iiseg_conv_c8_slice(_stream(), C.byref(d), dtp(x1), int(x1_ctot), dtp(x2), dtp(mask_in),
                                      dtp(self._W16c8), _ptr(self.b), dtp(add), add_kind, dtp(conv_out),
                                      conv_kind, dtp(conv_pool), dtp(conv_mask)), 'iiseg_conv_c8_slice')
        if prof is not None:
            prof.append(('conv_c8_kernel<x3>' if x3 else 'conv_c8_kernel', self.flops(B, OH, OW), ev0,
                         _ev()))
            if CONV_PROFILE_INFO is not None:
                CONV_PROFILE_INFO.append(dict(
                    Cin=self.Cin, Cout=self.Cout, C1=d.C1, C2=d.C2, H=H, W=W, OH=OH, OW=OW, B=B,
                    unpool=unpool, pool=pool_out is not None, add=add_kind, kind=conv_kind,
                    flat=self.c8_tiling(d, pool_out is not None)))
        return out

    def _call_halo_bf16(self, d, x1, x2, pre, pooled, add, out, pool_out, mask_in, mask_out, prof,
                        B, H, W):
        if pool_out is not None:
            fh, fw = self.out_hw(H, W)
            if tuple(pool_out.shape) != (B, self.Cout, fh // 2, fw // 2):
                raise RuntimeError('pool_out shape %s' % (tuple(pool_out.shape),))
        if self._W16 is None:
            self._W16 = torch.empty(self.lib.iiseg_conv_halo_bf16_weight_bytes(C.byref(d)) // 2,
                                    dtype=torch.bfloat16, device=self.W.device)
            check(self.lib.iiseg_conv_halo_bf16_pack(_stream(), C.byref(d), _ptr(self.W), self.so,
                                                     self.sc, _ptr(self._W16, torch.bfloat16)),
                  'iiseg_conv_halo_bf16_pack')
        ev0 = _ev() if prof is not None else None
        check(self.lib.iiseg_conv_halo_bf16(_stream(), C.byref(d), _ptr(x1), _ptr(x2), _ptr(pre),
                                            _ptr(pooled), _ptr(self._W16, torch.bfloat16),
                                            _ptr(self.b), _ptr(add), _ptr(out), _ptr(pool_out),
                                            _ptr(mask_in, torch.uint8),
                                            _ptr(mask_out, torch.uint8)),
              'iiseg_conv_halo_bf16')
        if prof is not None:
            prof.append(('conv_halo_bf16_kernel', self.flops(B, d.OH, d.OW), ev0, _ev()))
        return out

    def _call_wino_bf16(self, d, x1, x2, pre, pooled, add, out, prof):
        lib = self.lib
        if self._U16 is None:
            self._U16 = torch.empty(lib.iiseg_conv_wino_bf16_weight_bytes(C.byref(d)) // 2,
                                    dtype=torch.bfloat16, device=self.W.device)
            check(lib.iiseg_conv_wino_bf16_pack(_stream(), C.byref(d), _ptr(self.W), self.so,
                                                self.sc, _ptr(self._U16, torch.bfloat16)),
                  'iiseg_conv_wino_bf16_pack')
        ws = _wino_workspace((lib.iiseg_conv_wino_bf16_workspace_bytes(C.byref(d)) + 3) // 4,
                             x1.device)
        args = (C.byref(d), _ptr(x1), _ptr(x2), _ptr(pre), _ptr(pooled),
                _ptr(self._U16, torch.bfloat16), _ptr(self.b), _ptr(add), _ptr(ws), _ptr(out))
        if prof is None:
            check(lib.iiseg_conv_wino_bf16(_stream(), *args, 3), 'iiseg_conv_wino_bf16')
            return out
        r0, c0 = d.oy0 - ((d.oy0 - d.tile_y0) & 1), d.ox0 - ((d.ox0 - d.tile_x0) & 1)
        T = d.B * ((d.oy0 + d.OH - r0 + 1) // 2) * ((d.ox0 + d.OW - c0 + 1) // 2)
        kc = (self.Cin + 63) // 64 * 64
        gemm_flops = 16 * 2.0 * kc * self.Cout * T
        ev0 = _ev()
        for name, stage, fl in (('wino_input_bf16_kernel', 1, 0.0),
                                ('wino_fused_bf16_kernel', 2, gemm_flops)):
            check(lib.iiseg_conv_wino_bf16(_stream(), *args, stage), 'iiseg_conv_wino_bf16')
            ev1 = _ev()
            prof.append((name, fl, ev0, ev1))
            ev0 = ev1
        return out

    def _call_wino_f64(self, d, x1, x2, pre, pooled, add, out, prof, B):
        lib = self.lib
        dt = torch.float64
        if self._U is None:
            self._U = torch.empty(lib.iiseg_conv_wino_f64_weight_elems(C.byref(d)), dtype=dt,
                                  device=self.W.device)
            check(lib.iiseg_conv_wino_pack_f64(_stream(), C.byref(d), _ptr(self.W, dt), self.so, self.sc,
                                               _ptr(self._U, dt)), 'iiseg_conv_wino_pack_f64')
        ws = _wino_workspace64(lib.iiseg_conv_wino_f64_workspace_elems(C.byref(d)), x1.device)
        ev0 = _ev() if prof is not None else None
        check(lib.iiseg_conv_wino_f64(_stream(), C.byref(d), _ptr(x1, dt), _ptr(x2, dt), _ptr(pre, dt),
                                      _ptr(pooled, dt), _ptr(self._U, dt),
                                      _ptr(self.b, dt), _ptr(add, dt), _ptr(ws, dt), _ptr(out, dt)),
              'iiseg_conv_wino_f64')
        if prof is not None:
            prof.append(('wino64_gemm_kernel', self.flops(B, d.OH, d.OW), ev0, _ev()))
        return out

    def _call_wino(self, d, x1, x2, pre, pooled, add, out, prof):
        lib = self.lib
        if self._U is None:
            self._U = torch.empty(lib.iiseg_conv_wino_weight_elems(C.byref(d)), dtype=torch.float32,
                                  device=self.W.device)
            check(lib.iiseg_conv_wino_pack_f32(_stream(), C.byref(d), _ptr(self.W), self.so, self.sc,
                                               _ptr(self._U)), 'iiseg_conv_wino_pack_f32')
        ws = _wino_workspace(lib.iiseg_conv_wino_workspace_elems(C.byref(d)), x1.device)
        args = (C.byref(d), _ptr(x1), _ptr(x2), _ptr(pre), _ptr(pooled), _ptr(self._U),
                _ptr(self.b), _ptr(add), _ptr(ws), _ptr(out))
        fused = 8 if (self.Cin <= WINO_FUSED_MAX_CIN and self.Cin % 32 == 0 and add is None) else 0
        if prof is None:
            check(lib.iiseg_conv_wino_f32(_stream(), *args, 7 | fused), 'iiseg_conv_wino_f32')
            return out
        stages = (1 | fused, 2 | fused) if fused else (1, 2, 4)
        names = ('wino_input_kernel', 'wino_fused_kernel' if fused else 'wino_gemm_kernel',
                 'wino_output_kernel')
        r0, c0 = d.oy0 - ((d.oy0 - d.tile_y0) & 1), d.ox0 - ((d.ox0 - d.tile_x0) & 1)
        T = d.B * ((d.oy0 + d.OH - r0 + 1) // 2) * ((d.ox0 + d.OW - c0 + 1) // 2)
        gemm_flops = 16 * 2.0 * self.Cin * self.Cout * T
        ev0 = _ev()
        for i, stage in enumerate(stages):
            check(lib.iiseg_conv_wino_f32(_stream(), *args, stage), 'iiseg_conv_wino_f32')
            ev1 = _ev()
            prof.append((names[i], gemm_flops if i == 1 else 0.0, ev0, ev1))
            ev0 = ev1
        return out


DECONV_PHASE = True


class Deconv:

    def __init__(self, W, b, stride, device='cuda', dtype=torch.float32):
        self.dtype = dtype
        self.W = torch.as_tensor(W).to(dtype).contiguous().to(device)
        self.b = None if b is None else torch.as_tensor(b).to(dtype).contiguous().to(device)
        self.Cin, self.Cout, self.K, k2 = self.W.shape
        if k2 != self.K:
            raise RuntimeError('square kernels only')
        self.stride = int(stride)
        self._wp = None
        self.last_form = None

    def out_hw(self, H, W):
        return (H - 1) * self.stride + self.K, (W - 1) * self.stride + self.K

    def __call__(self, x, add=None, add_off=(0, 0), window=None, out=None):
        dt = self.dtype
        B, Cin, H, W = x.shape
        if Cin != self.Cin:
            raise RuntimeError('deconv expects %d channels, got %d' % (self.Cin, Cin))
        fullH, fullW = self.out_hw(H, W)
        oy0, ox0, OH, OW = window if window is not None else (0, 0, fullH, fullW)
        d = DeconvDesc()
        d.B, d.Cin, d.H, d.W, d.Cout, d.K, d.stride = B, Cin, H, W, self.Cout, self.K, self.stride
        d.oy0, d.ox0, d.OH, d.OW = oy0, ox0, OH, OW
        if add is not None:
            d.AH, d.AW, d.ay0, d.ax0 = add.shape[2], add.shape[3], add_off[0], add_off[1]
            if add.shape[0] != B or add.shape[1] != self.Cout:
                raise RuntimeError('add tensor shape %s' % (tuple(add.shape),))
        if out is None:
            out = torch.empty((B, self.Cout, OH, OW), dtype=dt, device=x.device)
        lib = _lib.load()
        if DECONV_PHASE and lib.iiseg_deconv_phase_supported(C.byref(d), 0 if add is None else 1,
                                                             1 if dt == torch.float64 else 0):
            if self._wp is None:
                self._wp = torch.empty(lib.iiseg_deconv_phase_weight_elems(C.byref(d)), dtype=dt, device=x.device)
                check(_fn('deconv_phase_pack', dt)(_stream(), C.byref(d), _ptr(self.W, dt), _ptr(self._wp, dt)),
                      'iiseg_deconv_phase_pack')
            check(_fn('deconv_phase', dt)(_stream(), C.byref(d), _ptr(x, dt), _ptr(self._wp, dt),
                                          _ptr(self.b, dt), _ptr(add, dt), _ptr(out, dt)), 'iiseg_deconv_phase')
            self.last_form = 'phase'
            return out
        check(_fn('deconv', dt)(_stream(), C.byref(d), _ptr(x, dt), _ptr(self.W, dt),
                                _ptr(self.b, dt), _ptr(add, dt), _ptr(out, dt)), 'iiseg_deconv')
        self.last_form = 'gather'
        return out


def is_c8(t):
    return isinstance(t, torch.Tensor) and t.dtype == torch.bfloat16 and t.dim() == 5 and \
        t.shape[-1] == 8


def c8_ctot(t):
    if not is_c8(t):
        raise RuntimeError('expected a bf16 C8 tensor')
    B, C8n, H, W, _ = t.shape
    st = t.stride()
    if tuple(st[1:]) != (H * W * 8, W * 8, 8, 1) or (B > 1 and (st[0] % (H * W * 8) or st[0] < C8n * H * W * 8)):
        raise RuntimeError('C8 operand: a contiguous tensor or a channel slice of one, got strides %s' % (st,))
    return C8n * 8 if B == 1 else st[0] // (H * W * 8) * 8


def _c8ptr(t):
    return None if t is None else C.c_void_p(t.data_ptr())


def is_c8_mask(t):
    return isinstance(t, torch.Tensor) and t.dtype == torch.uint8 and t.dim() == 5 and t.shape[-1] == 8


def c8_chunks(channels):
    return (int(channels) + 15) // 16 * 2
# ... 9 lines not shown
        out = empty_c8(B, Cc, H, W, x.device, x3=x3)
    if tuple(out.shape) != (B, c8_chunks(Cc) * (2 if x3 else 1), H, W, 8) or not is_c8(out):
        raise RuntimeError('nchw_to_c8 target %s' % (tuple(out.shape),))
    fn = _lib.load().iiseg_nchw_to_c8x3 if x3 else _lib.load().iiseg_nchw_to_c8
    check(fn(_stream(), _ptr(x), C.c_void_p(out.data_ptr()), B, Cc, H, W, c8_chunks(Cc)),
          'iiseg_nchw_to_c8')
    return out


def nchw_to_c8_slice(x, out8, c0):
    B, Cc, H, W = x.shape
    if not is_c8(out8) or c0 % 8 or tuple(out8.shape[2:4]) != (H, W) or out8.shape[0] != B:
        raise RuntimeError('nchw_to_c8_slice target %s @%d' % (tuple(out8.shape), c0))
    check(_lib.load().iiseg_nchw_to_c8_slice(_stream(), _ptr(x), C.c_void_p(out8.data_ptr()), B, Cc, H, W,
                                             c8_ctot(out8) // 8, c0 // 8), 'iiseg_nchw_to_c8_slice')
    return out8


def c8_slice_to_nchw(x8, c0, channels, out=None):
    if not is_c8(x8) or c0 % 8:
        raise RuntimeError('c8_slice_to_nchw needs a C8 tensor and c0 % 8 == 0')
    B, _, H, W, _ = x8.shape
    C8n = c8_ctot(x8) // 8
    if out is None:
        out = torch.empty((B, int(channels), H, W), dtype=torch.float32, device=x8.device)
    check(_lib.load().iiseg_c8_slice_to_nchw(_stream(), C.c_void_p(x8.data_ptr()), _ptr(out), B, int(channels),
                                             H, W, C8n, c0 // 8), 'iiseg_c8_slice_to_nchw')
    return out


def c8x3_to_float(t):
    B, C2, H, W, _ = t.shape
    v = t[:, :C2 // 2].to(torch.float32) + t[:, C2 // 2:].to(torch.float32)
    return v.permute(0, 1, 4, 2, 3).reshape(B, C2 // 2 * 8, H, W)


def c8_to_nchw(x8, channels, out=None, x3=False):
    if not is_c8(x8) or not x8.is_contiguous() or (x3 and x8.shape[1] % 2):
        raise RuntimeError('c8_to_nchw needs a contiguous C8 tensor')
    B, C8n, H, W, _ = x8.shape
    if x3:
        C8n //= 2
    if out is None:
        out = torch.empty((B, int(channels), H, W), dtype=torch.float32, device=x8.device)
    fn = _lib.load().iiseg_c8x3_to_nchw if x3 else _lib.load().iiseg_c8_to_nchw
    check(fn(_stream(), C.c_void_p(x8.data_ptr()), _ptr(out), B, int(channels), H, W, C8n),
          'iiseg_c8_to_nchw')
    return out


def unpool_c8(up, mask, out, window=None):
    B, C8n, H, W, _ = out.shape
    if not (is_c8(up) and is_c8(out) and is_c8_mask(mask)) or tuple(up.shape) != (B, C8n, H // 2, W // 2, 8) or \
            tuple(mask.shape) != tuple(up.shape) or not (up.is_contiguous() and out.is_contiguous() and
                                                          mask.is_contiguous()):
        raise RuntimeError('unpool_c8: up %s mask %s out %s' % (tuple(up.shape), tuple(mask.shape), tuple(out.shape)))
    y0, x0, wh, ww = window if window is not None else (0, 0, H // 2, W // 2)
    check(_lib.load().iiseg_unpool_c8(_stream(), _c8ptr(up), C.c_void_p(mask.data_ptr()), _c8ptr(out), B * C8n,
                                      H, W, int(y0), int(x0), int(wh), int(ww)), 'iiseg_unpool_c8')
    return out


def pool_mask_c8(pre, pooled, mask, origin, full_hw, window, x3=False):
    B, C8n, PH, PW, _ = pre.shape
    y0, x0, wh, ww = window
    if wh <= 0 or ww <= 0:
        return pooled
    if x3:
        check(_lib.load().iiseg_pool_mask_c8x3(
            _stream(), C.c_void_p(pre.data_ptr()), C.c_void_p(pooled.data_ptr()),
            None if mask is None else C.c_void_p(mask.data_ptr()), B, C8n, PH, PW, int(origin[0]),
            int(origin[1]), int(full_hw[0]), int(full_hw[1]), int(y0), int(x0), int(wh), int(ww)),
            'iiseg_pool_mask_c8x3')
        return pooled
    check(_lib.load().iiseg_pool_mask_c8(
        _stream(), C.c_void_p(pre.data_ptr()), 1 if pre.dtype == torch.float32 else 0,
        C.c_void_p(pooled.data_ptr()),
        None if mask is None else C.c_void_p(mask.data_ptr()), B * C8n, PH, PW, int(origin[0]),
        int(origin[1]), int(full_hw[0]), int(full_hw[1]), int(y0), int(x0), int(wh), int(ww)),
        'iiseg_pool_mask_c8')
    return pooled


def maxpool2x2(x, out=None, window=None):
    B, Cc, H, W = x.shape
    if out is None:
        out = torch.empty((B, Cc, H // 2, W // 2), dtype=x.dtype, device=x.device)
    if window is not None:
        y0, x0, wh, ww = window
        check(_fn('maxpool2x2_window', x.dtype)(_stream(), _ptr(x, x.dtype), _ptr(out, x.dtype),
                                                B * Cc, H, W, y0, x0, wh, ww),
              'iiseg_maxpool2x2_window')
        return out
    check(_fn('maxpool2x2', x.dtype)(_stream(), _ptr(x, x.dtype), _ptr(out, x.dtype), B * Cc, H, W),
          'iiseg_maxpool2x2')
    return out


def unpool_eqmask(up, pre, pooled, out=None, window=None):
    B, Cc, H, W = pre.shape
    if tuple(up.shape) != (B, Cc, H // 2, W // 2) or up.shape != pooled.shape:
        raise RuntimeError('unpool shapes: up %s pre %s pooled %s'
                           % (tuple(up.shape), tuple(pre.shape), tuple(pooled.shape)))
    if out is None:
        out = torch.empty_like(pre)
    dt = pre.dtype
    if window is not None:
        y0, x0, wh, ww = window
        check(_fn('unpool_eqmask_window', dt)(_stream(), _ptr(up, dt), _ptr(pre, dt),
                                              _ptr(pooled, dt), _ptr(out, dt), B * Cc, H, W, y0, x0,
                                              wh, ww), 'iiseg_unpool_eqmask_window')
        return out
    check(_fn('unpool_eqmask', dt)(_stream(), _ptr(up, dt), _ptr(pre, dt), _ptr(pooled, dt),
                                   _ptr(out, dt), B * Cc, H, W), 'iiseg_unpool_eqmask')
    return out


def crop_softmax(score, H, W, off=None, out=None, minuend=None):
    B, Cc, SH, SW = score.shape
    sy0, sx0 = off if off is not None else ((SH - H) // 2, (SW - W) // 2)
    dt = score.dtype
    if out is None:
        out = torch.empty((B, Cc, H, W), dtype=dt, device=score.device)
    check(_fn('crop_softmax', dt)(_stream(), _ptr(score, dt), _ptr(minuend, dt), _ptr(out, dt), B,
                                  Cc, SH, SW, sy0, sx0, H, W), 'iiseg_crop_softmax')
    return out


class RefineState:

    def __init__(self, B, H, W, device):
        lib = _lib.load()
        self.B, self.H, self.W = B, H, W
        self.nblk = lib.iiseg_refine_partials(H, W)
        self.active = torch.ones(B, dtype=torch.int32, device=device)
        self.iters = torch.zeros(B, dtype=torch.int32, device=device)
        self.last_norm = torch.zeros(B, dtype=torch.float64, device=device)
        self.partial = torch.zeros(B * self.nblk, dtype=torch.float64, device=device)

    def reset(self):
        self.active.fill_(1)
        self.iters.zero_()
        self.last_norm.zero_()


def refine_update(score, y, state, step, off=None, y8=None):
    B, Cc, SH, SW = score.shape
    H, W = y.shape[2], y.shape[3]
    sy0, sx0 = off if off is not None else ((SH - H) // 2, (SW - W) // 2)
    dt = y.dtype
    if y8 is not None:
        if dt != torch.float32 or not is_c8(y8) or tuple(y8.shape) != (B, y8.shape[1], H, W, 8) or \
                y8.shape[1] * 8 < Cc:
            raise RuntimeError('y8: bf16 C8 tensor of y\'s geometry')
        check(_lib.load().iiseg_refine_update_c8_f32(
            _stream(), _ptr(score), _ptr(y), _ptr(state.active, torch.int32),
            _ptr(state.partial, torch.float64), C.c_void_p(y8.data_ptr()), y8.shape[1], B, Cc, SH, SW,
            sy0, sx0, H, W, float(step)), 'iiseg_refine_update_c8_f32')
        return
    check(_fn('refine_update', dt)(_stream(), _ptr(score, dt), _ptr(y, dt),
                                   _ptr(state.active, torch.int32),
                                   _ptr(state.partial, torch.float64), B, Cc, SH, SW, sy0, sx0,
                                   H, W, float(step)), 'iiseg_refine_update')


def sqerr_softmax_bwd(score, y, off=None):
    B, Cc, SH, SW = score.shape
    H, W = y.shape[2], y.shape[3]
    sy0, sx0 = off if off is not None else ((SH - H) // 2, (SW - W) // 2)
    dt = y.dtype
# ... 242 lines not shown
```

Before: 500.6 images/s.

## Fuse 2x2 max-pool and byte-mask unpooling into fp32 Winograd conv kernels

The fp32 Winograd path gets two new abilities. Its output stage can now write a pooled map plus a byte argmax mask directly. Its input stage can unpool from a uint8 mask instead of re-reading the pre-pool activations and comparing them. This removes separate max-pool launches and the extra full-resolution reads in the DAE decoder unpooling. The cost is more template variants and extra register pressure in the output and input kernels. Fusion is only taken when the tile anchor is even and the pooling windows are whole.

```diff
diff --git a/include/iiseg.h b/include/iiseg.h
--- a/include/iiseg.h
+++ b/include/iiseg.h
@@ -85,6 +85,11 @@
 int iiseg_conv_wino_f32(void* stream, const iiseg_conv_desc* d, const float* x1, const float* x2,
                         const float* pre, const float* pooled, const float* U, const float* bias,
                         const float* add, float* workspace, float* out, uint32_t stages);
+int iiseg_conv_wino_pool_supported(const iiseg_conv_desc* d);
+int iiseg_conv_wino_mask_f32(void* stream, const iiseg_conv_desc* d, const float* x1, const float* x2,
+                             const float* pre, const float* pooled, const uint8_t* mask_in,
+                             const float* U, const float* bias, const float* add, float* workspace,
+                             float* out, float* pool_out, uint8_t* mask_out, uint32_t stages);
 
 int iiseg_conv_wino_bf16_supported(const iiseg_conv_desc* d);
 int64_t iiseg_conv_wino_bf16_weight_bytes(const iiseg_conv_desc* d);
@@ -185,6 +190,9 @@
                                 int32_t W, int32_t y0, int32_t x0, int32_t wh, int32_t ww);
 int iiseg_maxpool2x2_window_f64(void* stream, const double* x, double* out, int32_t BC, int32_t H,
                                 int32_t W, int32_t y0, int32_t x0, int32_t wh, int32_t ww);
+int iiseg_maxpool2x2_mask_window_f32(void* stream, const float* x, float* out, uint8_t* mask,
+                                     int32_t BC, int32_t H, int32_t W, int32_t y0, int32_t x0,
+                                     int32_t wh, int32_t ww);
 
 int iiseg_unpool_eqmask_f32(void* stream, const float* up, const float* pre,
                             const float* pooled, float* out, int32_t BC, int32_t H, int32_t W);
diff --git a/iterative_inference_segm_amd/_lib.py b/iterative_inference_segm_amd/_lib.py
--- a/iterative_inference_segm_amd/_lib.py
+++ b/iterative_inference_segm_amd/_lib.py
@@ -4,7 +4,7 @@
 HERE = os.path.dirname(os.path.abspath(__file__))
 LIB_PATH = os.path.join(HERE, 'libiiseg_hip.so')
 
-ABI_VERSION = 32
+ABI_VERSION = 33
 
 CONV_RELU = 1
 CONV_UNPOOL = 2
@@ -64,6 +64,8 @@
     'iiseg_conv_wino_workspace_elems': (_i64, [C.POINTER(ConvDesc)]),
     'iiseg_conv_wino_pack_f32': (C.c_int, [_vp, C.POINTER(ConvDesc), _vp, _i64, _i64, _vp]),
     'iiseg_conv_wino_f32': (C.c_int, [_vp, C.POINTER(ConvDesc)] + [_vp] * 9 + [C.c_uint32]),
+    'iiseg_conv_wino_pool_supported': (C.c_int, [C.POINTER(ConvDesc)]),
+    'iiseg_conv_wino_mask_f32': (C.c_int, [_vp, C.POINTER(ConvDesc)] + [_vp] * 12 + [C.c_uint32]),
     'iiseg_conv_wino_bf16_supported': (C.c_int, [C.POINTER(ConvDesc)]),
     'iiseg_conv_wino_bf16_weight_bytes': (_i64, [C.POINTER(ConvDesc)]),
     'iiseg_conv_wino_bf16_workspace_bytes': (_i64, [C.POINTER(ConvDesc)]),
@@ -116,6 +118,7 @@
     'iiseg_unpool_eqmask_f32': (C.c_int, [_vp, _vp, _vp, _vp, _vp, _i32, _i32, _i32]),
     'iiseg_maxpool2x2_window_f32': (C.c_int, [_vp] * 3 + [_i32] * 7),
     'iiseg_maxpool2x2_window_f64': (C.c_int, [_vp] * 3 + [_i32] * 7),
+    'iiseg_maxpool2x2_mask_window_f32': (C.c_int, [_vp] * 4 + [_i32] * 7),
     'iiseg_unpool_eqmask_window_f32': (C.c_int, [_vp] * 5 + [_i32] * 7),
     'iiseg_unpool_eqmask_window_f64': (C.c_int, [_vp] * 5 + [_i32] * 7),
     'iiseg_deconv_f32': (C.c_int, [_vp, C.POINTER(DeconvDesc)] + [_vp] * 5),
diff --git a/iterative_inference_segm_amd/csrc/abi.hip b/iterative_inference_segm_amd/csrc/abi.hip
--- a/iterative_inference_segm_amd/csrc/abi.hip
+++ b/iterative_inference_segm_amd/csrc/abi.hip
@@ -63,5 +63,5 @@
     return hipGetErrorString((hipError_t)iiseg_hip_error_slot());
 }
 
-extern "C" int iiseg_abi_version(void) { return 32; }
+extern "C" int iiseg_abi_version(void) { return 33; }
 extern "C" const char* iiseg_target_arch(void) { return "gfx950"; }
diff --git a/iterative_inference_segm_amd/csrc/conv_wino.hip b/iterative_inference_segm_amd/csrc/conv_wino.hip
--- a/iterative_inference_segm_amd/csrc/conv_wino.hip
+++ b/iterative_inference_segm_amd/csrc/conv_wino.hip
@@ -14,6 +14,7 @@
     const float* x2;
     const float* pre;
     const float* pooled;
+    const uint8_t* mask_in;
     int h2, w2;
     const float* U;
     const float* bias;
@@ -31,7 +32,26 @@
     int relu;
     int out_ctot, out_c0, out_H, out_W, out_y0, out_x0;
     int n_ttiles, n_mtiles;
+    float* pool;
+    uint8_t* mask_out;
+    int pool_H, pool_W;
 };
+
+__device__ __forceinline__ float pool4(float v00, float v01, float v10, float v11) {
+    const float a = v00 > v01 ? v00 : v01;
+    const float b = v10 > v11 ? v10 : v11;
+    return a > b ? a : b;
+}
+
+__device__ __forceinline__ void pool_store(const WinoParams& p, int b, int co, int ay, int ax,
+                                           float v00, float v01, float v10, float v11) {
+    const float m = pool4(v00, v01, v10, v11);
+    const size_t po = ((size_t)b * p.Cout + co) * p.pool_H * p.pool_W + (size_t)(ay >> 1) * p.pool_W + (ax >> 1);
+    p.pool[po] = m;
+    if (p.mask_out)
+        p.mask_out[po] = (uint8_t)((v00 == m ? 1u : 0u) | (v01 == m ? 2u : 0u) |
+                                   (v10 == m ? 4u : 0u) | (v11 == m ? 8u : 0u));
+}
 
 constexpr int RSRC_W3 = 0x00027000;
 
@@ -71,7 +91,7 @@
 }
 
 constexpr int ICH = 4;
-template <bool UNPOOL, int PY, int PX>
+template <bool UNPOOL, int PY, int PX, bool MB = false>
 __global__ __launch_bounds__(256) void wino_input_kernel(const WinoParams p) {
     const int t = blockIdx.x * 256 + threadIdx.x;
     if (t >= p.T) return;
@@ -105,12 +125,24 @@
     const size_t xis = (size_t)p.Kc * p.Tpad;
     constexpr int NC_ = UNPOOL ? ICH / 2 : ICH;
     const int c0 = blockIdx.y * NC_;
-    float pv[NC_][4][4];
-    float pq[UNPOOL ? NC_ : 1][NQY][NQX], uq[UNPOOL ? NC_ : 1][NQY][NQX];
+    float pv[MB ? 1 : NC_][4][4];
+    float pq[UNPOOL && !MB ? NC_ : 1][NQY][NQX], uq[UNPOOL ? NC_ : 1][NQY][NQX];
+    uint32_t mq[MB ? NC_ : 1][NQY][NQX];
 #pragma unroll
     for (int cc = 0; cc < NC_; ++cc) {
         const int c = min(c0 + cc, p.Kc - 1);
-        if constexpr (UNPOOL) {
+        if constexpr (MB) {
+            const uint8_t* mp = p.mask_in + ((size_t)b * p.C1 + c) * hw2;
+            const float* upp = p.x1 + ((size_t)b * p.C1 + c) * hw2;
+#pragma unroll
+            for (int i = 0; i < NQY; ++i)
+#pragma unroll
+                for (int j = 0; j < NQX; ++j) {
+                    const int o = (qrok[i] && qcok[j]) ? qoff[i] + j : 0;
+                    mq[cc][i][j] = mp[o];
+                    uq[cc][i][j] = upp[o];
+                }
+        } else if constexpr (UNPOOL) {
             const float* prep = p.pre + ((size_t)b * p.C1 + c) * HW;
             const float* poolp = p.pooled + ((size_t)b * p.C1 + c) * hw2;
             const float* upp = p.x1 + ((size_t)b * p.C1 + c) * hw2;
@@ -144,7 +176,12 @@
         for (int i = 0; i < 4; ++i)
 #pragma unroll
             for (int j = 0; j < 4; ++j) {
-                if constexpr (UNPOOL) {
+                if constexpr (MB) {
+                    const int qi = (PY + i) >> 1, qj = (PX + j) >> 1;
+                    const int bit = ((PY + i) & 1) * 2 + ((PX + j) & 1);
+                    const bool ok = rok[i] && cok[j] && qrok[qi] && qcok[qj];
+                    d[i][j] = (ok && ((mq[cc][qi][qj] >> bit) & 1u)) ? uq[cc][qi][qj] : 0.f;
+                } else if constexpr (UNPOOL) {
                     const int qi = (PY + i) >> 1, qj = (PX + j) >> 1;
                     const bool ok = rok[i] && cok[j] && qrok[qi] && qcok[qj];
                     d[i][j] = (ok && pv[cc][i][j] == pq[cc][qi][qj]) ? uq[cc][qi][qj] : 0.f;
@@ -173,7 +210,7 @@
 
 
 constexpr int ILDS_E = 12, ILDS_CH = 8;
-template <bool UNPOOL, int NT>
+template <bool UNPOOL, int NT, bool MB = false>
 __global__ __launch_bounds__(NT) void wino_input_lds_kernel(const WinoParams p, const int chunks) {
     constexpr int ILDS_CAP = ILDS_E * NT;
     __shared__ __attribute__((aligned(16))) float Ls[2][ILDS_CAP];
@@ -197,6 +234,7 @@
         if constexpr (UNPOOL) {
             ok = ok && iy < 2 * p.h2 && ix < 2 * p.w2;
             qoff[i] = ok ? (iy >> 1) * p.w2 + (ix >> 1) : -1;
+            if constexpr (MB) goff[i] = (iy & 1) * 2 + (ix & 1);
         }
     }
     const int tyl = tl / p.ntx, txl = tl - tyl * p.ntx;
@@ -208,7 +246,21 @@
     float v[ILDS_E];
 
     auto fetch = [&](int c) __attribute__((always_inline)) {
-        if constexpr (UNPOOL) {
+        if constexpr (MB) {
+            const uint8_t* mp = p.mask_in + ((size_t)b * p.C1 + c) * hw2;
+            const float* upp = p.x1 + ((size_t)b * p.C1 + c) * hw2;
+            uint32_t mq[ILDS_E];
+            float uq[ILDS_E];
+#pragma unroll
+            for (int i = 0; i < ILDS_E; ++i) {
+                const int qo = qoff[i] >= 0 ? qoff[i] : 0;
+                mq[i] = mp[qo];
+                uq[i] = upp[qo];
+            }
+#pragma unroll
+            for (int i = 0; i < ILDS_E; ++i)
+                v[i] = (qoff[i] >= 0 && ((mq[i] >> goff[i]) & 1u)) ? uq[i] : 0.f;
+        } else if constexpr (UNPOOL) {
             const float* prep = p.pre + ((size_t)b * p.C1 + c) * HW;
             const float* poolp = p.pooled + ((size_t)b * p.C1 + c) * hw2;
             const float* upp = p.x1 + ((size_t)b * p.C1 + c) * hw2;
@@ -567,8 +619,10 @@
         const bool rok[2] = {(unsigned)wy < (unsigned)p.OH, (unsigned)(wy + 1) < (unsigned)p.OH};
         const bool cok[2] = {(unsigned)wx < (unsigned)p.OW, (unsigned)(wx + 1) < (unsigned)p.OW};
         const bool pair = cok[0] && cok[1];
-        float* ob = p.out + ((size_t)b * p.out_ctot + p.out_c0) * OPL +
-                    (ptrdiff_t)(p.out_y0 + wy) * p.out_W + p.out_x0 + wx;
+        const bool whole = p.pool && rok[1] && cok[1];
+        float* ob = p.out ? p.out + ((size_t)b * p.out_ctot + p.out_c0) * OPL +
+                                (ptrdiff_t)(p.out_y0 + wy) * p.out_W + p.out_x0 + wx
+                          : nullptr;
         const float* ab = p.add ? p.add + (size_t)b * p.Cout * APL +
                                       (ptrdiff_t)(p.ay0 + wy) * p.AW + p.ax0 + wx
                                 : nullptr;
@@ -579,8 +633,29 @@
                 const int co = m0 + wm * WTM + i * 32 + (r & 3) + 8 * (r >> 2) + 4 * lh;
                 if (co >= p.Cout) continue;
                 const float bias = bias_r[i][r];
-                float* oc = ob + (size_t)co * OPL;
+                float* oc = ob ? ob + (size_t)co * OPL : nullptr;
                 const float* ac = ab ? ab + (size_t)co * APL : nullptr;
+                if (whole) {
+                    float v[2][2];
+#pragma unroll
+                    for (int a = 0; a < 2; ++a) {
+                        v[a][0] = Y[2 * a][i][j][r] + bias;
+                        v[a][1] = Y[2 * a + 1][i][j][r] + bias;
+                        if (ac) {
+                            const f32x2u a2 = *reinterpret_cast<const f32x2u*>(ac + a * p.AW);
+                            v[a][0] += a2[0];
+                            v[a][1] += a2[1];
+                        }
+                        if (p.relu) {
+                            v[a][0] = fmaxf(v[a][0], 0.f);
+                            v[a][1] = fmaxf(v[a][1], 0.f);
+                        }
+                        if (oc) *reinterpret_cast<f32x2u*>(oc + (size_t)a * p.out_W) = f32x2u{v[a][0], v[a][1]};
+                    }
+                    pool_store(p, b, co, p.oy0 + wy, p.ox0 + wx, v[0][0], v[0][1], v[1][0], v[1][1]);
+                    continue;
+                }
+                if (!oc) continue;
 #pragma unroll
                 for (int a = 0; a < 2; ++a) {
                     if (!rok[a]) continue;
@@ -659,21 +734,24 @@
             s2[1][j] = m1 - m2 - m3;
         }
         const float bias = p.bias ? p.bias[co] : 0.f;
-        float* o = p.out + ((size_t)b * p.out_ctot + p.out_c0 + co) * OPL +
-                   (ptrdiff_t)(p.out_y0 + wy) * p.out_W + p.out_x0 + wx;
+        float* o = p.out ? p.out + ((size_t)b * p.out_ctot + p.out_c0 + co) * OPL +
+                               (ptrdiff_t)(p.out_y0 + wy) * p.out_W + p.out_x0 + wx
+                         : nullptr;
+        float vt[2][2];
 #pragma unroll
         for (int i = 0; i < 2; ++i) {
             float y[2] = {s2[i][0] + s2[i][1] + s2[i][2], s2[i][1] - s2[i][2] - s2[i][3]};
 #pragma unroll
             for (int j = 0; j < 2; ++j) {
-                if (okr[i] && okc[j]) {
-                    float v = y[j] + bias;
-                    if (p.add) v += av[cc][i * 2 + j];
-                    if (p.relu) v = fmaxf(v, 0.f);
-                    o[(ptrdiff_t)i * p.out_W + j] = v;
-                }
-            }
-        }
+                float v = y[j] + bias;
+                if (p.add) v += av[cc][i * 2 + j];
+                if (p.relu) v = fmaxf(v, 0.f);
+                vt[i][j] = v;
+                if (o && okr[i] && okc[j]) o[(ptrdiff_t)i * p.out_W + j] = v;
+            }
+        }
+        if (p.pool && okr[1] && okc[1])
+            pool_store(p, b, co, p.oy0 + wy, p.ox0 + wx, vt[0][0], vt[0][1], vt[1][0], vt[1][1]);
     }
 }
 
@@ -712,6 +790,7 @@
 }
 
 void launch_wino_input(hipStream_t s, const WinoParams& p, bool unpool) {
+    const bool mb = unpool && p.mask_in;
     static const int lds = getenv("IISEG_WINO_INPUT_LDS") ? atoi(getenv("IISEG_WINO_INPUT_LDS")) : 1;
     const int ntt = p.nty * p.ntx;
     int nt = 0;
@@ -726,8 +805,9 @@
     if (lds && nt && best >= 0.8 && p.Kc % ILDS_CH == 0) {
         const int chunks = (ntt + nt - 1) / nt;
         const dim3 g2(p.B * chunks, p.Kc / ILDS_CH);
-#define WINO_ILDS(U, N) IISEG_LAUNCH((wino_input_lds_kernel<U, N>), g2, dim3(N), 0, s, p, chunks)
-        if (unpool) { if (nt == 256) WINO_ILDS(true, 256); else if (nt == 128) WINO_ILDS(true, 128); else WINO_ILDS(true, 64); }
+#define WINO_ILDS(U, N, ...) IISEG_LAUNCH((wino_input_lds_kernel<U, N, ##__VA_ARGS__>), g2, dim3(N), 0, s, p, chunks)
+        if (mb) { if (nt == 256) WINO_ILDS(true, 256, true); else if (nt == 128) WINO_ILDS(true, 128, true); else WINO_ILDS(true, 64, true); }
+        else if (unpool) { if (nt == 256) WINO_ILDS(true, 256); else if (nt == 128) WINO_ILDS(true, 128); else WINO_ILDS(true, 64); }
         else { if (nt == 256) WINO_ILDS(false, 256); else if (nt == 128) WINO_ILDS(false, 128); else WINO_ILDS(false, 64); }
 #undef WINO_ILDS
         return;
@@ -739,6 +819,13 @@
         return;
     }
     const int py = (p.ty0 - p.pad) & 1, px = (p.tx0 - p.pad) & 1;
+    if (mb) {
+        if (py && px) IISEG_LAUNCH((wino_input_kernel<true, 1, 1, true>), grid, block, 0, s, p);
+        else if (py) IISEG_LAUNCH((wino_input_kernel<true, 1, 0, true>), grid, block, 0, s, p);
+        else if (px) IISEG_LAUNCH((wino_input_kernel<true, 0, 1, true>), grid, block, 0, s, p);
+        else IISEG_LAUNCH((wino_input_kernel<true, 0, 0, true>), grid, block, 0, s, p);
+        return;
+    }
     if (py && px) IISEG_LAUNCH((wino_input_kernel<true, 1, 1>), grid, block, 0, s, p);
     else if (py) IISEG_LAUNCH((wino_input_kernel<true, 1, 0>), grid, block, 0, s, p);
     else if (px) IISEG_LAUNCH((wino_input_kernel<true, 0, 1>), grid, block, 0, s, p);
@@ -803,24 +890,45 @@
     return iiseg_check_launch();
 }
 
-extern "C" int iiseg_conv_wino_f32(void* stream, const iiseg_conv_desc* d, const float* x1,
-                                   const float* x2, const float* pre, const float* pooled,
-                                   const float* U, const float* bias,
-                                   const float* add, float* workspace, float* out,
-                                   uint32_t stages) {
+static bool wino_pool_ok(const iiseg_conv_desc* d) {
+    WinoGeom g;
+    if (wino_geom(d, g) != IISEG_OK) return false;
+    const int fullH = d->H + 2 * d->pad - 2, fullW = d->W + 2 * d->pad - 2;
+    if ((d->tile_y0 | d->tile_x0 | d->oy0 | d->ox0) & 1) return false;
+    if ((d->OH & 1) && d->oy0 + d->OH != fullH) return false;
+    if ((d->OW & 1) && d->ox0 + d->OW != fullW) return false;
+    return true;
+}
+
+extern "C" int iiseg_conv_wino_pool_supported(const iiseg_conv_desc* d) {
+    return wino_pool_ok(d) ? 1 : 0;
+}
+
+static int wino_run(void* stream, const iiseg_conv_desc* d, const float* x1, const float* x2,
+                    const float* pre, const float* pooled, const uint8_t* mask_in, const float* U,
+                    const float* bias, const float* add, float* workspace, float* out,
+                    float* pool_out, uint8_t* mask_out, uint32_t stages) {
     WinoGeom g;
     const int st = wino_geom(d, g);
     if (st) return st;
-    if (!x1 || !U || !workspace || !out) return IISEG_ERR_NULL;
+    if (!x1 || !U || !workspace || !(out || pool_out)) return IISEG_ERR_NULL;
     if (d->C2 > 0 && !x2) return IISEG_ERR_NULL;
     const bool unpool = (d->flags & IISEG_CONV_UNPOOL) != 0;
-    if (unpool && (!pre || !pooled)) return IISEG_ERR_NULL;
+    if (mask_in && !unpool) return IISEG_ERR_UNSUPPORTED;
+    if (unpool && !mask_in && (!pre || !pooled)) return IISEG_ERR_NULL;
+    if (mask_out && !pool_out) return IISEG_ERR_UNSUPPORTED;
+    if (pool_out && !wino_pool_ok(d)) return IISEG_ERR_UNSUPPORTED;
     if (((uintptr_t)U & 15) || ((uintptr_t)workspace & 15)) return IISEG_ERR_ALIGN;
-    WinoParams p;
+    WinoParams p = {};
     p.x1 = x1;
     p.x2 = x2;
-    p.pre = pre;
-    p.pooled = pooled;
+    p.pre = mask_in ? nullptr : pre;
+    p.pooled = mask_in ? nullptr : pooled;
+    p.mask_in = mask_in;
+    p.pool = pool_out;
+    p.mask_out = mask_out;
+    p.pool_H = (d->H + 2 * d->pad - 2) / 2;
+    p.pool_W = (d->W + 2 * d->pad - 2) / 2;
     p.h2 = d->H / 2;
     p.w2 = d->W / 2;
     p.U = U;
@@ -923,6 +1031,24 @@
     return iiseg_check_launch();
 }
 
+extern "C" int iiseg_conv_wino_f32(void* stream, const iiseg_conv_desc* d, const float* x1,
+                                   const float* x2, const float* pre, const float* pooled,
+                                   const float* U, const float* bias,
+                                   const float* add, float* workspace, float* out,
+                                   uint32_t stages) {
+    return wino_run(stream, d, x1, x2, pre, pooled, nullptr, U, bias, add, workspace, out, nullptr,
+                    nullptr, stages);
+}
+
+extern "C" int iiseg_conv_wino_mask_f32(void* stream, const iiseg_conv_desc* d, const float* x1,
+                                        const float* x2, const float* pre, const float* pooled,
+                                        const uint8_t* mask_in, const float* U, const float* bias,
+                                        const float* add, float* workspace, float* out,
+                                        float* pool_out, uint8_t* mask_out, uint32_t stages) {
+    return wino_run(stream, d, x1, x2, pre, pooled, mask_in, U, bias, add, workspace, out, pool_out,
+                    mask_out, stages);
+}
+
 namespace {
 
 struct GemmConvGeom {
diff --git a/iterative_inference_segm_amd/csrc/pool_unpool.hip b/iterative_inference_segm_amd/csrc/pool_unpool.hip
--- a/iterative_inference_segm_amd/csrc/pool_unpool.hip
+++ b/iterative_inference_segm_amd/csrc/pool_unpool.hip
@@ -45,9 +45,10 @@
 
 template <typename T>
 __global__ __launch_bounds__(256) void maxpool2x2_window_kernel(const T* __restrict__ x,
-                                                                T* __restrict__ out, int BC, int H,
-                                                                int W, int h, int w, int y0, int x0,
-                                                                int wh, int ww) {
+                                                                T* __restrict__ out,
+                                                                uint8_t* __restrict__ mask, int BC,
+                                                                int H, int W, int h, int w, int y0,
+                                                                int x0, int wh, int ww) {
     const size_t n = (size_t)BC * wh * ww;
     if (n < ((size_t)1 << 31)) {
         const unsigned n32 = (unsigned)n, uww = (unsigned)ww, uwh = (unsigned)wh;
@@ -60,7 +61,12 @@
             const T* r1 = r0 + W;
             const T a = r0[0] > r0[1] ? r0[0] : r0[1];
             const T b = r1[0] > r1[1] ? r1[0] : r1[1];
-            out[((size_t)bc * h + oy) * (size_t)w + ox] = a > b ? a : b;
+            const T m = a > b ? a : b;
+            const size_t o = ((size_t)bc * h + oy) * (size_t)w + ox;
+            out[o] = m;
+            if (mask)
+                mask[o] = (uint8_t)((r0[0] == m ? 1u : 0u) | (r0[1] == m ? 2u : 0u) |
+                                    (r1[0] == m ? 4u : 0u) | (r1[1] == m ? 8u : 0u));
         }
         return;
     }
@@ -74,7 +80,12 @@
         const T* r1 = r0 + W;
         const T a = r0[0] > r0[1] ? r0[0] : r0[1];
         const T b = r1[0] > r1[1] ? r1[0] : r1[1];
-        out[(bc * h + oy) * (size_t)w + ox] = a > b ? a : b;
+        const T m = a > b ? a : b;
+        const size_t o = (bc * h + oy) * (size_t)w + ox;
+        out[o] = m;
+        if (mask)
+            mask[o] = (uint8_t)((r0[0] == m ? 1u : 0u) | (r0[1] == m ? 2u : 0u) |
+                                (r1[0] == m ? 4u : 0u) | (r1[1] == m ? 8u : 0u));
     }
 }
 
@@ -173,13 +184,13 @@
 
 template <typename T>
 int maxpool_window(void* stream, const T* x, T* out, int32_t BC, int32_t H, int32_t W, int32_t y0,
-                   int32_t x0, int32_t wh, int32_t ww) {
+                   int32_t x0, int32_t wh, int32_t ww, uint8_t* mask = nullptr) {
     if (!x || !out) return IISEG_ERR_NULL;
     if (BC <= 0 || H < 2 || W < 2 || y0 < 0 || x0 < 0 || wh <= 0 || ww <= 0 || y0 + wh > H / 2 ||
         x0 + ww > W / 2)
         return IISEG_ERR_SHAPE;
     IISEG_LAUNCH(maxpool2x2_window_kernel<T>, dim3(grid_for((size_t)BC * wh * ww)), dim3(256),
-                       0, (hipStream_t)stream, x, out, BC, H, W, H / 2, W / 2, y0, x0, wh, ww);
+                       0, (hipStream_t)stream, x, out, mask, BC, H, W, H / 2, W / 2, y0, x0, wh, ww);
     return iiseg_check_launch();
 }
 
@@ -243,6 +254,12 @@
                                            int32_t wh, int32_t ww) {
     return maxpool_window<float>(stream, x, out, BC, H, W, y0, x0, wh, ww);
 }
+extern "C" int iiseg_maxpool2x2_mask_window_f32(void* stream, const float* x, float* out,
+                                                uint8_t* mask, int32_t BC, int32_t H, int32_t W,
+                                                int32_t y0, int32_t x0, int32_t wh, int32_t ww) {
+    if (!mask) return IISEG_ERR_NULL;
+    return maxpool_window<float>(stream, x, out, BC, H, W, y0, x0, wh, ww, mask);
+}
 extern "C" int iiseg_maxpool2x2_window_f64(void* stream, const double* x, double* out, int32_t BC,
                                            int32_t H, int32_t W, int32_t y0, int32_t x0,
                                            int32_t wh, int32_t ww) {
diff --git a/iterative_inference_segm_amd/dae.py b/iterative_inference_segm_amd/dae.py
--- a/iterative_inference_segm_amd/dae.py
+++ b/iterative_inference_segm_amd/dae.py
@@ -136,13 +136,49 @@
             return frozenset()
         levels = set()
         for L in range(1, self.total + 1):
-            enc = self.enc['conv%d_%d' % (L, self.conv_before_pool)]
+            name = 'conv%d_%d' % (L, self.conv_before_pool)
+            enc = self.enc[name]
             fed_by_h = self.conv_before_pool == 1 and \
                 ('input' if L == 1 else 'pool%d' % (L - 1)) in self.concat_h
-            if not fed_by_h and enc.pool_fusable(False) and enc.mask_ok(False) and \
-                    self.dec['up_conv%d' % L].mask_ok(False):
+            if fed_by_h and name in self.hsplit and self._wino_f32(self.hsplit[name][1]):
+                enc, fed_by_h = self.hsplit[name][1], False
+            if fed_by_h or not enc.mask_ok(False) or not self.dec['up_conv%d' % L].mask_ok(False):
+                continue
+            if enc.pool_fusable(False) or self._wino_f32(enc):
                 levels.add(L)
         return frozenset(levels)
+
+    @staticmethod
+    def _wino_f32(conv):
+        return conv.wino and conv.mma == 'f32' and conv.dtype == torch.float32
+
+    def _conv_pool(self, conv, p, i, t, kw, dep, primed, session, masked, masks, hb=None):
+        pw_ = None
+        fh, fw = conv.out_hw(t.shape[2], t.shape[3])
+        if i == self.conv_before_pool and not self.bn and (hb is None or self._wino_f32(conv)):
+            pw_ = conv.pool_window(t.shape[2], t.shape[3], dep if primed else None, c8=False,
+                                   anchor=kw['anchor'])
+        fused_pool = pool_mask = None
+        if pw_ is not None:
+            if primed:
+                fused_pool = session['pool%d' % (p + 1)]
+                kw.update(window=pw_, place=(pw_[0], pw_[1]))
+            else:
+                fused_pool = torch.empty((t.shape[0], conv.Cout, fh // 2, fw // 2),
+                                         dtype=t.dtype, device=t.device)
+            kw['pool_out'] = fused_pool
+        if hb is not None:
+            kw.update(add=hb, add_off=kw['place'] if 'place' in kw else (0, 0))
+        if (p + 1) not in masked or i != self.conv_before_pool:
+            return conv(t, **kw), fused_pool, None
+        m = session['mask%d' % (p + 1)] if primed else \
+            torch.empty((t.shape[0], conv.Cout, fh // 2, fw // 2), dtype=torch.uint8, device=t.device)
+        masks[p + 1] = m
+        if pw_ is None:
+            return conv(t, **kw), None, m
+        kw.update(mask_out=m, store_out=False)
+        conv(t, **kw)
+        return torch.empty((t.shape[0], conv.Cout, fh, fw), dtype=t.dtype, device='meta'), fused_pool, None
 
     def new_session(self, h_list=None, y=None, tags=None):
         tags = list(tags) if tags is not None else [None] * len(h_list or [])
@@ -215,7 +251,7 @@
             return lo, max(hi - lo, 0)
 
         for p in range(self.total):
-            fused_pool = None
+            fused_pool = pool_mask = None
             for i in range(1, self.conv_before_pool + 1):
                 name = 'conv%d_%d' % (p + 1, i)
                 conv = self.enc[name]
@@ -252,38 +288,15 @@
                         hx0, hw = clip(hd[1] + conv_h.pad - (conv_h.KW - 1), hd[1] + hd[3] + conv_h.pad,
                                        hb.shape[3])
                         conv_h(pending_h, window=(hy0, hx0, hh, hw), out=hb, place=(hy0, hx0))
-                    off = kw['place'] if 'place' in kw else (0, 0)
-                    t = conv_y(t, add=hb, add_off=off, **kw)
                     pending_h = None
+                    t, fused_pool, pool_mask = self._conv_pool(conv_y, p, i, t, kw, dep, primed, session,
+                                                               masked, masks, hb=hb)
                 elif pending_h is not None:
                     t = conv(pending_h, x2=t, **kw)
                     pending_h = None
                 else:
-                    pw_ = None
-                    if i == self.conv_before_pool and not self.bn:
-                        pw_ = conv.pool_window(t.shape[2], t.shape[3], dep if primed else None, c8=False)
-                    if pw_ is not None:
-                        fh, fw = conv.out_hw(t.shape[2], t.shape[3])
-                        if primed:
-                            pooled_t = session['pool%d' % (p + 1)]
-                            kw.update(window=pw_, place=(pw_[0], pw_[1]))
-                        else:
-                            pooled_t = torch.empty((t.shape[0], conv.Cout, fh // 2, fw // 2),
-                                                   dtype=t.dtype, device=t.device)
-                        fused_pool = pooled_t
-                        kw['pool_out'] = pooled_t
-                    if (p + 1) in masked:
-                        if pw_ is None:
-                            raise RuntimeError('internal: level %d was planned for byte masks but '
-                                               'its pool is not fused' % (p + 1))
-                        m = session['mask%d' % (p + 1)] if primed else \
-                            torch.empty(pooled_t.shape, dtype=torch.uint8, device=t.device)
-                        masks[p + 1] = m
-                        kw.update(mask_out=m, store_out=False)
-                        conv(t, **kw)
-                        t = torch.empty((t.shape[0], conv.Cout, fh, fw), dtype=t.dtype, device='meta')
-                    else:
-                        t = conv(t, **kw)
+                    t, fused_pool, pool_mask = self._conv_pool(conv, p, i, t, kw, dep, primed, session,
+                                                               masked, masks)
                 if self.bn:
                     ops.bn_affine(t, self.enc_bn[name], window=dep if primed else None)
                 if session is not None and not primed:
@@ -300,9 +313,10 @@
                 qy0, qh = clip(dep[0] // 2, (dep[0] + dep[2] + 1) // 2, buf.shape[2])
                 qx0, qw = clip(dep[1] // 2, (dep[1] + dep[3] + 1) // 2, buf.shape[3])
                 dep = (qy0, qx0, qh, qw)
-                t = buf if fused_pool is not None else ops.maxpool2x2(t, out=buf, window=dep)
+                t = buf if fused_pool is not None else \
+                    ops.maxpool2x2(t, out=buf, window=dep, mask=pool_mask)
             else:
-                t = fused_pool if fused_pool is not None else ops.maxpool2x2(t)
+                t = fused_pool if fused_pool is not None else ops.maxpool2x2(t, mask=pool_mask)
                 if session is not None:
                     session['pool%d' % (p + 1)] = t
             pool[p + 1] = t
diff --git a/iterative_inference_segm_amd/fcn8.py b/iterative_inference_segm_amd/fcn8.py
--- a/iterative_inference_segm_amd/fcn8.py
+++ b/iterative_inference_segm_amd/fcn8.py
@@ -109,7 +109,8 @@
                 if primed:
                     kw.update(window=dep, out=session[name], place=(dep[0], dep[1]))
                 if name == names[-1] and pending is None:
-                    pw_ = conv.pool_window(t.shape[2], t.shape[3], dep if primed else None, c8=c8)
+                    pw_ = conv.pool_window(t.shape[2], t.shape[3], dep if primed else None, c8=c8,
+                                           anchor=kw['anchor'])
                     if pw_ is not None:
                         if primed:
                             fused_pool = session['pool%d' % (bi + 1)]
diff --git a/iterative_inference_segm_amd/ops.py b/iterative_inference_segm_amd/ops.py
--- a/iterative_inference_segm_amd/ops.py
+++ b/iterative_inference_segm_amd/ops.py
@@ -19,6 +19,7 @@
 WINO_MIN_COUT = int(os.environ.get('IISEG_WINO_MIN_COUT', '128'))
 WINO_FUSED_MAX_CIN = int(os.environ.get('IISEG_WINO_FUSED_MAX_CIN', '256'))
 POOL_FUSE = os.environ.get('IISEG_POOL_FUSE', '1') != '0'
+WINO_POOL_FUSE = os.environ.get('IISEG_WINO_POOL_FUSE', '1') != '0'
 F64_POOL_FUSE = os.environ.get('IISEG_F64_POOL_FUSE', '1') != '0'
 F64_MASKS = os.environ.get('IISEG_F64_MASKS', '1') != '0'
 BNRELU_FUSE = os.environ.get('IISEG_BNRELU_FUSE', '0') != '0'
@@ -331,7 +332,8 @@
         B, C1 = x1.shape[0], x1.shape[1]
         if masked:
             if not self.mask_ok(False):
-                raise RuntimeError('DePool2D byte masks need a halo-kernel layer (Conv.mask_ok)')
+                raise RuntimeError('DePool2D byte masks need a halo-kernel or fp32 Winograd layer '
+                                   '(Conv.mask_ok)')
             if mask_in is not None and (pre is not None or mask_in.dtype != torch.uint8 or
                                         mask_in.shape != x1.shape or unpool_hw is None or
                                         (unpool_hw[0] // 2, unpool_hw[1] // 2) != tuple(x1.shape[2:])):
@@ -420,10 +422,16 @@
                 self.lib.iiseg_conv_halo_bf16_supported(C.byref(d)):
             return self._call_halo_bf16(d, x1, x2, pre, pooled, add, out, pool_out, mask_in,
                                         mask_out, prof, B, H, W)
-        if not masked and pool_out is None and self.wino and \
+        if self.wino and (self.mma == 'f32' or (not masked and pool_out is None)) and \
                 self.lib.iiseg_conv_wino_supported(C.byref(d)) and \
                 self._form_by_full_map(self.lib.iiseg_conv_wino_supported, d):
-            return self._call_wino(d, x1, x2, pre, pooled, add, out, prof)
+            if pool_out is not None:
+                fh, fw = self.out_hw(H, W)
+                if tuple(pool_out.shape) != (B, self.Cout, fh // 2, fw // 2) or pool_out.dtype != dt or \
+                        not self.lib.iiseg_conv_wino_pool_supported(C.byref(d)):
+                    raise RuntimeError('conv + pool fusion is not available for this launch '
+                                       '(Winograd: even tile anchor and whole pooling windows)')
+            return self._call_wino(d, x1, x2, pre, pooled, add, out, prof, mask_in, pool_out, mask_out)
         if masked and dt == torch.float64:
             if pool_out is not None:
                 fh, fw = self.out_hw(H, W)
@@ -600,7 +608,7 @@
             self._form_cache['f64_halo'] = ok
         return ok
 
-    def pool_fusable(self, c8=None):
+    def pool_fusable(self, c8=None, anchor=None):
         if not POOL_FUSE:
             return False
         if self.dtype == torch.float64:
@@ -612,7 +620,9 @@
             return True
         if self.mma == 'bf16':
             return self.halo_bf16
-        return not (self.wino or self.kernel != 'conv_halo_f32_kernel' or not 16 < self.Cout < 256)
+        if self.wino:
+            return anchor is not None and WINO_POOL_FUSE and not (int(anchor[0]) & 1 or int(anchor[1]) & 1)
+        return not (self.kernel != 'conv_halo_f32_kernel' or not 16 < self.Cout < 256)
 
     def mask_ok(self, c8=None):
         if self.c8 and c8 is not False:
@@ -621,12 +631,16 @@
             return F64_MASKS and (self.KH, self.KW) == (3, 3) and self.dil == 1 and not self.transposed and \
                 not self.wino_f64 and self._f64_halo_runs()
         if self.dtype != torch.float32 or (self.KH, self.KW) != (3, 3) or self.dil != 1 or \
-                self.transposed or self.kernel != 'conv_halo_f32_kernel' or self.wino_bf16:
+                self.transposed or self.wino_bf16:
+            return False
+        if self.mma == 'f32' and self.wino:
+            return WINO_POOL_FUSE
+        if self.kernel != 'conv_halo_f32_kernel':
             return False
         return self.halo_bf16 if self.mma == 'bf16' else not self.wino
 
-    def pool_window(self, H, W, region=None, c8=None):
-        if not self.pool_fusable(c8):
+    def pool_window(self, H, W, region=None, c8=None, anchor=None):
+        if not self.pool_fusable(c8, anchor):
             return None
         fh, fw = self.out_hw(H, W)
         if region is None:
@@ -946,7 +960,8 @@
             prof.append(('wino64_gemm_kernel', self.flops(B, d.OH, d.OW), ev0, _ev()))
         return out
 
-    def _call_wino(self, d, x1, x2, pre, pooled, add, out, prof):
+    def _call_wino(self, d, x1, x2, pre, pooled, add, out, prof, mask_in=None, pool_out=None,
+                   mask_out=None):
         lib = self.lib
         if self._U is None:
             self._U = torch.empty(lib.iiseg_conv_wino_weight_elems(C.byref(d)), dtype=torch.float32,
@@ -954,11 +969,18 @@
             check(lib.iiseg_conv_wino_pack_f32(_stream(), C.byref(d), _ptr(self.W), self.so, self.sc,
                                                _ptr(self._U)), 'iiseg_conv_wino_pack_f32')
         ws = _wino_workspace(lib.iiseg_conv_wino_workspace_elems(C.byref(d)), x1.device)
-        args = (C.byref(d), _ptr(x1), _ptr(x2), _ptr(pre), _ptr(pooled), _ptr(self._U),
-                _ptr(self.b), _ptr(add), _ptr(ws), _ptr(out))
+        if mask_in is None and pool_out is None:
+            fn, what = lib.iiseg_conv_wino_f32, 'iiseg_conv_wino_f32'
+            args = (C.byref(d), _ptr(x1), _ptr(x2), _ptr(pre), _ptr(pooled), _ptr(self._U),
+                    _ptr(self.b), _ptr(add), _ptr(ws), _ptr(out))
+        else:
+            fn, what = lib.iiseg_conv_wino_mask_f32, 'iiseg_conv_wino_mask_f32'
+            args = (C.byref(d), _ptr(x1), _ptr(x2), _ptr(pre), _ptr(pooled), _ptr(mask_in, torch.uint8),
+                    _ptr(self._U), _ptr(self.b), _ptr(add), _ptr(ws), _ptr(out), _ptr(pool_out),
+                    _ptr(mask_out, torch.uint8))
         fused = 8 if (self.Cin <= WINO_FUSED_MAX_CIN and self.Cin % 32 == 0 and add is None) else 0
         if prof is None:
-            check(lib.iiseg_conv_wino_f32(_stream(), *args, 7 | fused), 'iiseg_conv_wino_f32')
+            check(fn(_stream(), *args, 7 | fused), what)
             return out
         stages = (1 | fused, 2 | fused) if fused else (1, 2, 4)
         names = ('wino_input_kernel', 'wino_fused_kernel' if fused else 'wino_gemm_kernel',
@@ -968,7 +990,7 @@
         gemm_flops = 16 * 2.0 * self.Cin * self.Cout * T
         ev0 = _ev()
         for i, stage in enumerate(stages):
-            check(lib.iiseg_conv_wino_f32(_stream(), *args, stage), 'iiseg_conv_wino_f32')
+            check(fn(_stream(), *args, stage), what)
             ev1 = _ev()
             prof.append((names[i], gemm_flops if i == 1 else 0.0, ev0, ev1))
             ev0 = ev1
@@ -1144,10 +1166,19 @@
     return pooled
 
 
-def maxpool2x2(x, out=None, window=None):
+def maxpool2x2(x, out=None, window=None, mask=None):
     B, Cc, H, W = x.shape
     if out is None:
         out = torch.empty((B, Cc, H // 2, W // 2), dtype=x.dtype, device=x.device)
+    if mask is not None:
+        if x.dtype != torch.float32 or mask.dtype != torch.uint8 or mask.shape != out.shape:
+            raise RuntimeError('maxpool2x2 mask: float32 input, uint8 of the pooled shape')
+        y0, x0, wh, ww = window if window is not None else (0, 0, H // 2, W // 2)
+        check(_lib.load().iiseg_maxpool2x2_mask_window_f32(_stream(), _ptr(x), _ptr(out),
+                                                            _ptr(mask, torch.uint8), B * Cc, H, W,
+                                                            y0, x0, wh, ww),
+              'iiseg_maxpool2x2_mask_window_f32')
+        return out
     if window is not None:
         y0, x0, wh, ww = window
         check(_fn('maxpool2x2_window', x.dtype)(_stream(), _ptr(x, x.dtype), _ptr(out, x.dtype),
```

New measurement: 514.4 images/s, median of 6. +2.7%, better.
